# G1OJS/PyFT8

Measured on AMD Instinct MI355X. Metric: FT8 15-s frames decoded/sec, higher is better.
Workload: dtype f32

## Files before the change

pyft8_amd/csrc/ft8rx.hip:

```cpp
#include <hip/hip_runtime.h>
#include <math.h>
#include <stdarg.h>
#include <stdio.h>
#include <stdlib.h>
#include <string.h>
#include <new>
#include <string>
#include <vector>
#include "../../include/ft8rx.h"
#include "ft8_dev.h"

#define WL_MULT(i) ((i) == WL_BP0 ? 5 : (i) == WL_OSDNAN ? 10 : 1)
#define NF0MAX (FT8RX_MAX_F0 > 1024 ? 2048 : 1024)

#include "kernels/common.hpp"
#include "kernels/spectrogram.hpp"
#include "kernels/sync_search.hpp"
#include "kernels/llr.hpp"
#include "kernels/ap_patterns.hpp"
#include "kernels/bp.hpp"
#include "kernels/cycle_spectrum.hpp"
#include "kernels/fine_sync.hpp"
#include "kernels/osd.hpp"
#include "kernels/ap_calls.hpp"
#include "kernels/recall.hpp"
#include "kernels/report.hpp"
#include "kernels/synth.hpp"
#include "kernels/subtract.hpp"
#include "kernels/probes.hpp"
#include "host_messages.hpp"
#include "batch_plan.hpp"
#include "ilp_launch.hpp"

#define EV_EAGER_BYTES ((size_t)1 << 20)
#define HIPCHK(h, x) do { hipError_t _e = (x); if (_e != hipSuccess) { set_err(h, "%s failed: %s (%s:%d)", #x, hipGetErrorString(_e), __FILE__, __LINE__); return -2; } } while (0)

static std::vector<uint32_t> osd_trial_table(int S, int D, int T) {
    std::vector<uint32_t> t;
    const uint32_t N = OSD_NONE;
    t.push_back(N | (N << 8) | (N << 16));
    for (int i = 0; i < S; i++) t.push_back((uint32_t)i | (N << 8) | (N << 16));
    for (int i = 0; i < S; i++) for (int j = 0; j < D && j < i; j++) t.push_back((uint32_t)i | ((uint32_t)j << 8) | (N << 16));
    for (int i = 0; i < T; i++) for (int j = 0; j < i; j++) for (int k = 0; k < j; k++) t.push_back((uint32_t)i | ((uint32_t)j << 8) | ((uint32_t)k << 16));
    return t;
}
static int osd_nflip(int S, int T) { return S > T ? S : T; }

struct ft8rx_hashes { hostmsg::Hashes H; };

#define SYNC_WIN 352
static size_t sync_lds_bytes(const ft8rx_config& c) {
    const int nh0 = c.h0_hi - c.h0_lo;
    const size_t nrows = (size_t)((nh0 < SYNC_WIN ? nh0 : SYNC_WIN) + 24);
    return nrows * 16 * sizeof(double) + (nrows * 29 + 512) * sizeof(float);
}
static std::string g_create_err;

struct ResultSlot {
    ft8rx_record* rec = nullptr; int32_t* ncand = nullptr; ft8rx_event* ev = nullptr; int32_t* evcount = nullptr;
    ft8rx_record* h_rec = nullptr; int32_t* h_cnt = nullptr; ft8rx_event* h_ev = nullptr; int32_t* h_evc = nullptr;
    hipEvent_t ev_comp = nullptr, ev_done = nullptr;
    int B = 0;
    bool evpending = false;
    int32_t* d_evoffs = nullptr; ft8rx_event* h_evpacked = nullptr; ft8rx_event* d_evpacked = nullptr;
    bool packed = false;
    unsigned char* pk_buf = nullptr; hipEvent_t pk_fence = nullptr;
    ft8rx_packed_header* h_pkhdr = nullptr; ft8rx_packed_header* d_pkhdr = nullptr;
    bool recall = false;
    ft8rx_recall_entry* d_rc_ent = nullptr; int32_t* d_rc_cnt = nullptr; ft8rx_record* d_rc_rec = nullptr;
    ft8rx_record* h_rc_rec = nullptr; int32_t* h_rc_cnt = nullptr;
    bool reports = false;
    ft8rx_report* d_rp = nullptr; ft8rx_report* h_rp = nullptr;
};

static ApCalls ap_calls_off() { ApCalls a; memset(&a, 0, sizeof(a)); a.max_hd = FT8RX_AP_MAX_HD_DEFAULT; return a; }

struct ft8rx_handle {
    ft8rx_config cfg = {};
    int device = 0, max_frames = 0;
    hipStream_t stream = nullptr;
    int n_streams = 2;
    int ladder_mode = 0;
    int msg_types = 0;
    bool weak = false; float weak_sync_min = FT8RX_WEAK_SYNC_MIN_DEFAULT; int32_t weak_osd_max_hd = FT8RX_WEAK_OSD_MAX_HD_DEFAULT;
    ApCalls ap = ap_calls_off();
    uint32_t ap_version = 0, ap_chunk_version[batchplan::MAX_CHUNKS] = {};
    ApCalls* d_apc = nullptr;
    int32_t* d_apcount = nullptr;
    bool rc_armed = false; int rc_frames = 0; bool rc_td = false; std::vector<int32_t> rc_off;
    int32_t rc_max_hd = FT8RX_RECALL_MAX_HD_DEFAULT, rc_min_gap = FT8RX_RECALL_MIN_GAP_DEFAULT;
    ft8rx_recall_entry* d_rc_src = nullptr; int32_t* d_rc_srccnt = nullptr; int32_t* d_rc_off = nullptr;
    int32_t* d_rc_trip = nullptr; int32_t* d_rc_tout = nullptr; float* d_rc_tsd = nullptr; float* d_rc_sgrid = nullptr; float* d_rc_llr = nullptr;
    bool reports = false;
    int32_t* d_rp_items = nullptr; int32_t* d_rp_count = nullptr;
    int sub_frames = FT8RX_SUBBATCH_DEFAULT;
    hipStream_t sub[batchplan::MAX_STREAMS] = {};
    hipEvent_t ev_fork = nullptr, ev_join[batchplan::MAX_STREAMS] = {};
    hipStream_t copy_s = nullptr;
    hipEvent_t ev_chunk[batchplan::MAX_CHUNKS] = {};
    Tables T = {};
    std::vector<void*> allocs;
    struct Chunk { void* p; size_t cap, used; };
    std::vector<Chunk> arena;
    int16_t* d_audio = nullptr;
    int16_t* d_audio2 = nullptr;
    hipStream_t h2d_s = nullptr;
    float* d_grid = nullptr;
    float* d_best_score = nullptr; int32_t* d_best_h0 = nullptr;
    ft8rx_record* d_rec = nullptr; int32_t* d_ncand = nullptr; ft8rx_event* d_ev = nullptr; int32_t* d_evcount = nullptr;
    float* d_llr0 = nullptr; float* d_saved = nullptr;
    Att *d_att0 = nullptr, *d_attG = nullptr, *d_attB = nullptr, *d_attO = nullptr;
    cpx *d_A = nullptr, *d_spec = nullptr;
    const uint32_t* d_trials = nullptr; int n_trials = 0;
    int32_t* d_work[WL_N] = {};
    int32_t* d_wcount = nullptr;
    uint8_t* d_colmask = nullptr; bool use_mask = false;
    ResultSlot slots[2];
    int slot_enq = 0, slot_fetch = 0, inflight = 0, last_slot = -1, fetched_slot = -1;
    hipEvent_t ev_cdone[2][batchplan::MAX_STREAMS] = {};
    bool free_running = false, need_barrier = true; int part_B = 0, part_n = 0;
    uint64_t pk_cap = 0; uint64_t* d_pkneed = nullptr; int32_t* d_pknrec = nullptr;
    hipEvent_t d2h_ev[32] = {}; uint32_t d2h_next = 0;
    float* d_wf = nullptr; double2* d_part = nullptr; double* d_pulse = nullptr; double* d_pc = nullptr;
    ft8rx_subsig* d_sigs = nullptr; int32_t* d_sigcnt = nullptr; int sig_cap = 0;
    float2 *d_zdec = nullptr, *d_model = nullptr, *d_adec = nullptr; SubdCtx* d_subctx = nullptr;
    double* d_ones = nullptr;
    std::string err;
    bool profiling = false;
    std::vector<hipEvent_t> pev;
    std::vector<const char*> pnames;
    int n_stage = 0;
    float stage_ms[24] = {};
};
static_assert(sizeof(ft8rx_handle::ev_chunk) / sizeof(hipEvent_t) == batchplan::MAX_CHUNKS &&
              sizeof(ft8rx_handle::ap_chunk_version) / sizeof(uint32_t) == batchplan::MAX_CHUNKS &&
              sizeof(batchplan::BatchPlan::cb) / sizeof(int) == batchplan::MAX_CHUNKS + 1 &&
              batchplan::MAX_CHUNKS == 16 && batchplan::MAX_STREAMS == 8, "per-chunk arrays and the plan's boundaries");

static void set_err(ft8rx_handle* h, const char* fmt, ...) {
    char buf[512];
    va_list ap; va_start(ap, fmt); vsnprintf(buf, sizeof(buf), fmt, ap); va_end(ap);
    if (h) h->err = buf; else g_create_err = buf;
}

#include <mutex>
struct StreamPool { hipStream_t main = nullptr, copy = nullptr, h2d = nullptr, sub[8] = {}; };
static std::mutex g_pool_mu;
static StreamPool g_pool[64];
static hipStream_t pool_stream(int device, hipStream_t StreamPool::* which, bool blocking) {
    std::lock_guard<std::mutex> lk(g_pool_mu);
    StreamPool& P = g_pool[device & 63];
    if (!(P.*which)) {
        hipStream_t s = nullptr;
        if ((blocking ? hipStreamCreate(&s) : hipStreamCreateWithFlags(&s, hipStreamNonBlocking)) != hipSuccess) return nullptr;
        P.*which = s;
    }
    return P.*which;
}
static hipStream_t pool_sub(int device, int i) {
    std::lock_guard<std::mutex> lk(g_pool_mu);
    StreamPool& P = g_pool[device & 63];
    if (!P.sub[i] && hipStreamCreateWithFlags(&P.sub[i], hipStreamNonBlocking) != hipSuccess) P.sub[i] = nullptr;
    return P.sub[i];
}

template <typename T> static int dalloc(ft8rx_handle* h, T** p, size_t n) {
    void* q = nullptr;
    hipError_t e = hipMalloc(&q, n * sizeof(T));
    if (e != hipSuccess) { set_err(h, "hipMalloc(%zu bytes) failed: %s", n * sizeof(T), hipGetErrorString(e)); return -2; }
    h->allocs.push_back(q); *p = (T*)q; return 0;
}

static int need_staging(ft8rx_handle* h) {
    if (h->d_audio) return 0;
    return dalloc(h, &h->d_audio, (size_t)h->max_frames * FT8RX_NSAMP);
}

static void host_twiddle(int n, int count, std::vector<cpx>& w) {
    w.resize(count);
    for (int t = 0; t < count; t++) {
        double ang = (2.0 * M_PI * (double)t) / (double)n;
        w[t] = make_float2((float)cos(ang), (float)(-sin(ang)));
    }
}
template <typename T> static int upload(ft8rx_handle* h, const T** dst, const std::vector<T>& v) {
    T* p; if (dalloc(h, &p, v.size())) return -2;
    if (hipMemcpy(p, v.data(), v.size() * sizeof(T), hipMemcpyHostToDevice) != hipSuccess) { set_err(h, "table upload failed"); return -2; }
    *dst = p; return 0;
}

struct Scratch {
    ft8rx_handle* h;
    ~Scratch() { for (auto& c : h->arena) c.used = 0; }
    void* raw(size_t bytes) {
        bytes = (bytes + 255) & ~(size_t)255;
        if (!bytes) bytes = 256;
        for (auto& c : h->arena) if (c.cap - c.used >= bytes) { void* q = (char*)c.p + c.used; c.used += bytes; return q; }
        size_t largest = 0;
        for (auto& c : h->arena) if (c.cap > largest) largest = c.cap;
        size_t cap = bytes > 2 * largest ? bytes : 2 * largest;
        if (cap < ((size_t)1 << 20)) cap = (size_t)1 << 20;
        for (size_t i = 0; i < h->arena.size();) {
            if (h->arena[i].used == 0) { hipFree(h->arena[i].p); h->arena.erase(h->arena.begin() + i); } else i++;
        }
        void* q = nullptr;
        if (hipMalloc(&q, cap) != hipSuccess) { if (cap == bytes || hipMalloc(&q, bytes) != hipSuccess) return nullptr; cap = bytes; }
        h->arena.push_back({q, cap, bytes});
        return q;
    }
    template <typename T> T* get(size_t n) { return (T*)raw(n * sizeof(T)); }
    template <typename T> T* put(const T* src, size_t n) { T* q = get<T>(n); if (q && hipMemcpy(q, src, n * sizeof(T), hipMemcpyHostToDevice) != hipSuccess) return nullptr; return q; }
};

static int quiesce(ft8rx_handle* h, bool next_is_batch = false) {
    if (h->free_running || (h->last_slot >= 0 && !next_is_batch)) HIPCHK(h, hipStreamSynchronize(h->copy_s));
    h->free_running = false;
    h->need_barrier = true;
    return 0;
}
#define ENTER(h) do { HIPCHK(h, hipSetDevice((h)->device)); { const int _q = quiesce(h); if (_q) return _q; } } while (0)

template <class K, class KX, class... A>
static void launch_mt(K k, KX kx, unsigned mt, int grid, hipStream_t s, A... a) {
    if (!mt) k<<<grid, 64, 0, s>>>(a...);
    else kx<<<grid, 64, 0, s>>>(a..., mt);
}

extern "C" {

int ft8rx_default_config(ft8rx_config* c) {
    if (!c) return -1;
    c->sync_score_min = 85.0f; c->max_cands = 200; c->f0_lo = 32; c->f0_hi = 960; c->h0_lo = -37; c->h0_hi = 87;
    c->bp_nc0_a = 35; c->bp_iters_a = 5; c->bp_nc0_b = 90; c->bp_iters_b = 20; c->osd_single = 30; c->osd_double = 2;
    c->llr_sd_min = 5.0f;
    c->osd_triple = 0; c->osd_max_hd = 0;
    return 0;
}

int ft8rx_device_count(void) { int n = 0; if (hipGetDeviceCount(&n) != hipSuccess) return 0; return n; }
int ft8rx_device_pci_bus_id(int device, char* buf, int len) {
    if (!buf || len < 16) return -1;
    return hipDeviceGetPCIBusId(buf, len, device) == hipSuccess ? 0 : -2;
}
int ft8rx_build_info(int32_t* grid_cols, int32_t* spec_bins, int32_t* max_f0) {
    static_assert(NF0MAX >= FT8RX_GRID_COLS && NF0MAX >= FT8RX_MAX_F0, "per-f0 scratch stride");
    if (grid_cols) *grid_cols = FT8RX_GRID_COLS;
    if (spec_bins) *spec_bins = FT8RX_SPEC_BINS;
    if (max_f0) *max_f0 = FT8RX_MAX_F0;
    return 0;
}
int ft8rx_build_limits(int32_t* max_cands, int32_t* event_cap) {
    static_assert(FT8RX_MAX_CANDS <= NF0MAX && (1 << cand_shift(FT8RX_MAX_CANDS)) == FT8RX_MAX_CANDS,
                  "max_cands: never more than k_topk has keys, and the largest candidate stride is the limit itself");
    if (max_cands) *max_cands = FT8RX_MAX_CANDS;
    if (event_cap) *event_cap = FT8RX_EVENT_CAP;
    return 0;
}

int ft8rx_get_fft_plans(int32_t* p1920, int32_t* p3200, int32_t* p300, int32_t* p320) {
    const int32_t a[8] = {8, 4, 4, 5, 3, 0, 0, 0}, b[8] = {8, 4, 4, 5, 5, 0, 0, 0}, c[8] = {5, 5, 4, 3, 0, 0, 0, 0}, d[8] = {8, 8, 5, 0, 0, 0, 0, 0};
    if (p1920) memcpy(p1920, a, sizeof(a));
    if (p3200) memcpy(p3200, b, sizeof(b));
    if (p300) memcpy(p300, c, sizeof(c));
    if (p320) memcpy(p320, d, sizeof(d));
    return 0;
}

const char* ft8rx_last_error(ft8rx_handle* h) { return h ? h->err.c_str() : g_create_err.c_str(); }

void ft8rx_destroy(ft8rx_handle* h) {
    if (!h) return;
    hipSetDevice(h->device);
    if (h->stream) hipStreamSynchronize(h->stream);
    if (h->copy_s) hipStreamSynchronize(h->copy_s);
    if (h->h2d_s) hipStreamSynchronize(h->h2d_s);
    for (int i = 0; i < 8; i++) { if (h->sub[i]) hipStreamSynchronize(h->sub[i]); if (h->ev_join[i]) hipEventDestroy(h->ev_join[i]); }
    for (void* p : h->allocs) hipFree(p);
    for (auto& c : h->arena) hipFree(c.p);
    for (auto e : h->pev) hipEventDestroy(e);
    for (int k = 0; k < 2; k++) for (int i = 0; i < 8; i++) if (h->ev_cdone[k][i]) hipEventDestroy(h->ev_cdone[k][i]);
    for (int i = 0; i < 32; i++) if (h->d2h_ev[i]) hipEventDestroy(h->d2h_ev[i]);
    for (hipEvent_t e : h->ev_chunk) if (e) hipEventDestroy(e);
    if (h->ev_fork) hipEventDestroy(h->ev_fork);
    for (ResultSlot& sl : h->slots) {
        if (sl.ev_comp) hipEventDestroy(sl.ev_comp);
        if (sl.ev_done) hipEventDestroy(sl.ev_done);
        const auto hfree = [](void* p) { if (p) hipHostFree(p); };
        hfree(sl.h_rec); hfree(sl.h_cnt); hfree(sl.h_ev); hfree(sl.h_evc); hfree(sl.h_evpacked); hfree(sl.h_pkhdr);
        hfree(sl.h_rc_rec); hfree(sl.h_rc_cnt); hfree(sl.h_rp);
    }
    delete h;
}

int ft8rx_create(const ft8rx_config* cfg, int device, int max_frames, ft8rx_handle** out) {
    if (!cfg || !out || max_frames < 1) { set_err(nullptr, "ft8rx_create: bad arguments"); return -1; }
    if (cfg->max_cands < 1 || cfg->max_cands > FT8RX_MAX_CANDS || cfg->f0_lo < 4 || cfg->f0_hi > FT8RX_MAX_F0 || cfg->f0_lo >= cfg->f0_hi ||
        cfg->h0_hi <= cfg->h0_lo || cfg->h0_lo < FT8RX_MIN_H0 || cfg->h0_hi > FT8RX_MAX_H0 || cfg->bp_nc0_a > cfg->bp_nc0_b || cfg->bp_iters_a > cfg->bp_iters_b ||
        cfg->osd_single < 0 || cfg->osd_single > OSD_MAXFLIP || cfg->osd_double < 0 || cfg->osd_double > OSD_MAXFLIP ||
        cfg->osd_triple < 0 || cfg->osd_triple > 40 || cfg->osd_max_hd < 0 || cfg->osd_max_hd > 174 ||
        osd_trial_table(cfg->osd_single, cfg->osd_double, cfg->osd_triple).size() > OSD_MAXTRIALS) {
        set_err(nullptr, "ft8rx_create: configuration out of the supported range"); return -1; }
    int ndev = 0;
    if (hipGetDeviceCount(&ndev) != hipSuccess || ndev < 1) { set_err(nullptr, "ft8rx_create: no HIP device available (this library has no CPU fallback)"); return -3; }
    if (device < 0 || device >= ndev) { set_err(nullptr, "ft8rx_create: device %d out of range (%d devices)", device, ndev); return -1; }
    ft8rx_handle* h = new ft8rx_handle();
    h->cfg = *cfg; h->device = device; h->max_frames = max_frames;
    if (hipSetDevice(device) != hipSuccess || !(h->stream = pool_stream(device, &StreamPool::main, true))) { set_err(nullptr, "ft8rx_create: cannot open device %d", device); delete h; return -2; }
    const size_t B = (size_t)max_frames, S = (size_t)1 << cand_shift(*cfg);
    int rc = 0;
    rc |= dalloc(h, &h->d_grid, B * FT8RX_GRID_ROWS * FT8RX_GRID_COLS);
    rc |= dalloc(h, &h->d_best_score, B * NF0MAX);
    rc |= dalloc(h, &h->d_best_h0, B * NF0MAX);
    rc |= dalloc(h, &h->d_rec, B * S);
    rc |= dalloc(h, &h->d_ncand, B);
    rc |= dalloc(h, &h->d_llr0, B * S * 174);
    rc |= dalloc(h, &h->d_saved, B * S * 5 * 174);
    rc |= dalloc(h, &h->d_att0, B * S * 5);
    rc |= dalloc(h, &h->d_attG, B * S * 2);
    rc |= dalloc(h, &h->d_attB, B * S * 5);
    rc |= dalloc(h, &h->d_attO, B * S * 10);
    static_assert((size_t)(96000 + FT8RX_SPEC_BINS) * sizeof(cpx) <= (size_t)FT8RX_GRID_ROWS * FT8RX_GRID_COLS * sizeof(float), "scratch A + cycle spectrum fit a frame's grid");
    if (!rc) { h->d_A = reinterpret_cast<cpx*>(h->d_grid); h->d_spec = h->d_A + B * 96000; }
    for (int i = 0; i < WL_N; i++) rc |= dalloc(h, &h->d_work[i], B * S * WL_MULT(i));
    rc |= dalloc(h, &h->d_wcount, (size_t)batchplan::MAX_CHUNKS * WL_N);
    rc |= dalloc(h, &h->d_apc, batchplan::MAX_CHUNKS);
    rc |= dalloc(h, &h->d_apcount, (size_t)batchplan::MAX_CHUNKS * 2);
    rc |= dalloc(h, &h->d_ev, B * FT8RX_EVENT_CAP);
    rc |= dalloc(h, &h->d_evcount, B);
    ResultSlot* const sl = h->slots;
    sl[0].rec = h->d_rec; sl[0].ncand = h->d_ncand; sl[0].ev = h->d_ev; sl[0].evcount = h->d_evcount;
    rc |= dalloc(h, &sl[1].rec, B * S);
    rc |= dalloc(h, &sl[1].ncand, B);
    rc |= dalloc(h, &sl[1].ev, B * FT8RX_EVENT_CAP);
    rc |= dalloc(h, &sl[1].evcount, B);
    const bool ev_compact = B * FT8RX_EVENT_CAP * sizeof(ft8rx_event) > EV_EAGER_BYTES;
    for (int k = 0; k < 2 && ev_compact; k++) rc |= dalloc(h, &sl[k].d_evoffs, B + 1);
    for (int k = 0; k < 2 && !rc; k++) {
        bool okh = hipHostMalloc((void**)&sl[k].h_rec, sizeof(ft8rx_record) * B * cfg->max_cands, hipHostMallocDefault) == hipSuccess;
        okh = okh && hipHostMalloc((void**)&sl[k].h_cnt, sizeof(int32_t) * B, hipHostMallocDefault) == hipSuccess;
        okh = okh && hipHostMalloc((void**)&sl[k].h_ev, sizeof(ft8rx_event) * B * FT8RX_EVENT_CAP, hipHostMallocDefault) == hipSuccess;
        okh = okh && hipHostMalloc((void**)&sl[k].h_evc, sizeof(int32_t) * B, hipHostMallocDefault) == hipSuccess;
        if (ev_compact) okh = okh && hipHostMalloc((void**)&sl[k].h_evpacked, sizeof(ft8rx_event) * B * FT8RX_EVENT_CAP, hipHostMallocDefault) == hipSuccess
                                  && hipHostGetDevicePointer((void**)&sl[k].d_evpacked, sl[k].h_evpacked, 0) == hipSuccess;
        if (!okh) { set_err(h, "ft8rx_create: page-locked result buffers (%zu frames) could not be allocated", B); rc = -2; }
    }
    if (rc) { g_create_err = h->err; ft8rx_destroy(h); return -2; }
    std::vector<float> win(3840);
    for (int i = 0; i < 3840; i++) win[i] = (float)(0.5 + 0.5 * cos(M_PI * (double)(2 * i + 1 - 3840) / 3839.0));
    std::vector<double> taper(100);
    { double step = (0.0 - M_PI) / 99.0; for (int i = 0; i < 100; i++) { double y = (i == 99) ? 0.0 : (double)i * step + M_PI; taper[i] = 0.5 * (1.0 + cos(y)); } }
    std::vector<cpx> w;
    rc |= upload(h, &h->T.win, win);
    rc |= upload(h, &h->T.taper, taper);
    host_twiddle(1920, 1920, w);   rc |= upload(h, &h->T.W1920, w);
    host_twiddle(3840, FT8RX_GRID_COLS, w);    rc |= upload(h, &h->T.WR3840, w);
    host_twiddle(3200, 3200, w);   rc |= upload(h, &h->T.W3200, w);
    host_twiddle(96000, 96000, w); rc |= upload(h, &h->T.W96000, w);
    host_twiddle(300, 300, w);     rc |= upload(h, &h->T.W300, w);
    host_twiddle(320, 320, w);     rc |= upload(h, &h->T.W320, w);
    host_twiddle(192000, FT8RX_SPEC_BINS, w); rc |= upload(h, &h->T.WR192k, w);
    host_twiddle(32, 32, w);       rc |= upload(h, &h->T.W32, w);
    {
        std::vector<float> k32(1800);
        std::vector<cpx> cs(156), g1000(1000);
        for (int m = -900; m < 900; m++) {
            const int r = ((m % 100) + 100) % 100;
            k32[m + 900] = (r == 0) ? (m == 0 ? 32.0f : 0.0f) : (float)(sin(M_PI * (double)r / 100.0) / sin(M_PI * (double)m / 3200.0));
        }
        for (int sidx = 1; sidx < 7; sidx++) for (int q = 0; q <= 25; q++) {
            const double a = 2.0 * M_PI * (double)((q * sidx) % 100) / 100.0;
            cpx v = make_float2((float)cos(a), (float)sin(a));
            if (q == 0) v = make_float2(1.0f, 0.0f);
            cs[(sidx - 1) * 26 + q] = v;
        }
        for (int k = -150; k < 850; k++) {
            const int r = ((k % 100) + 100) % 100, j = (k - r) / 100;
            const double a = M_PI * (31.0 * (double)r - 100.0 * (double)j) / 3200.0;
            g1000[k + 150] = make_float2((float)cos(a), (float)sin(a));
        }
        std::vector<cpx> tw100(100);
        for (int m = 0; m < 100; m++) { const double a = -2.0 * M_PI * (double)m / 100.0; tw100[m] = make_float2((float)cos(a), (float)sin(a)); }
        rc |= upload(h, &h->T.K32, k32); rc |= upload(h, &h->T.CS100, cs); rc |= upload(h, &h->T.G1000, g1000); rc |= upload(h, &h->T.TW100, tw100);
    }
    if (rc) { g_create_err = h->err; ft8rx_destroy(h); return -2; }
    bool ok = true;
    ok &= hipMemcpyToSymbol(HIP_SYMBOL(d_CHK_N), FT8_CHK_N, sizeof(FT8_CHK_N)) == hipSuccess;
    ok &= hipMemcpyToSymbol(HIP_SYMBOL(d_CHK_V), FT8_CHK_V, sizeof(FT8_CHK_V)) == hipSuccess;
    {
        static uint8_t ev[522], ec[522]; static uint16_t ve[174][3];
        auto slot = [](int e) { const int c = FT8_EDGE_C[e], j = e - FT8_CHK_E0[c]; return j < 6 ? 83 * j + c : 498 + (c - 59); };
        for (int e = 0; e < 522; e++) { ev[slot(e)] = FT8_EDGE_V[e]; ec[slot(e)] = FT8_EDGE_C[e]; }
        for (int v = 0; v < 174; v++) for (int k = 0; k < 3; k++) ve[v][k] = (uint16_t)slot(FT8_VAR_E[v][k]);
        ok &= hipMemcpyToSymbol(HIP_SYMBOL(d_EDGE_V), ev, sizeof(ev)) == hipSuccess;
        ok &= hipMemcpyToSymbol(HIP_SYMBOL(d_EDGE_C), ec, sizeof(ec)) == hipSuccess;
        ok &= hipMemcpyToSymbol(HIP_SYMBOL(d_VAR_E), ve, sizeof(ve)) == hipSuccess;
    }
    ok &= hipMemcpyToSymbol(HIP_SYMBOL(d_G0), FT8_G0, sizeof(FT8_G0)) == hipSuccess;
    {
        static uint64_t rcg[83][2];
        memset(rcg, 0, sizeof(rcg));
        for (int r = 0; r < 91; r++) for (int j = 0; j < 83; j++) {
            const int v = 91 + j;
            if ((FT8_G0[r][v >> 6] >> (v & 63)) & 1ull) rcg[j][r >> 6] |= 1ull << (r & 63);
        }
        ok &= hipMemcpyToSymbol(HIP_SYMBOL(d_RCG), rcg, sizeof(rcg)) == hipSuccess;
    }
    {
        static uint64_t cm[128][3];
        memset(cm, 0, sizeof(cm));
        for (int c = 0; c < 83; c++) for (int j = 0; j < FT8_CHK_N[c]; j++) { int v = FT8_CHK_V[c][j]; cm[c][v >> 6] |= 1ull << (v & 63); }
        ok &= hipMemcpyToSymbol(HIP_SYMBOL(d_CHK_MASK), cm, sizeof(cm)) == hipSuccess;
    }
    {
        uint16_t syn[77];
        for (int pos = 0; pos < 77; pos++) syn[pos] = (uint16_t)hostmsg::crc14_serial(pos < 64 ? (1ull << pos) : 0ull, pos >= 64 ? (1ull << (pos - 64)) : 0ull);
        ok &= hipMemcpyToSymbol(HIP_SYMBOL(d_CRC_SYN), syn, sizeof(syn)) == hipSuccess;
    }
    {
        static uint32_t g0t[192][3];
        memset(g0t, 0, sizeof(g0t));
        for (int r = 0; r < 91; r++) for (int v = 0; v < 174; v++) if ((FT8_G0[r][v >> 6] >> (v & 63)) & 1ull) g0t[v][r >> 5] |= 1u << (r & 31);
        ok &= hipMemcpyToSymbol(HIP_SYMBOL(d_G0T), g0t, sizeof(g0t)) == hipSuccess;
        uint16_t syn91[96]; memset(syn91, 0, sizeof(syn91));
        for (int v = 0; v < 91; v++) {
            if (v < 77) { const int pos = 76 - v; syn91[v] = (uint16_t)hostmsg::crc14_serial(pos < 64 ? (1ull << pos) : 0ull, pos >= 64 ? (1ull << (pos - 64)) : 0ull); }
            else syn91[v] = (uint16_t)(1u << (13 - (v - 77)));
        }
        uint32_t synm[14][3]; memset(synm, 0, sizeof(synm));
        for (int v = 0; v < 91; v++) for (int k = 0; k < 14; k++) if ((syn91[v] >> k) & 1) synm[k][v >> 5] |= 1u << (v & 31);
        ok &= hipMemcpyToSymbol(HIP_SYMBOL(d_SYNM), synm, sizeof(synm)) == hipSuccess;
        static uint16_t ct[12][256];
        for (int b = 0; b < 12; b++) for (int x = 0; x < 256; x++) { uint16_t a = 0; for (int t = 0; t < 8; t++) if ((x >> t) & 1) a ^= syn91[8 * b + t]; ct[b][x] = a; }
        ok &= hipMemcpyToSymbol(HIP_SYMBOL(d_CRC_T), ct, sizeof(ct)) == hipSuccess;
        {
            float xn[174]; int perm[176], stk[64]; uint8_t p8[192];
            for (int i = 0; i < 174; i++) xn[i] = NAN;
            osd_std_sort_withnan(xn, perm, stk);
            memset(p8, 0, sizeof(p8));
            for (int i = 0; i < 174; i++) p8[i] = (uint8_t)perm[i];
            ok &= hipMemcpyToSymbol(HIP_SYMBOL(d_NANPERM), p8, sizeof(p8)) == hipSuccess;
        }
        const std::vector<uint32_t> tr = osd_trial_table(cfg->osd_single, cfg->osd_double, cfg->osd_triple);
        h->n_trials = (int)tr.size();
        if (upload(h, &h->d_trials, tr)) ok = false;
    }
    if (!ok) { set_err(nullptr, "ft8rx_create: device table upload failed"); ft8rx_destroy(h); return -2; }
    if (sync_lds_bytes(*cfg) > 65536) {
        ok &= hipFuncSetAttribute((const void*)k_sync, hipFuncAttributeMaxDynamicSharedMemorySize, (int)sync_lds_bytes(*cfg)) == hipSuccess;
        ok &= hipFuncSetAttribute((const void*)k_sync_acc, hipFuncAttributeMaxDynamicSharedMemorySize, (int)sync_lds_bytes(*cfg)) == hipSuccess;
    }
    if (!ok) { set_err(nullptr, "ft8rx_create: cannot reserve LDS for k_sync"); ft8rx_destroy(h); return -2; }
    int nfill = (int)B * FT8RX_GRID_COLS;
    k_fill_row0<<<(nfill + 255) / 256, 256, 0, h->stream>>>(h->d_grid, (int)B);
    if (hipStreamSynchronize(h->stream) != hipSuccess) { set_err(nullptr, "ft8rx_create: init kernel failed"); ft8rx_destroy(h); return -2; }
    bool okc = true;
    for (int i = 0; i < 24; i++) { hipEvent_t e = nullptr; okc = okc && hipEventCreate(&e) == hipSuccess; if (e) h->pev.push_back(e); }
    if (const char* e = getenv("FT8RX_SUBS_FIRST")) for (int i = 0; i < atoi(e) && i < 8; i++) pool_sub(device, i);
    okc = okc && (h->copy_s = pool_stream(device, &StreamPool::copy, false)) != nullptr;
    okc = okc && (h->h2d_s = pool_stream(device, &StreamPool::h2d, false)) != nullptr;
    for (hipEvent_t& e : h->ev_chunk) okc = okc && hipEventCreateWithFlags(&e, hipEventDisableTiming) == hipSuccess;
    okc = okc && hipEventCreateWithFlags(&h->ev_fork, hipEventDisableTiming) == hipSuccess;
    for (ResultSlot& s : h->slots) {
        okc = okc && hipEventCreateWithFlags(&s.ev_comp, hipEventDisableTiming) == hipSuccess;
        okc = okc && hipEventCreateWithFlags(&s.ev_done, hipEventDisableTiming) == hipSuccess;
    }
    if (!okc) { set_err(nullptr, "ft8rx_create: cannot create HIP streams/events"); ft8rx_destroy(h); return -2; }
    *out = h;
    return 0;
}

int ft8rx_set_profiling(ft8rx_handle* h, int on) { if (!h) return -1; h->profiling = on != 0; return 0; }

int ft8rx_get_stage_times(ft8rx_handle* h, int* n, const char** names, float* ms) {
    if (!h || !n) return -1;
    *n = h->n_stage;
    for (int i = 0; i < h->n_stage; i++) { if (names) names[i] = h->pnames[i]; if (ms) ms[i] = h->stage_ms[i]; }
    return 0;
}


#ifndef LADDER_GRID_CAP
#define LADDER_GRID_CAP (4 * 256 * 32)
#endif

static int ladder_grid(int max_items) { const int cap = LADDER_GRID_CAP; return max_items < cap ? max_items : cap; }

static void launch_sync(const float* grid, float* bs, int32_t* bh, const ft8rx_config& c, int B, hipStream_t s, bool weak) {
    const auto first = weak ? k_sync3 : k_sync, acc = weak ? k_sync3_acc : k_sync_acc;
    const int win = weak ? SYNC3_WIN : SYNC_WIN;
    const size_t lds = weak ? 0 : sync_lds_bytes(c);
    const int ntile = (c.f0_hi - c.f0_lo + 15) / 16;
    for (int lo = c.h0_lo; lo < c.h0_hi; lo += win) {
        ft8rx_config w = c;
        w.h0_lo = lo; w.h0_hi = lo + win < c.h0_hi ? lo + win : c.h0_hi;
        (lo == c.h0_lo ? first : acc)<<<dim3(ntile, B), 256, lds, s>>>(grid, bs, bh, w);
    }
}
static ft8rx_config weak_config(const ft8rx_handle* h) {
    ft8rx_config w = h->cfg;
    w.sync_score_min = h->weak_sync_min;
    w.llr_sd_min = -INFINITY;
    if (!w.osd_max_hd) w.osd_max_hd = h->weak_osd_max_hd;
    return w;
}
static void launch_fine(ft8rx_handle* h, const ft8rx_config& cfg, bool weak, int n_blocks, hipStream_t s, const cpx* spec, ft8rx_record* rec,
                        const int32_t* ncand, float* llr, const int32_t* trip, int32_t* t_out, float* t_sd, float* t_sgrid, WorkList work,
                        bool need_td) {
    if (weak) { k_fine_weak<<<n_blocks, FINE_NT, 0, s>>>(spec, rec, ncand, llr, h->T, cfg, trip, t_out, t_sd, t_sgrid, work); return; }
    ft8rx_ilp_fine(n_blocks, s, spec, rec, ncand, llr, h->T, cfg, trip, t_out, t_sd, t_sgrid, work);
    if (need_td) k_fine_td<<<n_blocks, FINE_NT, 0, s>>>(spec, rec, ncand, llr, h->T, cfg, trip, t_out, t_sd, t_sgrid, work);
}

static bool osd_wide(int nflip) { return nflip > OSD_FLIPS_A; }
static void launch_osd(unsigned mt, int grid, hipStream_t s, int mode, const float* llr, const float* saved, const Att* attB, ft8rx_record* rec,
                       const int32_t* ncand, Att* attO, ft8rx_event* ev, int32_t* evc, const uint32_t* trials, int ntr, int nflip, int max_hd,
                       int sh, WorkList work, WorkList nanl) {
    const bool wide = osd_wide(nflip);
    launch_mt(wide ? k_osd_wide : k_osd, wide ? k_osd_wide_ext : k_osd_ext, mt, grid, s,
              mode, llr, saved, attB, rec, ncand, attO, ev, evc, trials, ntr, nflip, max_hd, sh, work, nanl);
    launch_mt(wide ? k_osd_nan_wide : k_osd_nan, wide ? k_osd_nan_wide_ext : k_osd_nan_ext, mt, OSD_NAN_GRID, s,
              mode, llr, saved, attB, rec, ncand, attO, ev, evc, trials, ntr, nflip, max_hd, sh, nanl);
}

static void launch_ap_calls(ft8rx_handle* h, int B, const float* llr0, ft8rx_record* rec, const int32_t* ncand, Att* attO, ft8rx_event* ev,
                            int32_t* evc, int32_t* cand_items, int32_t* osd_items, int32_t* ac, const ApCalls* apc, hipStream_t s) {
    const ft8rx_config& c = h->cfg;
    const int sh = cand_shift(c); const size_t S = (size_t)1 << sh;
    const int nflip = osd_nflip(c.osd_single, c.osd_triple);
    hipMemsetAsync(ac, 0, 2 * sizeof(int32_t), s);
    const WorkList cl = {cand_items, ac}, ol = {osd_items, ac + 1};
    k_ap_worklist<<<(B * S + 255) / 256, 256, 0, s>>>(rec, ncand, B, sh, cl);
    k_bp_ap<<<ladder_grid(B * c.max_cands * h->ap.np), 64, 0, s>>>(llr0, rec, ncand, attO, ev, evc, c, apc, cl, ol);
    (osd_wide(nflip) ? k_osd_ap_wide : k_osd_ap)<<<ladder_grid(B * c.max_cands * 3), 64, 0, s>>>(
        llr0, rec, ncand, attO, ev, evc, h->d_trials, h->n_trials, nflip, sh, apc, ol);
    k_select_ap<<<(B * S + 255) / 256, 256, 0, s>>>(rec, attO, apc, cl);
}

static void launch_reports(ft8rx_handle* h, int B, const cpx* spec, const ft8rx_record* rec, const int32_t* ncand, int32_t* items,
                           int32_t* count, ft8rx_report* rep, hipStream_t s) {
    const ft8rx_config& c = h->cfg;
    const int sh = cand_shift(c); const size_t S = (size_t)1 << sh;
    hipMemsetAsync(count, 0, sizeof(int32_t), s);
    const WorkList wl = {items, count};
    k_report_worklist<<<(B * S + 255) / 256, 256, 0, s>>>(rec, ncand, B, sh, wl, rep);
    k_report<<<ladder_grid(B * c.max_cands), FINE_NT, 0, s>>>(spec, rec, rep, h->T, sh, wl);
}

static void enqueue_chain(ft8rx_handle* h, const int16_t* d_audio, int f0, int B, hipStream_t s, bool prof, int slot, int chunk) {
    const ResultSlot& sl = h->slots[slot];
    const bool weak = h->weak;
    const ft8rx_config cw = weak ? weak_config(h) : h->cfg;
    const ft8rx_config& c = weak ? cw : h->cfg;
    const size_t F = (size_t)f0;
    const int sh = cand_shift(c); const size_t S = (size_t)1 << sh, FS = F * S;
    const int16_t* audio = d_audio + F * FT8RX_NSAMP;
    float* grid = h->d_grid + F * FT8RX_GRID_ROWS * FT8RX_GRID_COLS;
    float* bs = h->d_best_score + F * NF0MAX; int32_t* bh = h->d_best_h0 + F * NF0MAX;
    ft8rx_record* rec = sl.rec + FS; int32_t* ncand = sl.ncand + F;
    float* llr0 = h->d_llr0 + FS * 174; float* saved = h->d_saved + FS * 5 * 174;
    Att* att0 = h->d_att0 + FS * 5; Att* attG = h->d_attG + FS * 2; Att* attB = h->d_attB + FS * 5; Att* attO = h->d_attO + FS * 10;
    cpx* A = reinterpret_cast<cpx*>(grid); cpx* spec = A + (size_t)B * 96000;
    ft8rx_event* ev = sl.ev + F * FT8RX_EVENT_CAP; int32_t* evc = sl.evcount + F;
#define STAGE(name) do { if (prof) { hipEventRecord(h->pev[h->pnames.size()], s); h->pnames.push_back(name); } } while (0)
    int32_t* wc = h->d_wcount + WL_N * chunk;
    WorkList wl[WL_N];
    for (int i = 0; i < WL_N; i++) { wl[i].items = h->d_work[i] + FS * WL_MULT(i); wl[i].count = wc + i; }
    STAGE("spectrogram");
    ft8rx_ilp_spectrogram(B, s, audio, grid, h->T);
    STAGE("sync");
    launch_sync(grid, bs, bh, c, B, s, weak);
    STAGE("topk");
    k_topk<<<B, 1024, 0, s>>>(bs, bh, rec, ncand, c, evc, wc, h->use_mask ? h->d_colmask + F * NF0MAX : nullptr);
    STAGE("grid_llr");
    const unsigned mt = (unsigned)h->msg_types;
    launch_mt(k_grid_llr, k_grid_llr_ext, mt, XCD_GRID(B, c.max_cands), s, grid, rec, ncand, llr0, c, nullptr, nullptr, nullptr, att0, ev, evc, B);
    k_worklist_att<<<(B * S * 5 + 255) / 256, 256, 0, s>>>(rec, ncand, att0, B, sh, wl[WL_BP0]);
    STAGE("bp_grid");
    launch_mt(k_bp, k_bp_ext, mt, ladder_grid(B * c.max_cands * 5), s, 0, llr0, rec, ncand, nullptr, att0, nullptr, ev, evc, c, c.bp_nc0_a, c.bp_iters_a, wl[WL_BP0], 0, 5);
    STAGE("select0");
    k_select0<<<(B * S + 255) / 256, 256, 0, s>>>(rec, ncand, att0, B, sh, wl[WL_FINE]);
    STAGE("cycle_fft");
    k_cyc_a<<<dim3(40, B), 256, 0, s>>>(audio, A, h->T);
    k_cyc_bc<<<dim3(CYC_BC_GRID, B), 256, 0, s>>>(A, spec, h->T);
    STAGE("fine");
    launch_fine(h, c, weak, ladder_grid(B * c.max_cands), s, spec, rec, ncand, llr0, nullptr, nullptr, nullptr, nullptr, wl[WL_FINE],
                c.h0_lo < FT8RX_MIN_H0_FD || c.h0_hi > FT8RX_MAX_H0_FD + 1);
    k_worklist<<<(B * S + 255) / 256, 256, 0, s>>>(rec, ncand, B, sh, wl[WL_BP1]);
    STAGE("bp_fine");
    const auto bp_fine = [&](int n_variants, const WorkList& work, int v0) {
        launch_mt(k_bp, k_bp_ext, mt, B * c.max_cands * n_variants, s, 1, llr0, rec, ncand, attG, attB, saved, ev, evc, c, c.bp_nc0_b, c.bp_iters_b,
                  work, v0, n_variants);
    };
    if (h->ladder_mode == 0) {
        bp_fine(1, wl[WL_BP1], 0);
        k_select1<<<(B * S + 255) / 256, 256, 0, s>>>(0, rec, ncand, attG, attB, B, c, wl[WL_BP1B]);
        bp_fine(1, wl[WL_BP1B], 1);
        k_select1<<<(B * S + 255) / 256, 256, 0, s>>>(1, rec, ncand, attG, attB, B, c, wl[WL_BP1C]);
        bp_fine(3, wl[WL_BP1C], 2);
        STAGE("select1");
        k_select1<<<(B * S + 255) / 256, 256, 0, s>>>(2, rec, ncand, attG, attB, B, c, wl[WL_OSD]);
    } else {
        bp_fine(5, wl[WL_BP1], 0);
        STAGE("select1");
        k_select1<<<(B * S + 255) / 256, 256, 0, s>>>(3, rec, ncand, attG, attB, B, c, wl[WL_OSD]);
    }
    STAGE("osd");
    launch_osd(mt, ladder_grid(B * c.max_cands * 10), s, 0, llr0, saved, attB, rec, ncand, attO, ev, evc, h->d_trials, h->n_trials,
               osd_nflip(c.osd_single, c.osd_triple), c.osd_max_hd, sh, wl[WL_OSD], wl[WL_OSDNAN]);
    STAGE("select2");
    k_select2<<<(B * S + 255) / 256, 256, 0, s>>>(rec, ncand, attO, B, sh);
    if (h->ap.np) {
        STAGE("ap_calls");
        ApCalls* apc = h->d_apc + chunk;
        if (h->ap_chunk_version[chunk] != h->ap_version) {
            k_ap_stage<<<1, 64, 0, s>>>(apc, h->ap);
            h->ap_chunk_version[chunk] = h->ap_version;
        }
        launch_ap_calls(h, B, llr0, rec, ncand, attO, ev, evc, wl[WL_BP0].items, wl[WL_OSDNAN].items, h->d_apcount + 2 * chunk, apc, s);
    }
    if (sl.recall) {
        STAGE("recall");
        ft8rx_recall_entry* ent = sl.d_rc_ent + F * FT8RX_RECALL_MAX;
        int32_t* rcnt = sl.d_rc_cnt + F;
        k_recall_stage<<<B, FT8RX_RECALL_MAX, 0, s>>>(h->d_rc_src + F * FT8RX_RECALL_MAX, h->d_rc_srccnt + F, ent, rcnt, sl.d_rc_rec + F * FT8RX_RECALL_MAX);
        const int base = h->rc_off[F], n = h->rc_off[F + B] - base;
        if (n > 0) {
            k_recall_trip<<<B, FT8RX_RECALL_MAX, 0, s>>>(ent, rcnt, h->d_rc_off + F, h->d_rc_trip);
            const size_t b = (size_t)base;
            launch_fine(h, c, false, n, s, spec, nullptr, nullptr, h->d_rc_llr + b * 174, h->d_rc_trip + 3 * b, h->d_rc_tout + 5 * b,
                        h->d_rc_tsd + b, h->d_rc_sgrid + b * 632, WorkList{nullptr, nullptr}, h->rc_td);
            k_recall_score<<<n, 64, 0, s>>>(h->d_rc_sgrid, h->d_rc_tout, h->d_rc_trip, h->d_rc_off + F, base, ent, rec, ncand, sh,
                                            h->rc_max_hd, h->rc_min_gap, sl.d_rc_rec + F * FT8RX_RECALL_MAX);
        }
    }
    if (sl.reports) {
        STAGE("report");
        launch_reports(h, B, spec, rec, ncand, h->d_rp_items + FS, h->d_rp_count + chunk, sl.d_rp + FS, s);
    }
    if (prof) hipEventRecord(h->pev[h->pnames.size()], s);
#undef STAGE
}

static void enqueue_chunk(ft8rx_handle* h, const int16_t* d_audio, int f0, int n, hipStream_t s, int slot, int chunk) {
    const int sub = (h->sub_frames > 0 && h->sub_frames < n) ? h->sub_frames : n;
    for (int o = 0; o < n; o += sub) enqueue_chain(h, d_audio, f0 + o, (o + sub <= n) ? sub : n - o, s, false, slot, chunk);
}

using batchplan::BatchPlan;
using batchplan::Entry;

static int batch_begin(ft8rx_handle* h, Entry e, int B, int slot, bool chunked, int16_t** stage) {
    ResultSlot& sl = h->slots[slot];
    h->pnames.clear();
    if (h->inflight == 2) { h->slot_fetch ^= 1; h->inflight = 1; }
    if (e != batchplan::DEVICE && need_staging(h)) return -2;
    if (h->rc_armed && B != h->rc_frames) { set_err(h, "recall entries were set for %d frames, the batch has %d", h->rc_frames, B); return -1; }
    sl.recall = h->rc_armed;
    h->rc_armed = false;
    sl.reports = h->reports;
    *stage = h->d_audio;
    if (e == batchplan::HOST_PIPELINED) {
        if (slot == 1 && !h->d_audio2 && dalloc(h, &h->d_audio2, (size_t)h->max_frames * FT8RX_NSAMP)) return -2;
        *stage = slot ? h->d_audio2 : h->d_audio;
        HIPCHK(h, hipStreamWaitEvent(h->h2d_s, sl.ev_comp, 0));
    }
    for (int i = 1; i < h->n_streams && chunked; i++) if (!h->sub[i - 1]) {
        if (!(h->sub[i - 1] = pool_sub(h->device, i - 1))) { set_err(h, "cannot create a chunk stream"); return -2; }
        HIPCHK(h, hipEventCreateWithFlags(&h->ev_join[i - 1], hipEventDisableTiming));
    }
    return 0;
}

static int batch_submit(ft8rx_handle* h, const BatchPlan& plan, Entry e, int slot, const int16_t* audio, int16_t* stage) {
    ResultSlot& sl = h->slots[slot];
    const bool host = e != batchplan::DEVICE;
    const int16_t* d_audio = host ? stage : audio; const int16_t* host_audio = host ? audio : nullptr;
    const int ns = h->n_streams, nc = plan.nc, B = plan.cb[nc];
    const bool free_run = plan.mode == batchplan::FREE_RUN, pipelined = e == batchplan::HOST_PIPELINED, sync_host = e == batchplan::HOST_SYNC;
    hipStream_t cs = pipelined ? h->h2d_s : h->copy_s;
    const size_t frame_bytes = sizeof(int16_t) * (size_t)FT8RX_NSAMP;
    auto chunk_stream = [&](int k) { const int i = k % ns; return i == 0 ? h->stream : h->sub[i - 1]; };
    if (free_run) {
        for (int i = 0; i < ns; i++) for (int k = 0; k < 2; k++)
            if (!h->ev_cdone[k][i]) HIPCHK(h, hipEventCreateWithFlags(&h->ev_cdone[k][i], hipEventDisableTiming));
        if (h->need_barrier || h->part_B != B || h->part_n != nc) {
            if (h->free_running) HIPCHK(h, hipStreamWaitEvent(h->stream, h->slots[h->last_slot].ev_comp, 0));
            HIPCHK(h, hipEventRecord(h->ev_fork, h->stream));
            for (int i = 1; i < ns; i++) HIPCHK(h, hipStreamWaitEvent(h->sub[i - 1], h->ev_fork, 0));
            h->need_barrier = false; h->part_B = B; h->part_n = nc;
        }
    } else {
        { const int q = quiesce(h, true); if (q) return q; }
        HIPCHK(h, hipStreamWaitEvent(h->stream, sl.ev_done, 0));
        if (plan.mode == batchplan::SINGLE) {
            if (host_audio) HIPCHK(h, hipMemcpyAsync(stage, host_audio, frame_bytes * B, hipMemcpyHostToDevice, h->stream));
            if (h->profiling) enqueue_chain(h, d_audio, 0, B, h->stream, true, slot, 0);
            else enqueue_chunk(h, d_audio, 0, B, h->stream, slot, 0);
            return 0;
        }
        HIPCHK(h, hipEventRecord(h->ev_fork, h->stream));
        if (sync_host) HIPCHK(h, hipStreamWaitEvent(cs, h->ev_fork, 0));
        for (int i = 1; i < ns; i++) HIPCHK(h, hipStreamWaitEvent(h->sub[i - 1], h->ev_fork, 0));
    }
    if (pipelined) {
        HIPCHK(h, hipMemcpyAsync(stage, host_audio, frame_bytes * B, hipMemcpyHostToDevice, cs));
        HIPCHK(h, hipEventRecord(h->ev_chunk[0], cs));
        if (!free_run) for (int i = 0; i < ns; i++) HIPCHK(h, hipStreamWaitEvent(chunk_stream(i), h->ev_chunk[0], 0));
    }
    for (int k = 0; k < nc; k++) {
        const int f0 = plan.cb[k], n = plan.cb[k + 1] - f0;
        if (n <= 0 && !free_run) continue;
        hipStream_t s = chunk_stream(k);
        if (free_run) {
            HIPCHK(h, hipStreamWaitEvent(s, sl.ev_done, 0));
            if (pipelined) HIPCHK(h, hipStreamWaitEvent(s, h->ev_chunk[0], 0));
        } else if (sync_host) {
            HIPCHK(h, hipMemcpyAsync(stage + (size_t)f0 * FT8RX_NSAMP, host_audio + (size_t)f0 * FT8RX_NSAMP, frame_bytes * n, hipMemcpyHostToDevice, cs));
            HIPCHK(h, hipEventRecord(h->ev_chunk[k], cs));
            HIPCHK(h, hipStreamWaitEvent(s, h->ev_chunk[k], 0));
        }
        if (n > 0) enqueue_chunk(h, d_audio, f0, n, s, slot, k);
        if (free_run) {
            HIPCHK(h, hipEventRecord(h->ev_cdone[slot][k], s));
            HIPCHK(h, hipStreamWaitEvent(h->copy_s, h->ev_cdone[slot][k], 0));
        }
    }
    if (free_run) h->free_running = true;
    else for (int i = 1; i < ns; i++) {
        HIPCHK(h, hipEventRecord(h->ev_join[i - 1], h->sub[i - 1]));
        HIPCHK(h, hipStreamWaitEvent(h->stream, h->ev_join[i - 1], 0));
    }
    return 0;
}

static int batch_finish(ft8rx_handle* h, int slot, int B, hipStream_t fin) {
    ResultSlot& sl = h->slots[slot];
    const int mc = h->cfg.max_cands, sh = cand_shift(h->cfg);
    const bool pack_events = sl.d_evpacked && (size_t)B * FT8RX_EVENT_CAP * sizeof(ft8rx_event) > EV_EAGER_BYTES;
    if (pack_events) {
        k_ev_scan<<<1, 1024, 0, fin>>>(sl.evcount, B, sl.d_evoffs);
        k_ev_compact<<<B, 64, 0, fin>>>(sl.ev, sl.evcount, sl.d_evoffs, sl.d_evpacked);
    }
    sl.packed = sl.pk_buf != nullptr;
    if (sl.packed) {
        if (sl.pk_fence) { HIPCHK(h, hipStreamWaitEvent(fin, sl.pk_fence, 0)); sl.pk_fence = nullptr; }
        k_pack_count<<<B, 256, 0, fin>>>(sl.rec, sl.ncand, sl.ev, sl.evcount, h->d_pkneed, h->d_pknrec, sh);
        k_pack_scan<<<1, 1024, 0, fin>>>(h->d_pknrec, sl.ncand, sl.evcount, B, mc, (unsigned long long)h->pk_cap, sl.pk_buf, sl.d_pkhdr);
        k_pack_write<<<B, 256, 0, fin>>>(sl.rec, sl.ev, h->d_pkneed, B, sl.pk_buf, sh);
    }
    HIPCHK(h, hipEventRecord(sl.ev_comp, fin));
    if (fin != h->copy_s) HIPCHK(h, hipStreamWaitEvent(h->copy_s, sl.ev_comp, 0));
    HIPCHK(h, hipMemcpyAsync(sl.h_cnt, sl.ncand, sizeof(int32_t) * B, hipMemcpyDeviceToHost, h->copy_s));
    HIPCHK(h, hipMemcpy2DAsync(sl.h_rec, sizeof(ft8rx_record) * mc, sl.rec, sizeof(ft8rx_record) << sh, sizeof(ft8rx_record) * mc, B, hipMemcpyDeviceToHost, h->copy_s));
    HIPCHK(h, hipMemcpyAsync(sl.h_evc, sl.evcount, sizeof(int32_t) * B, hipMemcpyDeviceToHost, h->copy_s));
    sl.evpending = pack_events;
    if (!pack_events) HIPCHK(h, hipMemcpyAsync(sl.h_ev, sl.ev, sizeof(ft8rx_event) * (size_t)B * FT8RX_EVENT_CAP, hipMemcpyDeviceToHost, h->copy_s));
    if (sl.recall) {
        HIPCHK(h, hipMemcpyAsync(sl.h_rc_cnt, sl.d_rc_cnt, sizeof(int32_t) * B, hipMemcpyDeviceToHost, h->copy_s));
        HIPCHK(h, hipMemcpyAsync(sl.h_rc_rec, sl.d_rc_rec, sizeof(ft8rx_record) * FT8RX_RECALL_MAX * (size_t)B, hipMemcpyDeviceToHost, h->copy_s));
    }
    if (sl.reports)
        HIPCHK(h, hipMemcpy2DAsync(sl.h_rp, sizeof(ft8rx_report) * mc, sl.d_rp, sizeof(ft8rx_report) << sh, sizeof(ft8rx_report) * mc, B, hipMemcpyDeviceToHost, h->copy_s));
    HIPCHK(h, hipEventRecord(sl.ev_done, h->copy_s));
    sl.B = B; h->last_slot = slot; h->slot_enq ^= 1; h->inflight++;
    return 0;
}

static int launch_batch(ft8rx_handle* h, Entry e, const int16_t* audio, int B) {
    HIPCHK(h, hipSetDevice(h->device));
    const BatchPlan plan = batchplan::plan_batch(B, h->n_streams, h->profiling, e);
    const int slot = h->slot_enq;
    int16_t* stage = nullptr;
    if (const int rc = batch_begin(h, e, B, slot, plan.mode != batchplan::SINGLE, &stage)) return rc;
    if (const int rc = batch_submit(h, plan, e, slot, audio, stage)) return rc;
    HIPCHK(h, hipGetLastError());
    return batch_finish(h, slot, B, plan.mode == batchplan::FREE_RUN ? h->copy_s : h->stream);
}

static void fetch_events(ResultSlot& sl) {
    if (!sl.evpending) return;
    size_t off = 0;
    for (int f = 0; f < sl.B; f++) {
        int c = sl.h_evc[f]; c = c > FT8RX_EVENT_CAP ? FT8RX_EVENT_CAP : (c < 0 ? 0 : c);
        if (c) memcpy(sl.h_ev + (size_t)f * FT8RX_EVENT_CAP, sl.h_evpacked + off, sizeof(ft8rx_event) * (size_t)c);
        off += (size_t)c;
    }
    sl.evpending = false;
}

int ft8rx_enqueue_batch(ft8rx_handle* h, const int16_t* d_audio, int B) {
    if (!h || !d_audio) return -1;
    if (B < 1 || B > h->max_frames) { set_err(h, "ft8rx_enqueue_batch: n_frames %d outside [1, %d]", B, h->max_frames); return -1; }
    return launch_batch(h, batchplan::DEVICE, d_audio, B);
}

int ft8rx_enqueue_batch_host(ft8rx_handle* h, const int16_t* audio, int B) {
    if (!h || !audio) return -1;
    if (B < 1 || B > h->max_frames) { set_err(h, "ft8rx_enqueue_batch_host: n_frames %d outside [1, %d]", B, h->max_frames); return -1; }
    return launch_batch(h, batchplan::HOST_PIPELINED, audio, B);
}

int ft8rx_set_streams(ft8rx_handle* h, int n) { if (!h || n < 1 || n > batchplan::MAX_STREAMS) return -1; h->n_streams = n; return 0; }
int ft8rx_set_subbatch(ft8rx_handle* h, int frames) { if (!h || frames < 0) return -1; h->sub_frames = frames; return 0; }
int ft8rx_set_ladder_mode(ft8rx_handle* h, int mode) { if (!h || mode < 0 || mode > 1) return -1; h->ladder_mode = mode; return 0; }

int ft8rx_set_weak(ft8rx_handle* h, int32_t on, float sync_min, int32_t osd_max_hd) {
    if (!h) return -1;
    if (on) {
        if (!(sync_min > 0.0f) || !(sync_min < INFINITY)) { set_err(h, "ft8rx_set_weak: sync_min %g must be a positive score", (double)sync_min); return -1; }
        if (osd_max_hd < 1 || osd_max_hd > 174) { set_err(h, "ft8rx_set_weak: osd_max_hd %d outside [1, 174]", osd_max_hd); return -1; }
        if (h->slots[0].pk_buf) { set_err(h, "ft8rx_set_weak: not supported together with the packed output (ft8rx_set_packed_output)"); return -1; }
        if (h->msg_types) { set_err(h, "ft8rx_set_weak: not supported together with msg_types != 0"); return -1; }
        if (h->ap.np) { set_err(h, "ft8rx_set_weak: not supported together with ft8rx_set_ap_calls"); return -1; }
        if (h->rc_armed) { set_err(h, "ft8rx_set_weak: not supported together with ft8rx_set_recall"); return -1; }
        h->weak_sync_min = sync_min; h->weak_osd_max_hd = osd_max_hd;
    }
    h->weak = on != 0;
    return 0;
}

int ft8rx_set_msg_types(ft8rx_handle* h, int32_t mask) {
    if (!h) return -1;
    if (mask < 0 || mask > FT8RX_MT_ALL) { set_err(h, "ft8rx_set_msg_types: mask %d outside [0, %d]", mask, FT8RX_MT_ALL); return -1; }
    if (mask && h->slots[0].pk_buf) { set_err(h, "ft8rx_set_msg_types: the packed output renders only the reference's message types"); return -1; }
    if (mask && h->ap.np) { set_err(h, "ft8rx_set_msg_types: not supported together with ft8rx_set_ap_calls"); return -1; }
    if (mask && h->rc_armed) { set_err(h, "ft8rx_set_msg_types: not supported together with ft8rx_set_recall"); return -1; }
    if (mask && h->weak) { set_err(h, "ft8rx_set_msg_types: not supported together with ft8rx_set_weak"); return -1; }
    h->msg_types = mask;
    return 0;
}

static int build_ap_patterns(const char* my, const char* dx, ApCalls* a, std::string* err) {
    const bool hm = my && *my, hd = dx && *dx;
    const long cm = hm ? hostmsg::pack_c28_std(my) : 0, cd = hd ? hostmsg::pack_c28_std(dx) : 0;
    if (cm < 0) { *err = std::string("my_call '") + my + "' is not a standard callsign"; return -1; }
    if (cd < 0) { *err = std::string("dx_call '") + dx + "' is not a standard callsign"; return -1; }
    const int32_t max_hd = a->max_hd;
    memset(a, 0, sizeof(*a)); a->max_hd = max_hd;
    auto word = [](long c1, long c2, unsigned g15) { return ((unsigned __int128)c1 << 49) | ((unsigned __int128)c2 << 20) | ((unsigned __int128)g15 << 3) | 1u; };
    const unsigned G_RRR = 32402, G_73 = 32404, G_RR73 = 32403;
    for (int p = 5; p <= 10; p++) {
        const bool on = p == 5 ? hm : p == 7 ? hd : (hm && hd);
        if (!on) continue;
        const int k = p - FT8RX_AP_FIRST;
        const unsigned __int128 w = word(p == 7 ? 2 : cm, p == 5 ? 0 : cd, p == 8 ? G_RRR : p == 9 ? G_73 : G_RR73);
        const uint64_t lo = (uint64_t)w, hi = (uint64_t)(w >> 64);
        if (p >= 8) {
            hostmsg::encode_cw174(lo, hi, a->val[k]);
            a->msk[k][0] = a->msk[k][1] = ~0ull; a->msk[k][2] = (1ull << 46) - 1;
            a->lo[k] = lo; a->hi[k] = hi;
            hostmsg::Hashes H; std::string f[3];
            if (!hostmsg::unpack_ext(lo, hi, 0, H, f)) { *err = "the words of my_call / dx_call do not unpack as a standard message"; return -1; }
        } else {
            const int nk = p == 5 ? 29 : 58;
            for (int i = 0; i < 77; i++) {
                if (!(i < nk || i >= 74)) continue;
                const unsigned b = (unsigned)((w >> (76 - i)) & 1u);
                a->msk[k][i >> 6] |= 1ull << (i & 63);
                if (b) a->val[k][i >> 6] |= 1ull << (i & 63);
            }
        }
        a->pat[a->np++] = p;
    }
    return 0;
}

int ft8rx_set_ap_calls(ft8rx_handle* h, const char* my_call, const char* dx_call) {
    if (!h) return -1;
    ApCalls a = h->ap;
    std::string err;
    if (build_ap_patterns(my_call, dx_call, &a, &err)) { set_err(h, "ft8rx_set_ap_calls: %s", err.c_str()); return -1; }
    if (a.np && h->msg_types) { set_err(h, "ft8rx_set_ap_calls: not supported together with msg_types != 0"); return -1; }
    if (a.np && h->weak) { set_err(h, "ft8rx_set_ap_calls: not supported together with ft8rx_set_weak"); return -1; }
    if (a.np && h->slots[0].pk_buf) { set_err(h, "ft8rx_set_ap_calls: not supported on the packed output"); return -1; }
    h->ap = a; h->ap_version++;
    return 0;
}

int ft8rx_set_ap_max_hd(ft8rx_handle* h, int32_t max_hd) {
    if (!h) return -1;
    if (max_hd < 1 || max_hd > 174) { set_err(h, "ft8rx_set_ap_max_hd: %d outside [1, 174]", max_hd); return -1; }
    h->ap.max_hd = max_hd; h->ap_version++;
    return 0;
}

int ft8rx_ap_patterns(const char* my_call, const char* dx_call, uint8_t* bits_out, uint8_t* mask_out) {
    ApCalls a = ap_calls_off();
    std::string err;
    if (build_ap_patterns(my_call, dx_call, &a, &err)) { g_create_err = "ft8rx_ap_patterns: " + err; return -1; }
    for (int k = 0; k < FT8RX_AP_N; k++) for (int i = 0; i < 174; i++) {
        if (bits_out) bits_out[k * 174 + i] = (uint8_t)((a.val[k][i >> 6] >> (i & 63)) & 1ull);
        if (mask_out) mask_out[k * 174 + i] = (uint8_t)((a.msk[k][i >> 6] >> (i & 63)) & 1ull);
    }
    return 0;
}

static int recall_kind(uint64_t lo, uint64_t hi) {
    const unsigned i3 = (unsigned)(lo & 7u);
    if (i3 != 1 && i3 != 2) return RC_SKIP;
    const uint64_t ca = ((lo >> 49) | (hi << 15)) & 0xFFFFFFFull, cb = (lo >> 20) & 0xFFFFFFFull;
    const uint64_t STD = 2063592ull + 4194304ull;
    if (cb < STD || !(ca < 3 || ca >= STD)) return RC_SKIP;
    hostmsg::Hashes H; std::string f[3];
    if (!hostmsg::unpack_ext(lo, hi & 0x1FFFull, 0, H, f)) return RC_SKIP;
    for (int k = 0; k < 3; k++) if (f[k].find('<') != std::string::npos) return RC_SKIP;
    return ca < 3 ? RC_TOKEN : RC_CALL;
}

int ft8rx_recall_hypotheses(const ft8rx_recall_entry* entry, uint64_t* words_lo, uint64_t* words_hi) {
    if (!entry) return -1;
    const uint64_t lo = entry->msg_lo, hi = entry->msg_hi & 0x1FFFull;
    const int kind = recall_kind(lo, hi);
    if (kind == RC_SKIP) return 0;
    int n = 0;
    for (int k = 0; k < 126; k++) {
        uint64_t w; unsigned g15 = 0, r = 0;
        if (k == 0) w = lo;
        else if (kind != RC_CALL) break;
        else {
            if (k <= 3) g15 = 32401u + (unsigned)k;
            else if (k < 65) g15 = (unsigned)(32435 + (k - 4) - 30);
            else { g15 = (unsigned)(32435 + (k - 65) - 30); r = 1; }
            w = (lo & ~(0xFFFFull << 3)) | ((uint64_t)g15 << 3) | ((uint64_t)r << 18);
            if (w == lo) continue;
        }
        if (words_lo) words_lo[n] = w;
        if (words_hi) words_hi[n] = hi;
        n++;
    }
    return n;
}

static int recall_alloc(ft8rx_handle* h) {
    if (h->d_rc_src) return 0;
    const size_t B = (size_t)h->max_frames, N = B * FT8RX_RECALL_MAX;
    int rc = 0;
    rc |= dalloc(h, &h->d_rc_src, N); rc |= dalloc(h, &h->d_rc_srccnt, B); rc |= dalloc(h, &h->d_rc_off, B + 1);
    rc |= dalloc(h, &h->d_rc_trip, N * 3); rc |= dalloc(h, &h->d_rc_tout, N * 5); rc |= dalloc(h, &h->d_rc_tsd, N);
    rc |= dalloc(h, &h->d_rc_sgrid, N * 632); rc |= dalloc(h, &h->d_rc_llr, N * 174);
    for (int k = 0; k < 2 && !rc; k++) {
        ResultSlot& sl = h->slots[k];
        rc |= dalloc(h, &sl.d_rc_ent, N); rc |= dalloc(h, &sl.d_rc_cnt, B); rc |= dalloc(h, &sl.d_rc_rec, N);
        if (!rc && (hipHostMalloc((void**)&sl.h_rc_rec, sizeof(ft8rx_record) * N, hipHostMallocDefault) != hipSuccess ||
                    hipHostMalloc((void**)&sl.h_rc_cnt, sizeof(int32_t) * B, hipHostMallocDefault) != hipSuccess)) {
            set_err(h, "ft8rx_set_recall: page-locked result buffers could not be allocated"); rc = -2; }
    }
    if (rc) { h->d_rc_src = nullptr; return -2; }
    return 0;
}

int ft8rx_set_recall(ft8rx_handle* h, const ft8rx_recall_entry* entries, const int32_t* counts, int n_frames) {
    if (!h) return -1;
    ENTER(h);
    if (!entries || n_frames == 0) { h->rc_armed = false; return 0; }
    if (!counts || n_frames < 1 || n_frames > h->max_frames) { set_err(h, "ft8rx_set_recall: n_frames %d outside [1, %d]", n_frames, h->max_frames); return -1; }
    if (h->msg_types) { set_err(h, "ft8rx_set_recall: not supported together with msg_types != 0"); return -1; }
    if (h->weak) { set_err(h, "ft8rx_set_recall: not supported together with ft8rx_set_weak"); return -1; }
    if (h->slots[0].pk_buf) { set_err(h, "ft8rx_set_recall: not supported on the packed output"); return -1; }
    const ft8rx_config& c = h->cfg;
    std::vector<ft8rx_recall_entry> st((size_t)n_frames * FT8RX_RECALL_MAX);
    std::vector<int32_t> cnt(n_frames), off(n_frames + 1, 0);
    bool td = false;
    for (int f = 0; f < n_frames; f++) {
        if (counts[f] < 0 || counts[f] > FT8RX_RECALL_MAX) { set_err(h, "ft8rx_set_recall: counts[%d] = %d outside [0, %d]", f, counts[f], FT8RX_RECALL_MAX); return -1; }
        cnt[f] = counts[f]; off[f + 1] = off[f] + counts[f];
        for (int e = 0; e < counts[f]; e++) {
            ft8rx_recall_entry E = entries[(size_t)f * FT8RX_RECALL_MAX + e];
            if (E.f0_idx < c.f0_lo || E.f0_idx >= c.f0_hi || E.h0_idx < c.h0_lo || E.h0_idx >= c.h0_hi) {
                set_err(h, "ft8rx_set_recall: entry %d of frame %d at (f0_idx %d, h0_idx %d) lies outside the search range", e, f, E.f0_idx, E.h0_idx); return -1; }
            E.pad = (uint16_t)recall_kind(E.msg_lo, E.msg_hi);
            td |= E.h0_idx < FT8RX_MIN_H0_FD || E.h0_idx > FT8RX_MAX_H0_FD;
            st[(size_t)f * FT8RX_RECALL_MAX + e] = E;
        }
    }
    if (recall_alloc(h)) return -2;
    HIPCHK(h, hipMemcpy(h->d_rc_src, st.data(), sizeof(ft8rx_recall_entry) * st.size(), hipMemcpyHostToDevice));
    HIPCHK(h, hipMemcpy(h->d_rc_srccnt, cnt.data(), sizeof(int32_t) * cnt.size(), hipMemcpyHostToDevice));
    HIPCHK(h, hipMemcpy(h->d_rc_off, off.data(), sizeof(int32_t) * off.size(), hipMemcpyHostToDevice));
    h->rc_off = off; h->rc_frames = n_frames; h->rc_td = td; h->rc_armed = true;
    return 0;
}

int ft8rx_fetch_recall(ft8rx_handle* h, int n_frames, ft8rx_record* records, int32_t* counts) {
    if (!h) return -1;
    const int slot = h->fetched_slot;
    if (slot < 0) { set_err(h, "ft8rx_fetch_recall: no batch has been fetched"); return -1; }
    const ResultSlot& sl = h->slots[slot];
    if (n_frames < 1 || n_frames > sl.B) { set_err(h, "ft8rx_fetch_recall: %d frames requested, the batch had %d", n_frames, sl.B); return -1; }
    HIPCHK(h, hipEventSynchronize(sl.ev_done));
    if (!sl.recall) {
        if (counts) memset(counts, 0, sizeof(int32_t) * n_frames);
        if (records) memset(records, 0, sizeof(ft8rx_record) * FT8RX_RECALL_MAX * (size_t)n_frames);
        return 0;
    }
    if (counts) memcpy(counts, sl.h_rc_cnt, sizeof(int32_t) * n_frames);
    if (records) memcpy(records, sl.h_rc_rec, sizeof(ft8rx_record) * FT8RX_RECALL_MAX * (size_t)n_frames);
    return 0;
}

int ft8rx_set_reports(ft8rx_handle* h, int32_t on) {
    if (!h) return -1;
    ENTER(h);
    if (!on) { h->reports = false; return 0; }
    if (h->slots[0].pk_buf) { set_err(h, "ft8rx_set_reports: not supported together with the packed output (ft8rx_set_packed_output)"); return -1; }
    if (!h->d_rp_items) {
        const size_t B = (size_t)h->max_frames, N = B << cand_shift(h->cfg);
        int rc = 0;
        rc |= dalloc(h, &h->d_rp_items, N); rc |= dalloc(h, &h->d_rp_count, (size_t)batchplan::MAX_CHUNKS);
        for (int k = 0; k < 2 && !rc; k++) {
            rc |= dalloc(h, &h->slots[k].d_rp, N);
            if (!rc && hipHostMalloc((void**)&h->slots[k].h_rp, sizeof(ft8rx_report) * B * h->cfg.max_cands, hipHostMallocDefault) != hipSuccess) {
                set_err(h, "ft8rx_set_reports: page-locked result buffers could not be allocated"); rc = -2; }
        }
        if (rc) { h->d_rp_items = nullptr; return -2; }
    }
    h->reports = true;
    return 0;
}

int ft8rx_fetch_reports(ft8rx_handle* h, int n_frames, ft8rx_report* reports) {
    if (!h || !reports) return -1;
    const int slot = h->fetched_slot;
    if (slot < 0) { set_err(h, "ft8rx_fetch_reports: no batch has been fetched"); return -1; }
    const ResultSlot& sl = h->slots[slot];
    if (n_frames < 1 || n_frames > sl.B) { set_err(h, "ft8rx_fetch_reports: %d frames requested, the batch had %d", n_frames, sl.B); return -1; }
    HIPCHK(h, hipEventSynchronize(sl.ev_done));
    const size_t bytes = sizeof(ft8rx_report) * (size_t)n_frames * h->cfg.max_cands;
    if (!sl.reports) memset(reports, 0, bytes);
    else memcpy(reports, sl.h_rp, bytes);
    return 0;
}

int ft8rx_set_recall_gates(ft8rx_handle* h, int32_t max_hd, int32_t min_gap) {
    if (!h) return -1;
    if (max_hd < 1 || max_hd > 174 || min_gap < 0 || min_gap > 174) { set_err(h, "ft8rx_set_recall_gates: max_hd %d / min_gap %d outside [1, 174] / [0, 174]", max_hd, min_gap); return -1; }
    h->rc_max_hd = max_hd; h->rc_min_gap = min_gap;
    return 0;
}

int ft8rx_set_search_mask(ft8rx_handle* h, const uint8_t* mask, int n_frames) {
    if (!h) return -1;
    ENTER(h);
    if (!mask) { h->use_mask = false; return 0; }
    if (n_frames < 1 || n_frames > h->max_frames) { set_err(h, "ft8rx_set_search_mask: n_frames %d outside [1, %d]", n_frames, h->max_frames); return -1; }
    if (!h->d_colmask && dalloc(h, &h->d_colmask, (size_t)h->max_frames * NF0MAX)) return -2;
    const int nf0 = h->cfg.f0_hi - h->cfg.f0_lo;
    HIPCHK(h, hipMemsetAsync(h->d_colmask, 0, (size_t)h->max_frames * NF0MAX, h->stream));
    HIPCHK(h, hipMemcpy2DAsync(h->d_colmask, NF0MAX, mask, (size_t)nf0, (size_t)nf0, n_frames, hipMemcpyHostToDevice, h->stream));
    HIPCHK(h, hipStreamSynchronize(h->stream));
    h->use_mask = true;
    return 0;
}

int ft8rx_sync(ft8rx_handle* h) {
    if (!h) return -1;
    HIPCHK(h, hipSetDevice(h->device));
    HIPCHK(h, hipStreamSynchronize(h->stream));
    HIPCHK(h, hipStreamSynchronize(h->copy_s));
    if (h->profiling && !h->pnames.empty()) {
        h->n_stage = (int)h->pnames.size();
        for (int i = 0; i < h->n_stage; i++) hipEventElapsedTime(&h->stage_ms[i], h->pev[i], h->pev[i + 1]);
    }
    return 0;
}

static int fetch_begin(ft8rx_handle* h, const char* who, int B, bool with_events, bool to_device, int* slot) {
    if (!h || B < 1 || B > h->max_frames) return -1;
    if (h->last_slot < 0) { set_err(h, "%s: nothing has been enqueued", who); return -1; }
    HIPCHK(h, hipSetDevice(h->device));
    *slot = (h->inflight && !to_device) ? h->slot_fetch : h->last_slot;
    ResultSlot& sl = h->slots[*slot];
    if (B > sl.B) { set_err(h, "%s: %d frames requested, the batch had %d", who, B, sl.B); return -1; }
    HIPCHK(h, hipEventSynchronize(to_device ? sl.ev_comp : sl.ev_done));
    if (with_events && !to_device) fetch_events(sl);
    return 0;
}
static void fetch_end(ft8rx_handle* h, int slot) {
    h->fetched_slot = slot;
    if (h->inflight) { h->slot_fetch ^= 1; h->inflight--; }
}

int ft8rx_fetch_results(ft8rx_handle* h, int B, ft8rx_record* records, int32_t* counts, ft8rx_event* events, int32_t* event_counts) {
    int slot;
    if (const int rc = fetch_begin(h, "ft8rx_fetch_results", B, events != nullptr, false, &slot)) return rc;
    const ResultSlot& sl = h->slots[slot];
    const size_t mc = (size_t)h->cfg.max_cands;
    if (counts) memcpy(counts, sl.h_cnt, sizeof(int32_t) * B);
    if (records) memcpy(records, sl.h_rec, sizeof(ft8rx_record) * mc * B);
    if (event_counts) memcpy(event_counts, sl.h_evc, sizeof(int32_t) * B);
    if (events) for (int f = 0; f < B; f++) {
        int c = sl.h_evc[f]; if (c > FT8RX_EVENT_CAP) c = FT8RX_EVENT_CAP;
        if (c > 0) memcpy(events + (size_t)f * FT8RX_EVENT_CAP, sl.h_ev + (size_t)f * FT8RX_EVENT_CAP, sizeof(ft8rx_event) * (size_t)c);
    }
    fetch_end(h, slot);
    return 0;
}

int ft8rx_fetch_results_view(ft8rx_handle* h, int B, const ft8rx_record** records, const int32_t** counts,
                             const ft8rx_event** events, const int32_t** event_counts) {
    int slot;
    if (const int rc = fetch_begin(h, "ft8rx_fetch_results_view", B, events != nullptr, false, &slot)) return rc;
    const ResultSlot& sl = h->slots[slot];
    if (records) *records = sl.h_rec;
    if (counts) *counts = sl.h_cnt;
    if (events) *events = sl.h_ev;
    if (event_counts) *event_counts = sl.h_evc;
    fetch_end(h, slot);
    return 0;
}

int ft8rx_set_packed_output(ft8rx_handle* h, void* d_buf0, void* d_buf1, uint64_t cap_bytes) {
    if (!h) return -1;
    ENTER(h);
    HIPCHK(h, hipStreamSynchronize(h->copy_s));
    ResultSlot* const sl = h->slots;
    sl[0].pk_fence = sl[1].pk_fence = nullptr;
    if (!d_buf0 && !d_buf1) { sl[0].pk_buf = sl[1].pk_buf = nullptr; h->pk_cap = 0; return 0; }
    if (h->msg_types) { set_err(h, "ft8rx_set_packed_output: msg_types != 0 -- the packed output renders only the reference's message types"); return -1; }
    if (h->ap.np) { set_err(h, "ft8rx_set_packed_output: not supported while ft8rx_set_ap_calls has a call set"); return -1; }
    if (h->rc_armed) { set_err(h, "ft8rx_set_packed_output: not supported while ft8rx_set_recall entries are pending"); return -1; }
    if (h->weak) { set_err(h, "ft8rx_set_packed_output: not supported together with ft8rx_set_weak"); return -1; }
    if (h->reports) { set_err(h, "ft8rx_set_packed_output: not supported together with ft8rx_set_reports"); return -1; }
    if (!d_buf0 || !d_buf1 || d_buf0 == d_buf1 || cap_bytes < sizeof(ft8rx_packed_header)) {
        set_err(h, "ft8rx_set_packed_output: two distinct buffers of at least %zu bytes each are needed", sizeof(ft8rx_packed_header)); return -1; }
    void* in[2] = {d_buf0, d_buf1};
    unsigned char* dev[2];
    for (int k = 0; k < 2; k++) {
        hipPointerAttribute_t at;
        if (hipPointerGetAttributes(&at, in[k]) != hipSuccess) { (void)hipGetLastError(); set_err(h, "ft8rx_set_packed_output: buffer %d is neither device nor page-locked host memory", k); return -1; }
        if (at.type != hipMemoryTypeDevice && at.type != hipMemoryTypeHost && at.type != hipMemoryTypeManaged) {
            set_err(h, "ft8rx_set_packed_output: buffer %d is ordinary host memory; use device memory or ft8rx_alloc_host", k); return -1; }
        dev[k] = (unsigned char*)(at.type == hipMemoryTypeHost ? at.devicePointer : in[k]);
        if (!dev[k] || ((uintptr_t)dev[k] & 15)) { set_err(h, "ft8rx_set_packed_output: buffer %d is not device-accessible / 16-byte aligned", k); return -1; }
    }
    if (!h->d_pkneed) {
        int rc = dalloc(h, &h->d_pkneed, (size_t)h->max_frames * ((1 << cand_shift(h->cfg)) / 64));
        rc |= dalloc(h, &h->d_pknrec, (size_t)h->max_frames);
        if (rc) return -2;
        for (int k = 0; k < 2; k++) {
            if (hipHostMalloc((void**)&sl[k].h_pkhdr, sizeof(ft8rx_packed_header), hipHostMallocDefault) != hipSuccess ||
                hipHostGetDevicePointer((void**)&sl[k].d_pkhdr, sl[k].h_pkhdr, 0) != hipSuccess) { set_err(h, "ft8rx_set_packed_output: page-locked header could not be allocated"); return -2; }
            memset(sl[k].h_pkhdr, 0, sizeof(ft8rx_packed_header));
        }
    }
    sl[0].pk_buf = dev[0]; sl[1].pk_buf = dev[1]; h->pk_cap = cap_bytes;
    return 0;
}

int ft8rx_packed_output_fence(ft8rx_handle* h, int which, void* hip_event) {
    if (!h || which < 0 || which > 1) return -1;
    h->slots[which].pk_fence = (hipEvent_t)hip_event;
    return 0;
}

int ft8rx_packed_results(ft8rx_handle* h, int32_t* which, ft8rx_packed_header* header) {
    if (!h) return -1;
    if (h->fetched_slot < 0 || !h->slots[h->fetched_slot].packed) { set_err(h, "ft8rx_packed_results: the batch fetched last was enqueued without a packed output (ft8rx_set_packed_output)"); return -1; }
    if (which) *which = h->fetched_slot;
    if (header) *header = *h->slots[h->fetched_slot].h_pkhdr;
    return 0;
}

int ft8rx_results_to_device(ft8rx_handle* h, int B, ft8rx_record* d_records, int32_t* d_counts, ft8rx_event* d_events, int32_t* d_event_counts) {
    int slot;
    if (const int rc = fetch_begin(h, "ft8rx_results_to_device", B, false, true, &slot)) return rc;
    const ResultSlot& sl = h->slots[slot];
    HIPCHK(h, hipStreamSynchronize(h->stream));
    const int mc = h->cfg.max_cands;
    if (d_counts) HIPCHK(h, hipMemcpyAsync(d_counts, sl.ncand, sizeof(int32_t) * B, hipMemcpyDeviceToDevice, h->stream));
    if (d_records) HIPCHK(h, hipMemcpy2DAsync(d_records, sizeof(ft8rx_record) * mc, sl.rec, sizeof(ft8rx_record) << cand_shift(h->cfg),
                                              sizeof(ft8rx_record) * mc, B, hipMemcpyDeviceToDevice, h->stream));
    if (d_event_counts) HIPCHK(h, hipMemcpyAsync(d_event_counts, sl.evcount, sizeof(int32_t) * B, hipMemcpyDeviceToDevice, h->stream));
    if (d_events) HIPCHK(h, hipMemcpyAsync(d_events, sl.ev, sizeof(ft8rx_event) * (size_t)B * FT8RX_EVENT_CAP, hipMemcpyDeviceToDevice, h->stream));
    HIPCHK(h, hipStreamSynchronize(h->stream));
    return 0;
}

static int launch_batch_sync(ft8rx_handle* h, const int16_t* audio, int B) {
    h->inflight = 0; h->slot_fetch = h->slot_enq;
    if (need_staging(h)) return -2;
    return launch_batch(h, batchplan::HOST_SYNC, audio, B);
}

int ft8rx_decode_batch(ft8rx_handle* h, const int16_t* audio, int B, ft8rx_record* records, int32_t* counts,
                       ft8rx_event* events, int32_t* event_counts) {
    if (!h || !audio) return -1;
    if (B < 1 || B > h->max_frames) { set_err(h, "ft8rx_decode_batch: n_frames %d outside [1, %d]", B, h->max_frames); return -1; }
    if (const int rc = launch_batch_sync(h, audio, B)) return rc;
    return ft8rx_fetch_results(h, B, records, counts, events, event_counts);
}

int ft8rx_decode_messages(ft8rx_handle* h, const int16_t* audio, int B, ft8rx_message* out, int max_msgs, int32_t* out_counts,
                          int n_threads, ft8rx_hashes* table, int32_t* flags) {
    if (!h || !audio || !out || !out_counts) return -1;
    if (B < 1 || B > h->max_frames || max_msgs < 1) { set_err(h, "ft8rx_decode_messages: bad n_frames / max_msgs"); return -1; }
    if (h->msg_types) { set_err(h, "ft8rx_decode_messages: msg_types != 0 -- ft8rx_message holds only the reference's message types"); return -1; }
    if (h->rc_armed) { set_err(h, "ft8rx_decode_messages: recall entries (ft8rx_set_recall) are not supported; use ft8rx_decode_batch + ft8rx_fetch_recall"); return -1; }
    int rc = launch_batch_sync(h, audio, B);
    if (rc) return rc;
    const ft8rx_record* rec; const int32_t* cnt; const ft8rx_event* ev; const int32_t* evc;
    rc = ft8rx_fetch_results_view(h, B, &rec, &cnt, &ev, &evc);
    if (rc) return rc;
    return hostmsg::package_batch(rec, cnt, ev, evc, B, h->cfg.max_cands, out, max_msgs, out_counts, n_threads, table ? &table->H : nullptr, flags);
}

#define NEED(p) do { if (!(p)) { set_err(h, "scratch allocation/copy failed (%s:%d)", __FILE__, __LINE__); return -2; } } while (0)

int ft8rx_spectrogram(ft8rx_handle* h, const int16_t* audio, int B, float* grid) {
    if (!h || !audio || !grid || B < 1 || B > h->max_frames) return -1;
    ENTER(h);
    if (need_staging(h)) return -2;
    HIPCHK(h, hipMemcpy(h->d_audio, audio, sizeof(int16_t) * (size_t)B * FT8RX_NSAMP, hipMemcpyHostToDevice));
    ft8rx_ilp_spectrogram(B, h->stream, h->d_audio, h->d_grid, h->T);
    HIPCHK(h, hipStreamSynchronize(h->stream));
    HIPCHK(h, hipMemcpy(grid, h->d_grid, sizeof(float) * (size_t)B * FT8RX_GRID_ROWS * FT8RX_GRID_COLS, hipMemcpyDeviceToHost));
    return 0;
}

int ft8rx_hop_spectrum(ft8rx_handle* h, const int16_t* window3840, float* row) {
    if (!h || !window3840 || !row) return -1;
    ENTER(h);
    if (need_staging(h)) return -2;
    float* d_row = h->d_best_score;
    HIPCHK(h, hipMemcpyAsync(h->d_audio, window3840, sizeof(int16_t) * 3840, hipMemcpyHostToDevice, h->stream));
    ft8rx_ilp_hop_spectrum(h->stream, h->d_audio, d_row, h->T);
    HIPCHK(h, hipMemcpyAsync(row, d_row, sizeof(float) * FT8RX_GRID_COLS, hipMemcpyDeviceToHost, h->stream));
    HIPCHK(h, hipStreamSynchronize(h->stream));
    return 0;
}

int ft8rx_sync_search(ft8rx_handle* h, const float* grid, int B, int32_t* f0_idx, int32_t* h0_idx, float* score, int32_t* counts) {
    if (!h || !grid || B < 1 || B > h->max_frames) return -1;
    ENTER(h);
    const ft8rx_config& c = h->cfg;
    HIPCHK(h, hipMemcpy(h->d_grid, grid, sizeof(float) * (size_t)B * FT8RX_GRID_ROWS * FT8RX_GRID_COLS, hipMemcpyHostToDevice));
    launch_sync(h->d_grid, h->d_best_score, h->d_best_h0, c, B, h->stream, false);
    k_topk<<<B, 1024, 0, h->stream>>>(h->d_best_score, h->d_best_h0, h->d_rec, h->d_ncand, c, nullptr, nullptr, nullptr);
    HIPCHK(h, hipStreamSynchronize(h->stream));
    const size_t S = (size_t)1 << cand_shift(c);
    std::vector<ft8rx_record> rec((size_t)B * S);
    HIPCHK(h, hipMemcpy(rec.data(), h->d_rec, sizeof(ft8rx_record) * rec.size(), hipMemcpyDeviceToHost));
    HIPCHK(h, hipMemcpy(counts, h->d_ncand, sizeof(int32_t) * B, hipMemcpyDeviceToHost));
    for (int f = 0; f < B; f++) for (int i = 0; i < c.max_cands; i++) {
        const ft8rx_record& r = rec[(size_t)f * S + i];
        size_t o = (size_t)f * c.max_cands + i;
        f0_idx[o] = r.f0_idx; h0_idx[o] = r.h0_idx; score[o] = r.score;
    }
    return 0;
}

static int sync_scores(ft8rx_handle* h, const float* grid, int B, int f0_lo, int f0_hi, float* score, int32_t* h0_idx, bool weak) {
    const char* who = weak ? "ft8rx_sync_scores_weak" : "ft8rx_sync_scores";
    if (!h || !grid || !score || !h0_idx || B < 1 || B > h->max_frames) return -1;
    if (f0_lo < 4 || f0_hi <= f0_lo || f0_hi > FT8RX_GRID_COLS - 15 || f0_hi - f0_lo > NF0MAX) {
        set_err(h, "%s: f0 range [%d, %d) outside [4, %d]", who, f0_lo, f0_hi, FT8RX_GRID_COLS - 15); return -1; }
    ENTER(h);
    ft8rx_config c = h->cfg;
    c.f0_lo = f0_lo; c.f0_hi = f0_hi;
    HIPCHK(h, hipMemcpy(h->d_grid, grid, sizeof(float) * (size_t)B * FT8RX_GRID_ROWS * FT8RX_GRID_COLS, hipMemcpyHostToDevice));
    const int nf0 = f0_hi - f0_lo;
    launch_sync(h->d_grid, h->d_best_score, h->d_best_h0, c, B, h->stream, weak);
    HIPCHK(h, hipGetLastError());
    HIPCHK(h, hipMemcpy2DAsync(score, sizeof(float) * nf0, h->d_best_score, sizeof(float) * NF0MAX, sizeof(float) * nf0, B, hipMemcpyDeviceToHost, h->stream));
    HIPCHK(h, hipMemcpy2DAsync(h0_idx, sizeof(int32_t) * nf0, h->d_best_h0, sizeof(int32_t) * NF0MAX, sizeof(int32_t) * nf0, B, hipMemcpyDeviceToHost, h->stream));
    HIPCHK(h, hipStreamSynchronize(h->stream));
    return 0;
}

int ft8rx_sync_scores(ft8rx_handle* h, const float* grid, int B, int f0_lo, int f0_hi, float* score, int32_t* h0_idx) {
    return sync_scores(h, grid, B, f0_lo, f0_hi, score, h0_idx, false);
}
int ft8rx_sync_scores_weak(ft8rx_handle* h, const float* grid, int B, int f0_lo, int f0_hi, float* score, int32_t* h0_idx) {
    return sync_scores(h, grid, B, f0_lo, f0_hi, score, h0_idx, true);
}

static std::vector<int32_t> pack_triples(int n, const int32_t* frame, const int32_t* f0_idx, const int32_t* h0_idx) {
    std::vector<int32_t> trip(3 * (size_t)n);
    for (int i = 0; i < n; i++) { trip[3 * i] = frame[i]; trip[3 * i + 1] = f0_idx[i]; trip[3 * i + 2] = h0_idx[i]; }
    return trip;
}

int ft8rx_llr_grid(ft8rx_handle* h, const float* grid, int B, int n, const int32_t* frame, const int32_t* f0_idx,
                   const int32_t* h0_idx, float* llr, float* sd, int32_t* snr) {
    if (!h || !grid || B < 1 || B > h->max_frames || n < 1) return -1;
    ENTER(h);
    HIPCHK(h, hipMemcpy(h->d_grid, grid, sizeof(float) * (size_t)B * FT8RX_GRID_ROWS * FT8RX_GRID_COLS, hipMemcpyHostToDevice));
    const std::vector<int32_t> trip = pack_triples(n, frame, f0_idx, h0_idx);
    Scratch S{h};
    int32_t* d_trip = S.put(trip.data(), trip.size()); NEED(d_trip);
    float* d_llr = S.get<float>((size_t)n * 174); NEED(d_llr);
    float* d_sd = S.get<float>(n); NEED(d_sd);
    int32_t* d_snr = S.get<int32_t>(n); NEED(d_snr);
    k_grid_llr<<<n, 64, 0, h->stream>>>(h->d_grid, nullptr, nullptr, d_llr, h->cfg, d_trip, d_sd, d_snr, nullptr, nullptr, nullptr, n);
    HIPCHK(h, hipStreamSynchronize(h->stream));
    HIPCHK(h, hipMemcpy(llr, d_llr, sizeof(float) * (size_t)n * 174, hipMemcpyDeviceToHost));
    HIPCHK(h, hipMemcpy(sd, d_sd, sizeof(float) * n, hipMemcpyDeviceToHost));
    HIPCHK(h, hipMemcpy(snr, d_snr, sizeof(int32_t) * n, hipMemcpyDeviceToHost));
    return 0;
}

int ft8rx_cycle_spectrum(ft8rx_handle* h, const int16_t* audio, int B, float* spec) {
    if (!h || !audio || !spec || B < 1 || B > h->max_frames) return -1;
    ENTER(h);
    if (need_staging(h)) return -2;
    HIPCHK(h, hipMemcpy(h->d_audio, audio, sizeof(int16_t) * (size_t)B * FT8RX_NSAMP, hipMemcpyHostToDevice));
    k_cyc_a<<<dim3(40, B), 256, 0, h->stream>>>(h->d_audio, h->d_A, h->T);
    k_cyc_bc<<<dim3(CYC_BC_GRID, B), 256, 0, h->stream>>>(h->d_A, h->d_spec, h->T);
    HIPCHK(h, hipStreamSynchronize(h->stream));
    HIPCHK(h, hipMemcpy(spec, h->d_spec, sizeof(cpx) * (size_t)B * FT8RX_SPEC_BINS, hipMemcpyDeviceToHost));
    return 0;
}

static int fine_probe(ft8rx_handle* h, const float* spec, int B, int n, const int32_t* frame, const int32_t* f0_idx, const int32_t* h0_idx,
                      int32_t* ret, int32_t* ttweak, int32_t* ftweak, int32_t* nsync, float* llr, float* sd, int32_t* snr, float* sgrid, bool weak) {
    if (!h || !spec || B < 1 || B > h->max_frames || n < 1) return -1;
    if (weak) for (int i = 0; i < n; i++)
        if (frame[i] < 0 || frame[i] >= B || f0_idx[i] < 4 || f0_idx[i] >= FT8RX_MAX_F0 || h0_idx[i] < FT8RX_MIN_H0 || h0_idx[i] >= FT8RX_MAX_H0) {
            set_err(h, "ft8rx_fine_weak: triple %d (frame %d, f0 %d, h0 %d) outside [0, %d) x [4, %d) x [%d, %d)", i,
                    frame[i], f0_idx[i], h0_idx[i], B, FT8RX_MAX_F0, FT8RX_MIN_H0, FT8RX_MAX_H0); return -1; }
    ENTER(h);
    HIPCHK(h, hipMemcpy(h->d_spec, spec, sizeof(cpx) * (size_t)B * FT8RX_SPEC_BINS, hipMemcpyHostToDevice));
    const std::vector<int32_t> trip = pack_triples(n, frame, f0_idx, h0_idx);
    Scratch S{h};
    int32_t* d_trip = S.put(trip.data(), trip.size()); NEED(d_trip);
    float* d_llr = S.get<float>((size_t)n * 174); NEED(d_llr);
    HIPCHK(h, hipMemset(d_llr, 0, sizeof(float) * (size_t)n * 174));
    float* d_sd = S.get<float>(n); NEED(d_sd);
    int32_t* d_out = S.get<int32_t>((size_t)n * 5); NEED(d_out);
    float* d_sg = sgrid ? S.get<float>((size_t)n * 632) : nullptr; if (sgrid) NEED(d_sg);
    launch_fine(h, weak ? weak_config(h) : h->cfg, weak, n, h->stream, h->d_spec, nullptr, nullptr, d_llr, d_trip, d_out, d_sd, d_sg,
                WorkList{nullptr, nullptr}, true);
    HIPCHK(h, hipStreamSynchronize(h->stream));
    std::vector<int32_t> o((size_t)n * 5);
    HIPCHK(h, hipMemcpy(o.data(), d_out, sizeof(int32_t) * o.size(), hipMemcpyDeviceToHost));
    for (int i = 0; i < n; i++) { ret[i] = o[5 * i]; ttweak[i] = o[5 * i + 1]; ftweak[i] = o[5 * i + 2]; nsync[i] = o[5 * i + 3]; snr[i] = o[5 * i + 4]; }
    HIPCHK(h, hipMemcpy(llr, d_llr, sizeof(float) * (size_t)n * 174, hipMemcpyDeviceToHost));
    HIPCHK(h, hipMemcpy(sd, d_sd, sizeof(float) * n, hipMemcpyDeviceToHost));
    if (sgrid) HIPCHK(h, hipMemcpy(sgrid, d_sg, sizeof(float) * (size_t)n * 632, hipMemcpyDeviceToHost));
    return 0;
}

int ft8rx_fine(ft8rx_handle* h, const float* spec, int B, int n, const int32_t* frame, const int32_t* f0_idx, const int32_t* h0_idx,
               int32_t* ret, int32_t* ttweak, int32_t* ftweak, int32_t* nsync, float* llr, float* sd, int32_t* snr, float* sgrid) {
    return fine_probe(h, spec, B, n, frame, f0_idx, h0_idx, ret, ttweak, ftweak, nsync, llr, sd, snr, sgrid, false);
}
int ft8rx_fine_weak(ft8rx_handle* h, const float* spec, int B, int n, const int32_t* frame, const int32_t* f0_idx, const int32_t* h0_idx,
                    int32_t* ret, int32_t* ttweak, int32_t* ftweak, int32_t* nsync, float* llr, float* sd, int32_t* snr, float* sgrid) {
    return fine_probe(h, spec, B, n, frame, f0_idx, h0_idx, ret, ttweak, ftweak, nsync, llr, sd, snr, sgrid, true);
}

int ft8rx_ldpc(ft8rx_handle* h, const float* llr, int n, int max_ncheck0, int max_iters, int32_t* ok, uint64_t* msg_lo,
               uint64_t* msg_hi, int32_t* n_its, int32_t* has_out, float* llr_out) {
    if (!h || !llr || n < 1) return -1;
    ENTER(h);
    Scratch S{h};
    float* d_in = S.put(llr, (size_t)n * 174); NEED(d_in);
    float* d_out = S.get<float>((size_t)n * 174); NEED(d_out);
    HIPCHK(h, hipMemset(d_out, 0, sizeof(float) * (size_t)n * 174));
    Att* d_att = S.get<Att>(n); NEED(d_att);
    k_bp<<<n, 64, 0, h->stream>>>(2, d_in, nullptr, nullptr, nullptr, d_att, d_out, nullptr, nullptr, h->cfg, max_ncheck0, max_iters, WorkList{nullptr, nullptr}, 0, 1);
    HIPCHK(h, hipStreamSynchronize(h->stream));
    std::vector<Att> a(n);
    HIPCHK(h, hipMemcpy(a.data(), d_att, sizeof(Att) * n, hipMemcpyDeviceToHost));
    for (int i = 0; i < n; i++) { ok[i] = a[i].ok; msg_lo[i] = a[i].lo; msg_hi[i] = a[i].hi; n_its[i] = a[i].ok ? a[i].n_its : -1; has_out[i] = a[i].has_out; }
    if (llr_out) HIPCHK(h, hipMemcpy(llr_out, d_out, sizeof(float) * (size_t)n * 174, hipMemcpyDeviceToHost));
    return 0;
}

int ft8rx_ap_calls_probe(ft8rx_handle* h, const float* llr, int n, ft8rx_record* records, ft8rx_event* events, int32_t* event_count) {
    if (!h || !llr || !records || n < 1 || n > h->cfg.max_cands) { if (h) set_err(h, "ft8rx_ap_calls_probe: 1 <= n <= max_cands"); return -1; }
    if (!h->ap.np) { set_err(h, "ft8rx_ap_calls_probe: no call set (ft8rx_set_ap_calls)"); return -1; }
    ENTER(h);
    Scratch S{h};
    const size_t st = (size_t)1 << cand_shift(h->cfg);
    std::vector<ft8rx_record> r0(st);
    memset(r0.data(), 0, sizeof(ft8rx_record) * st);
    for (int i = 0; i < n; i++) r0[i].status = FT8RX_ST_EXHAUSTED;
    std::vector<float> l0(st * 174, 0.0f);
    memcpy(l0.data(), llr, sizeof(float) * (size_t)n * 174);
    const int32_t nc = n, zero = 0;
    float* d_llr = S.put(l0.data(), l0.size()); NEED(d_llr);
    ft8rx_record* d_rec = S.put(r0.data(), st); NEED(d_rec);
    int32_t* d_nc = S.put(&nc, 1); NEED(d_nc);
    int32_t* d_evc = S.put(&zero, 1); NEED(d_evc);
    Att* d_att = S.get<Att>(st * 10); NEED(d_att);
    ft8rx_event* d_ev = S.get<ft8rx_event>(FT8RX_EVENT_CAP); NEED(d_ev);
    int32_t* d_cl = S.get<int32_t>(st); NEED(d_cl);
    int32_t* d_ol = S.get<int32_t>(st * 3); NEED(d_ol);
    int32_t* d_ac = S.get<int32_t>(2); NEED(d_ac);
    ApCalls* d_apc = S.get<ApCalls>(1); NEED(d_apc);
    k_ap_stage<<<1, 64, 0, h->stream>>>(d_apc, h->ap);
    launch_ap_calls(h, 1, d_llr, d_rec, d_nc, d_att, d_ev, d_evc, d_cl, d_ol, d_ac, d_apc, h->stream);
    HIPCHK(h, hipStreamSynchronize(h->stream));
    HIPCHK(h, hipMemcpy(records, d_rec, sizeof(ft8rx_record) * (size_t)n, hipMemcpyDeviceToHost));
    int32_t ne = 0;
    HIPCHK(h, hipMemcpy(&ne, d_evc, sizeof(int32_t), hipMemcpyDeviceToHost));
    if (event_count) *event_count = ne;
    if (events) HIPCHK(h, hipMemcpy(events, d_ev, sizeof(ft8rx_event) * (size_t)(ne < FT8RX_EVENT_CAP ? ne : FT8RX_EVENT_CAP), hipMemcpyDeviceToHost));
    return 0;
}

int ft8rx_recall_probe(ft8rx_handle* h, const float* sgrid, const ft8rx_recall_entry* entries, int n, ft8rx_record* records) {
    if (!h || !sgrid || !entries || !records || n < 1) { if (h) set_err(h, "ft8rx_recall_probe: bad arguments"); return -1; }
    ENTER(h);
    Scratch S{h};
    std::vector<ft8rx_recall_entry> st((size_t)n * FT8RX_RECALL_MAX);
    std::vector<int32_t> trip(3 * (size_t)n), off(n + 1), tout(5 * (size_t)n, 0);
    for (int i = 0; i < n; i++) {
        ft8rx_recall_entry E = entries[i];
        E.pad = (uint16_t)recall_kind(E.msg_lo, E.msg_hi);
        st[(size_t)i * FT8RX_RECALL_MAX] = E;
        trip[3 * i] = i; trip[3 * i + 1] = E.f0_idx; trip[3 * i + 2] = E.h0_idx; off[i] = i;
    }
    off[n] = n;
    float* d_sg = S.put(sgrid, (size_t)n * 632); NEED(d_sg);
    ft8rx_recall_entry* d_ent = S.put(st.data(), st.size()); NEED(d_ent);
    int32_t* d_trip = S.put(trip.data(), trip.size()); NEED(d_trip);
    int32_t* d_off = S.put(off.data(), off.size()); NEED(d_off);
    int32_t* d_tout = S.put(tout.data(), tout.size()); NEED(d_tout);
    ft8rx_record* d_rec = S.get<ft8rx_record>((size_t)n * FT8RX_RECALL_MAX); NEED(d_rec);
    HIPCHK(h, hipMemset(d_rec, 0, sizeof(ft8rx_record) * (size_t)n * FT8RX_RECALL_MAX));
    k_recall_score<<<n, 64, 0, h->stream>>>(d_sg, d_tout, d_trip, d_off, 0, d_ent, nullptr, nullptr, 0, h->rc_max_hd, h->rc_min_gap, d_rec);
    HIPCHK(h, hipStreamSynchronize(h->stream));
    HIPCHK(h, hipMemcpy2D(records, sizeof(ft8rx_record), d_rec, sizeof(ft8rx_record) * FT8RX_RECALL_MAX, sizeof(ft8rx_record), n, hipMemcpyDeviceToHost));
    return 0;
}

int ft8rx_report_probe(ft8rx_handle* h, const float* spec, int B, int n, const int32_t* frame, const int32_t* f0_idx, const int32_t* h0_idx,
                       const int32_t* ttweak, const int32_t* ftweak, const uint64_t* msg_lo, const uint64_t* msg_hi, ft8rx_report* reports) {
    if (!h || !spec || !frame || !f0_idx || !h0_idx || !ttweak || !ftweak || !msg_lo || !msg_hi || !reports || B < 1 || B > h->max_frames || n < 1) {
        if (h) set_err(h, "ft8rx_report_probe: bad arguments (1 <= n_frames <= max_frames, n >= 1)"); return -1; }
    const int sh = cand_shift(h->cfg); const size_t S = (size_t)1 << sh;
    std::vector<ft8rx_record> r0((size_t)B * S);
    memset(r0.data(), 0, sizeof(ft8rx_record) * r0.size());
    std::vector<int32_t> nc(B, 0), where(n);
    for (int i = 0; i < n; i++) {
        if (frame[i] < 0 || frame[i] >= B || f0_idx[i] < -32768 || f0_idx[i] > 32767 || h0_idx[i] < -32768 || h0_idx[i] > 32767 ||
            ttweak[i] < -128 || ttweak[i] > 127 || ftweak[i] < -128 || ftweak[i] > 127) {
            set_err(h, "ft8rx_report_probe: candidate %d (frame %d, f0 %d, h0 %d, tweaks %d / %d) is out of range", i, frame[i], f0_idx[i], h0_idx[i], ttweak[i], ftweak[i]); return -1; }
        if (nc[frame[i]] >= (int)S) { set_err(h, "ft8rx_report_probe: more than %zu candidates in frame %d", S, frame[i]); return -1; }
        where[i] = (int32_t)((size_t)frame[i] * S + nc[frame[i]]++);
        ft8rx_record& r = r0[where[i]];
        r.msg_lo = msg_lo[i]; r.msg_hi = msg_hi[i]; r.f0_idx = (int16_t)f0_idx[i]; r.h0_idx = (int16_t)h0_idx[i];
        r.ttweak = (int8_t)ttweak[i]; r.ftweak = (int8_t)ftweak[i]; r.status = FT8RX_ST_DECODED;
    }
    ENTER(h);
    HIPCHK(h, hipMemcpy(h->d_spec, spec, sizeof(cpx) * (size_t)B * FT8RX_SPEC_BINS, hipMemcpyHostToDevice));
    Scratch Sc{h};
    ft8rx_record* d_rec = Sc.put(r0.data(), r0.size()); NEED(d_rec);
    int32_t* d_nc = Sc.put(nc.data(), nc.size()); NEED(d_nc);
    int32_t* d_items = Sc.get<int32_t>((size_t)B * S); NEED(d_items);
    int32_t* d_count = Sc.get<int32_t>(1); NEED(d_count);
    ft8rx_report* d_rep = Sc.get<ft8rx_report>((size_t)B * S); NEED(d_rep);
    launch_reports(h, B, h->d_spec, d_rec, d_nc, d_items, d_count, d_rep, h->stream);
    HIPCHK(h, hipGetLastError());
    HIPCHK(h, hipStreamSynchronize(h->stream));
    std::vector<ft8rx_report> out((size_t)B * S);
    HIPCHK(h, hipMemcpy(out.data(), d_rep, sizeof(ft8rx_report) * out.size(), hipMemcpyDeviceToHost));
    for (int i = 0; i < n; i++) reports[i] = out[where[i]];
    return 0;
}

int ft8rx_osd_ext(ft8rx_handle* h, const float* llr, int n, int singleflips, int doubleflips, int tripleflips, int max_hd,
                  int32_t* ok, uint64_t* msg_lo, uint64_t* msg_hi, int32_t* trial, int32_t* hd) {
    if (!h || !llr || n < 1) return -1;
    if (singleflips < 0 || singleflips > OSD_MAXFLIP || doubleflips < 0 || doubleflips > OSD_MAXFLIP || tripleflips < 0 || tripleflips > 40 ||
        max_hd < 0 || max_hd > 174) { set_err(h, "ft8rx_osd: flip counts out of range"); return -1; }
    const std::vector<uint32_t> tr = osd_trial_table(singleflips, doubleflips, tripleflips);
    if (tr.size() > OSD_MAXTRIALS) { set_err(h, "ft8rx_osd: %zu trials exceed %d", tr.size(), OSD_MAXTRIALS); return -1; }
    ENTER(h);
    Scratch S{h};
    float* d_in = S.put(llr, (size_t)n * 174); NEED(d_in);
    uint32_t* d_tr = S.put(tr.data(), tr.size()); NEED(d_tr);
    Att* d_att = S.get<Att>(n); NEED(d_att);
    int32_t* d_nan = S.get<int32_t>((size_t)n + 1); NEED(d_nan);
    HIPCHK(h, hipMemsetAsync(d_nan, 0, sizeof(int32_t), h->stream));
    const WorkList nanl{d_nan + 1, d_nan};
    launch_osd(0, n, h->stream, 2, d_in, nullptr, nullptr, nullptr, nullptr, d_att, nullptr, nullptr, d_tr, (int)tr.size(),
               osd_nflip(singleflips, tripleflips), max_hd, cand_shift(h->cfg), WorkList{nullptr, nullptr}, nanl);
    HIPCHK(h, hipStreamSynchronize(h->stream));
    std::vector<Att> a(n);
    HIPCHK(h, hipMemcpy(a.data(), d_att, sizeof(Att) * n, hipMemcpyDeviceToHost));
    for (int i = 0; i < n; i++) {
        ok[i] = a[i].ok; msg_lo[i] = a[i].lo; msg_hi[i] = a[i].hi; trial[i] = a[i].ok ? a[i].n_its : -1;
        if (hd) hd[i] = a[i].ok ? a[i].pad[0] : -1;
    }
    return 0;
}

int ft8rx_osd(ft8rx_handle* h, const float* llr, int n, int singleflips, int doubleflips, int32_t* ok, uint64_t* msg_lo,
              uint64_t* msg_hi, int32_t* trial) {
    return ft8rx_osd_ext(h, llr, n, singleflips, doubleflips, 0, 0, ok, msg_lo, msg_hi, trial, nullptr);
}

int ft8rx_crc_valid(ft8rx_handle* h, const float* cw91, int n, int32_t* res, uint64_t* msg_lo, uint64_t* msg_hi) {
    if (!h || !cw91 || n < 1) return -1;
    ENTER(h);
    Scratch S{h};
    float* d_in = S.put(cw91, (size_t)n * 91); NEED(d_in);
    int32_t* d_res = S.get<int32_t>(n); NEED(d_res);
    uint64_t* d_lo = S.get<uint64_t>(n); NEED(d_lo);
    uint64_t* d_hi = S.get<uint64_t>(n); NEED(d_hi);
    k_crc_probe<<<n, 64, 0, h->stream>>>(d_in, n, d_res, d_lo, d_hi);
    HIPCHK(h, hipStreamSynchronize(h->stream));
    HIPCHK(h, hipMemcpy(res, d_res, sizeof(int32_t) * n, hipMemcpyDeviceToHost));
    HIPCHK(h, hipMemcpy(msg_lo, d_lo, sizeof(uint64_t) * n, hipMemcpyDeviceToHost));
    HIPCHK(h, hipMemcpy(msg_hi, d_hi, sizeof(uint64_t) * n, hipMemcpyDeviceToHost));
    return 0;
}

int ft8rx_valid77(ft8rx_handle* h, const uint64_t* msg_lo, const uint64_t* msg_hi, int n, int32_t* valid) {
    if (!h || !msg_lo || !msg_hi || n < 1) return -1;
    ENTER(h);
    Scratch S{h};
    uint64_t* d_lo = S.put(msg_lo, n); NEED(d_lo);
    uint64_t* d_hi = S.put(msg_hi, n); NEED(d_hi);
    int32_t* d_v = S.get<int32_t>(n); NEED(d_v);
    k_valid_probe<<<(n + 255) / 256, 256, 0, h->stream>>>(d_lo, d_hi, n, d_v);
    HIPCHK(h, hipStreamSynchronize(h->stream));
    HIPCHK(h, hipMemcpy(valid, d_v, sizeof(int32_t) * n, hipMemcpyDeviceToHost));
    return 0;
}

int ft8rx_valid77_ext(ft8rx_handle* h, const uint64_t* msg_lo, const uint64_t* msg_hi, int n, int32_t mask, int32_t* valid) {
    if (!h || !msg_lo || !msg_hi || n < 1 || mask < 0 || mask > FT8RX_MT_ALL) return -1;
    ENTER(h);
    Scratch S{h};
    uint64_t* d_lo = S.put(msg_lo, n); NEED(d_lo);
    uint64_t* d_hi = S.put(msg_hi, n); NEED(d_hi);
    int32_t* d_v = S.get<int32_t>(n); NEED(d_v);
    k_valid_ext_probe<<<(n + 255) / 256, 256, 0, h->stream>>>(d_lo, d_hi, n, (unsigned)mask, d_v);
    HIPCHK(h, hipStreamSynchronize(h->stream));
    HIPCHK(h, hipMemcpy(valid, d_v, sizeof(int32_t) * n, hipMemcpyDeviceToHost));
    return 0;
}

int16_t* ft8rx_staging_audio(ft8rx_handle* h) {
    if (!h || hipSetDevice(h->device) != hipSuccess || need_staging(h)) return nullptr;
    return h->d_audio;
}

int ft8rx_d2h_async(ft8rx_handle* h, void* dst, const void* d_src, uint64_t bytes, int32_t* ticket) {
    if (!h || !dst || !d_src || !ticket) return -1;
    HIPCHK(h, hipSetDevice(h->device));
    const uint32_t id = h->d2h_next;
    hipEvent_t& e = h->d2h_ev[id & 31];
    if (!e) HIPCHK(h, hipEventCreateWithFlags(&e, hipEventDisableTiming));
    else if (id >= 32 && hipEventQuery(e) == hipErrorNotReady) HIPCHK(h, hipEventSynchronize(e));
    if (bytes) HIPCHK(h, hipMemcpyAsync(dst, d_src, (size_t)bytes, hipMemcpyDeviceToHost, h->copy_s));
    HIPCHK(h, hipEventRecord(e, h->copy_s));
    h->d2h_next = id + 1;
    *ticket = (int32_t)(id & 0x7fffffffu);
    return 0;
}
int ft8rx_d2h_query(ft8rx_handle* h, int32_t ticket) {
    if (!h || ticket < 0) return -1;
    const uint32_t id = (uint32_t)ticket, next = h->d2h_next & 0x7fffffffu;
    const uint32_t age = (next - id) & 0x7fffffffu;
    if (age == 0u || age > 0x40000000u) { set_err(h, "ft8rx_d2h_query: ticket %d was never issued", ticket); return -1; }
    if (age > 32u) return 1;
    const hipError_t r = hipEventQuery(h->d2h_ev[id & 31]);
    if (r == hipSuccess) return 1;
    if (r == hipErrorNotReady) return 0;
    set_err(h, "ft8rx_d2h_query: %s", hipGetErrorString(r));
    return -2;
}
void* ft8rx_d2h_event(ft8rx_handle* h, int32_t ticket) {
    if (!h || ticket < 0) return nullptr;
    const uint32_t id = (uint32_t)ticket, next = h->d2h_next & 0x7fffffffu;
    const uint32_t age = (next - id) & 0x7fffffffu;
    return (age >= 1u && age <= 32u) ? (void*)h->d2h_ev[id & 31] : nullptr;
}

int ft8rx_copy_to_host(ft8rx_handle* h, void* dst, const void* d_src, uint64_t bytes) {
    if (!h || !dst || !d_src) return -1;
    ENTER(h);
    HIPCHK(h, hipMemcpy(dst, d_src, (size_t)bytes, hipMemcpyDeviceToHost));
    return 0;
}

int ft8rx_subtract(ft8rx_handle* h, int16_t* d_audio, int B, ft8rx_subsig* sigs, const int32_t* counts, int max_sigs,
                   int refine, float* audio_f32_out) {
    if (!h || !d_audio || !sigs || !counts) return -1;
    if (B < 1 || B > h->max_frames || max_sigs < 1 || max_sigs > 256 || refine < 0 || refine > 3) { set_err(h, "ft8rx_subtract: bad n_frames / max_sigs / refine"); return -1; }
    ENTER(h);
    HIPCHK(h, hipStreamSynchronize(h->stream));
    if (!h->d_wf) {
        const size_t MB = (size_t)h->max_frames;
        int rc = dalloc(h, &h->d_wf, MB * FT8RX_NSAMP);
        rc |= dalloc(h, &h->d_part, MB * SUB_NCH * 20);
        rc |= dalloc(h, &h->d_pulse, (size_t)5760);
        rc |= dalloc(h, &h->d_pc, (size_t)5760);
        rc |= dalloc(h, &h->d_sigcnt, MB);
        if (rc) return -2;
        std::vector<double> pulse(5760), pc(5760);
        const double c = M_PI * sqrt(2.0 / log(2.0)), bt = 2.0;
        double acc = 0.0;
        for (int i = 0; i < 5760; i++) {
            const double tt = ((double)i - 1.5 * 1920.0) / 1920.0;
            pulse[i] = 0.5 * (erf(c * bt * (tt + 0.5)) - erf(c * bt * (tt - 0.5)));
            acc += pulse[i]; pc[i] = acc;
        }
        HIPCHK(h, hipMemcpy(h->d_pulse, pulse.data(), sizeof(double) * 5760, hipMemcpyHostToDevice));
        HIPCHK(h, hipMemcpy(h->d_pc, pc.data(), sizeof(double) * 5760, hipMemcpyHostToDevice));
    }
    if (h->sig_cap < max_sigs) {
        ft8rx_subsig* p = nullptr;
        if (dalloc(h, &p, (size_t)h->max_frames * max_sigs)) return -2;
        h->d_sigs = p; h->sig_cap = max_sigs;
    }
    int nmax = 0;
    for (int f = 0; f < B; f++) {
        if (counts[f] < 0 || counts[f] > max_sigs) { set_err(h, "ft8rx_subtract: counts[%d] = %d outside [0, %d]", f, counts[f], max_sigs); return -1; }
        if (counts[f] > nmax) nmax = counts[f];
    }
    HIPCHK(h, hipMemcpyAsync(h->d_sigs, sigs, sizeof(ft8rx_subsig) * (size_t)B * max_sigs, hipMemcpyHostToDevice, h->stream));
    HIPCHK(h, hipMemcpyAsync(h->d_sigcnt, counts, sizeof(int32_t) * B, hipMemcpyHostToDevice, h->stream));
    const size_t n = (size_t)B * FT8RX_NSAMP;
    k_sub_to_f32<<<(unsigned)((n + 255) / 256), 256, 0, h->stream>>>(d_audio, h->d_wf, n);
    const SubTables T{h->d_pulse, h->d_pc};
    SubShifts coarse, fine;
    coarse.stride = 1; fine.stride = 1;
    coarse.n = 16; for (int i = 0; i < 16; i++) coarse.shift[i] = -1680 + 120 * i;
    fine.n = 9;    for (int i = 0; i < 9; i++) fine.shift[i] = -120 + 30 * i;
    for (int i = 9; i < SUB_MAXSHIFT; i++) fine.shift[i] = 0;
    if (refine == 2 && !h->d_zdec) {
        const size_t MB = (size_t)h->max_frames;
        int rc = dalloc(h, &h->d_zdec, MB * SUBD_NZ);
        rc |= dalloc(h, &h->d_model, MB * SUBD_N);
        rc |= dalloc(h, &h->d_adec, MB * (SUBD_N + 1));
        rc |= dalloc(h, &h->d_subctx, MB);
        if (rc) return -2;
    }
    SubShifts dcoarse, dfine;
    dcoarse.stride = 1; dfine.stride = 1;
    dcoarse.n = 15; for (int i = 0; i < 15; i++) dcoarse.shift[i] = SUBD_D * (-52 + 4 * i);
    dcoarse.shift[15] = 0;
    dfine.n = 9;    for (int i = 0; i < 9; i++) dfine.shift[i] = SUBD_D * (-4 + i);
    for (int i = 9; i < SUB_MAXSHIFT; i++) dfine.shift[i] = 0;
    const dim3 gmodel((SUBD_N + 255) / 256, B);
    Tables Tones = h->T;
    if (refine == 3) {
        if (!h->d_ones) {
            if (dalloc(h, &h->d_ones, (size_t)100)) return -2;
            double ones[100]; for (int i = 0; i < 100; i++) ones[i] = 1.0;
            HIPCHK(h, hipMemcpy(h->d_ones, ones, sizeof(ones), hipMemcpyHostToDevice));
        }
        Tones.taper = h->d_ones;
    }
    for (int s = 0; s < nmax; s++) {
        if (refine == 3) {
            k_cyc_a_f32<<<dim3(40, B), 256, 0, h->stream>>>(h->d_wf, h->d_A, h->T);
            k_cyc_bc<<<dim3(CYC_BC_GRID, B), 256, 0, h->stream>>>(h->d_A, h->d_spec, h->T);
            k_refine3<<<B, FINE_NT, 0, h->stream>>>(h->d_spec, h->d_sigs, h->d_sigcnt, max_sigs, s, Tones);
            k_sub_accum<<<dim3(SUB_GRIDX, B), 256, 0, h->stream>>>(h->d_wf, h->d_sigs, h->d_sigcnt, max_sigs, s, T, h->d_part);
            k_sub_apply<<<dim3(SUB_GRIDX, B), 256, 0, h->stream>>>(h->d_wf, h->d_sigs, h->d_sigcnt, max_sigs, s, T, h->d_part);
            continue;
        }
        if (refine == 2) {
            k_subd_mix<<<dim3(SUBD_NZ / 256, B), 256, 0, h->stream>>>(h->d_wf, h->d_sigs, h->d_sigcnt, max_sigs, s, h->d_zdec, h->d_subctx);
            k_subd_model<<<gmodel, 256, 0, h->stream>>>(h->d_sigs, h->d_sigcnt, max_sigs, s, T, h->d_subctx, h->d_model);
            k_subd_scan<<<B, 256, 0, h->stream>>>(h->d_zdec, h->d_model, h->d_sigs, h->d_sigcnt, max_sigs, s, h->d_subctx, dcoarse, h->d_part);
            k_sub_pick<<<B, 256, 0, h->stream>>>(h->d_sigs, h->d_sigcnt, max_sigs, s, dcoarse, h->d_part, -1.0f, 0.0625f, 113, SUBD_D * SUBD_CH);
            k_subd_model<<<gmodel, 256, 0, h->stream>>>(h->d_sigs, h->d_sigcnt, max_sigs, s, T, h->d_subctx, h->d_model);
            k_subd_scan<<<B, 256, 0, h->stream>>>(h->d_zdec, h->d_model, h->d_sigs, h->d_sigcnt, max_sigs, s, h->d_subctx, dfine, h->d_part);
            k_sub_pick<<<B, 256, 0, h->stream>>>(h->d_sigs, h->d_sigcnt, max_sigs, s, dfine, h->d_part, 0.4375f, 0.015625f, 9, SUBD_D * SUBD_CH);
            k_subd_model<<<gmodel, 256, 0, h->stream>>>(h->d_sigs, h->d_sigcnt, max_sigs, s, T, h->d_subctx, h->d_model);
            k_subd_accum<<<B, 256, 0, h->stream>>>(h->d_zdec, h->d_model, h->d_sigs, h->d_sigcnt, max_sigs, s, h->d_subctx, h->d_adec);
            k_subd_apply<<<dim3(SUB_GRIDX, B), 256, 0, h->stream>>>(h->d_wf, h->d_sigs, h->d_sigcnt, max_sigs, s, T, h->d_adec);
            continue;
        }
        if (refine) {
            k_sub_scan<<<dim3(SUB_GRIDX, B), 256, 0, h->stream>>>(h->d_wf, h->d_sigs, h->d_sigcnt, max_sigs, s, T, coarse, h->d_part);
            k_sub_pick<<<B, 256, 0, h->stream>>>(h->d_sigs, h->d_sigcnt, max_sigs, s, coarse, h->d_part, -1.0f, 0.0625f, 113, SUB_CH);
            k_sub_scan<<<dim3(SUB_GRIDX, B), 256, 0, h->stream>>>(h->d_wf, h->d_sigs, h->d_sigcnt, max_sigs, s, T, fine, h->d_part);
            k_sub_pick<<<B, 256, 0, h->stream>>>(h->d_sigs, h->d_sigcnt, max_sigs, s, fine, h->d_part, 0.4375f, 0.015625f, 9, SUB_CH);
        }
        k_sub_accum<<<dim3(SUB_GRIDX, B), 256, 0, h->stream>>>(h->d_wf, h->d_sigs, h->d_sigcnt, max_sigs, s, T, h->d_part);
        k_sub_apply<<<dim3(SUB_GRIDX, B), 256, 0, h->stream>>>(h->d_wf, h->d_sigs, h->d_sigcnt, max_sigs, s, T, h->d_part);
    }
    k_sub_to_i16<<<(unsigned)((n + 255) / 256), 256, 0, h->stream>>>(h->d_wf, d_audio, n);
    HIPCHK(h, hipGetLastError());
    if (audio_f32_out) HIPCHK(h, hipMemcpyAsync(audio_f32_out, h->d_wf, sizeof(float) * n, hipMemcpyDeviceToHost, h->stream));
    if (refine) HIPCHK(h, hipMemcpyAsync(sigs, h->d_sigs, sizeof(ft8rx_subsig) * (size_t)B * max_sigs, hipMemcpyDeviceToHost, h->stream));
    HIPCHK(h, hipStreamSynchronize(h->stream));
    return 0;
}

int ft8rx_encode_tones(const uint64_t* msg_lo, const uint64_t* msg_hi, int n, uint8_t* tones) {
    if (!msg_lo || !msg_hi || !tones || n < 0) return -1;
    for (int i = 0; i < n; i++) hostmsg::encode_tones(msg_lo[i], msg_hi[i], tones + (size_t)i * 79);
    return 0;
}

void* ft8rx_alloc_host(ft8rx_handle* h, uint64_t bytes) {
    if (!h || bytes == 0) return nullptr;
    void* p = nullptr;
    if (hipSetDevice(h->device) != hipSuccess || hipHostMalloc(&p, (size_t)bytes, hipHostMallocDefault) != hipSuccess) {
        set_err(h, "ft8rx_alloc_host: hipHostMalloc(%llu) failed", (unsigned long long)bytes);
        return nullptr;
    }
    return p;
}

int ft8rx_free_host(ft8rx_handle* h, void* p) {
    if (!p) return -1;
    const hipError_t e = hipHostFree(p);
    if (e != hipSuccess) { if (h) set_err(h, "hipHostFree failed: %s", hipGetErrorString(e)); return -2; }
    return 0;
}

int ft8rx_synth_frames_ex(ft8rx_handle* h, uint64_t seed, int first_index, int n_frames, int n_signals,
                          const void* signal_table, int signal_bytes, const double* pulse_cumsum, int16_t* d_audio, int no_noise) {
    if (!h || !signal_table || !pulse_cumsum || !d_audio || n_frames < 1 || n_signals < 0 || n_signals > 64) return -1;
    if (signal_bytes != (int)sizeof(SynthSig)) { set_err(h, "ft8rx_synth_frames: signal record is %d bytes, expected %d", signal_bytes, (int)sizeof(SynthSig)); return -1; }
    ENTER(h);
    Scratch S{h};
    SynthSig* d_s = S.put((const SynthSig*)signal_table, (size_t)n_frames * (n_signals ? n_signals : 1)); NEED(d_s);
    double* d_q = S.put(pulse_cumsum, 5761); NEED(d_q);
    k_synth<<<dim3((FT8RX_NSAMP / 4 + 255) / 256, n_frames), 256, 0, h->stream>>>(d_audio, d_s, n_signals, d_q, (uint32_t)seed, (uint32_t)(seed >> 32), first_index, no_noise);
    HIPCHK(h, hipStreamSynchronize(h->stream));
    return 0;
}

int ft8rx_synth_frames(ft8rx_handle* h, uint64_t seed, int first_index, int n_frames, int n_signals,
                       const void* signal_table, int signal_bytes, const double* pulse_cumsum, int16_t* d_audio) {
    return ft8rx_synth_frames_ex(h, seed, first_index, n_frames, n_signals, signal_table, signal_bytes, pulse_cumsum, d_audio, 0);
}

int ft8rx_package_batch(const ft8rx_record* records, const int32_t* counts, const ft8rx_event* events, const int32_t* event_counts,
                        int n_frames, int max_cands, ft8rx_message* out, int max_msgs, int32_t* out_counts, int n_threads,
                        ft8rx_hashes* table, int32_t* flags) {
    return hostmsg::package_batch(records, counts, events, event_counts, n_frames, max_cands, out, max_msgs, out_counts, n_threads,
                                  table ? &table->H : nullptr, flags);
}

int ft8rx_package_batch_ext(const ft8rx_record* records, const int32_t* counts, const ft8rx_event* events, const int32_t* event_counts,
                            int n_frames, int max_cands, ft8rx_message_ext* out, int max_msgs, int32_t* out_counts, int n_threads,
                            ft8rx_hashes* table, int32_t* flags, int32_t mask) {
    if (mask < 0 || mask > FT8RX_MT_ALL) return -1;
    return hostmsg::package_batch(records, counts, events, event_counts, n_frames, max_cands, out, max_msgs, out_counts, n_threads,
                                  table ? &table->H : nullptr, flags, (unsigned)mask);
}

int ft8rx_package_batch_recall(const ft8rx_record* records, const int32_t* counts, const ft8rx_event* events, const int32_t* event_counts,
                               const ft8rx_record* recall, const int32_t* recall_counts, int n_frames, int max_cands, ft8rx_message* out,
                               int max_msgs, int32_t* out_counts, int n_threads, ft8rx_hashes* table, int32_t* flags) {
    if (!recall || !recall_counts) return -1;
    return hostmsg::package_batch(records, counts, events, event_counts, n_frames, max_cands, out, max_msgs, out_counts, n_threads,
                                  table ? &table->H : nullptr, flags, 0u, recall, recall_counts);
}

int ft8rx_package_packed(const void* packed, uint64_t bytes, int frame_lo, int n_frames, ft8rx_message* out, int max_msgs,
                         int32_t* out_counts, int n_threads, ft8rx_hashes* table, int32_t* flags) {
    return hostmsg::package_packed(packed, bytes, frame_lo, n_frames, out, max_msgs, out_counts, n_threads, table ? &table->H : nullptr, flags);
}

int ft8rx_merge_messages(ft8rx_message* out, int32_t* out_counts, int max_out, const ft8rx_message* add, const int32_t* add_counts,
                         int max_add, int n_frames, int pass_tag, int drop_osd, ft8rx_message* fresh, int32_t* fresh_counts) {
    if (!out || !out_counts || !add || !add_counts || n_frames < 0 || max_out < 1 || max_add < 1) return -1;
    hostmsg::merge_messages(out, out_counts, max_out, add, add_counts, max_add, n_frames, pass_tag, drop_osd, fresh, fresh_counts);
    return 0;
}

int ft8rx_subtraction_list(const ft8rx_message* msgs, const int32_t* counts, int max_msgs, const ft8rx_record* records, int max_cands,
                           int n_frames, int min_snr, ft8rx_subsig* sigs, int max_sigs, int32_t* sig_counts) {
    if (!msgs || !counts || !records || !sigs || !sig_counts || n_frames < 0 || max_msgs < 1 || max_cands < 1 || max_sigs < 1) return -1;
    return hostmsg::subtraction_list(msgs, counts, max_msgs, records, max_cands, n_frames, min_snr, sigs, max_sigs, sig_counts);
}

ft8rx_hashes* ft8rx_hashes_create(void) { return new (std::nothrow) ft8rx_hashes(); }
void ft8rx_hashes_destroy(ft8rx_hashes* t) { delete t; }
int ft8rx_hashes_clear(ft8rx_hashes* t) { if (!t) return -1; t->H.clear(); return 0; }
int ft8rx_hashes_add(ft8rx_hashes* t, const char* call) { if (!t || !call) return -1; t->H.add(call); return 0; }
int ft8rx_hashes_size(const ft8rx_hashes* t) { return t ? (int)t->H.size() : -1; }

int ft8rx_set_reject_log(const char* path) { hostmsg::set_reject_log(path); return 0; }

#ifdef FINE_TIMING
int ft8rx_debug_fine_times(ft8rx_handle* h, unsigned long long* out32, int reset) {
    if (!h) return -1;
    ENTER(h);
    return ft8rx_ilp_fine_times(out32, reset);
}
#endif

#ifdef BP_TIMING
int ft8rx_debug_bp_times(ft8rx_handle* h, unsigned long long* out8, int reset) {
    if (!h) return -1;
    ENTER(h);
    if (hipDeviceSynchronize() != hipSuccess) return -2;
    std::vector<unsigned long long> all((size_t)65536 * 8);
    if (out8) {
        if (hipMemcpyFromSymbol(all.data(), HIP_SYMBOL(g_bp_t), sizeof(unsigned long long) * all.size()) != hipSuccess) return -2;
        for (int i = 0; i < 8; i++) out8[i] = 0;
        for (size_t b = 0; b < 65536; b++) for (int i = 0; i < 8; i++) out8[i] += all[b * 8 + i];
    }
    if (reset) { std::fill(all.begin(), all.end(), 0ull); if (hipMemcpyToSymbol(HIP_SYMBOL(g_bp_t), all.data(), sizeof(unsigned long long) * all.size()) != hipSuccess) return -2; }
    return 0;
}
#endif
#ifdef OSD_TIMING
int ft8rx_debug_osd_times(ft8rx_handle* h, unsigned long long* out16, int reset) {
    if (!h) return -1;
    ENTER(h);
    if (hipDeviceSynchronize() != hipSuccess) return -2;
    std::vector<unsigned long long> all((size_t)32768 * 10);
    if (out16) {
        if (hipMemcpyFromSymbol(all.data(), HIP_SYMBOL(g_osd_t), sizeof(unsigned long long) * all.size()) != hipSuccess) return -2;
        for (int i = 0; i < 16; i++) out16[i] = 0;
        for (size_t b = 0; b < 32768; b++) for (int i = 0; i < 10; i++) out16[i == 9 ? 15 : i] += all[b * 10 + i];
    }
    if (reset) { std::fill(all.begin(), all.end(), 0ull); if (hipMemcpyToSymbol(HIP_SYMBOL(g_osd_t), all.data(), sizeof(unsigned long long) * all.size()) != hipSuccess) return -2; }
    return 0;
}
#endif

int ft8rx_math_probe(ft8rx_handle* h, int which, const float* x, int n, float* y) {
    if (!h || !x || !y || n < 1) return -1;
    ENTER(h);
    Scratch S{h};
    if (which == 0 || which == 1) {
        float* d_x = S.put(x, n); NEED(d_x);
        float* d_y = S.get<float>(n); NEED(d_y);
        k_math_probe<<<(n + 255) / 256, 256, 0, h->stream>>>(which, d_x, d_y, n);
        HIPCHK(h, hipStreamSynchronize(h->stream));
        HIPCHK(h, hipMemcpy(y, d_y, sizeof(float) * n, hipMemcpyDeviceToHost));
        return 0;
    }
    if (which == 2) {
        cpx* d_x = S.put((const cpx*)x, n); NEED(d_x);
        cpx* d_y = S.get<cpx>(n); NEED(d_y);
        const size_t lds = 2 * (size_t)n * sizeof(cpx);
        if (n == 1920) k_fft_probe<1920, 8, 4, 4, 5, 3><<<1, 256, lds, h->stream>>>(d_x, d_y, h->T.W1920);
        else if (n == 3200) k_fft_probe<3200, 8, 4, 4, 5, 5><<<1, 256, lds, h->stream>>>(d_x, d_y, h->T.W3200);
        else if (n == 300) k_fft_probe<300, 5, 5, 4, 3><<<1, 256, lds, h->stream>>>(d_x, d_y, h->T.W300);
        else if (n == 320) k_fft_probe<320, 8, 8, 5><<<1, 256, lds, h->stream>>>(d_x, d_y, h->T.W320);
        else { set_err(h, "ft8rx_math_probe: no FFT plan of length %d", n); return -1; }
        HIPCHK(h, hipStreamSynchronize(h->stream));
        HIPCHK(h, hipMemcpy(y, d_y, sizeof(cpx) * n, hipMemcpyDeviceToHost));
        return 0;
    }
    return -1;
}

}
```

pyft8_amd/csrc/kernels/ap_calls.hpp:

```cpp
#ifndef FT8RX_AP_CALLS_HPP
#define FT8RX_AP_CALLS_HPP

__global__ void k_ap_stage(ApCalls* dst, ApCalls a) {
    if (threadIdx.x == 0) *dst = a;
}

__global__ void k_ap_worklist(const ft8rx_record* rec, const int32_t* ncand, int B, int sh, WorkList next) {
    const int c = blockIdx.x * blockDim.x + threadIdx.x;
    const bool on = cand_live(c, B, sh, ncand) && rec[c].status == FT8RX_ST_EXHAUSTED;
    work_push_block(next, on, c);
}

FT8_DEV void ap_codeword_test(int lane, int c, int p, const float* __restrict__ llr0, Att* __restrict__ att7, ft8rx_event* ev,
                              int32_t* evcount, int sh, const ApCalls* __restrict__ a) {
    const float* src = llr0 + (size_t)c * 174;
    const int k = p - FT8RX_AP_FIRST;
    const uint64_t h0 = __ballot(src[lane] > 0.0f), h1 = __ballot(src[64 + lane] > 0.0f), h2 = __ballot(lane < 46 && src[128 + (lane < 46 ? lane : 0)] > 0.0f);
    const int hd = __popcll(h0 ^ a->val[k][0]) + __popcll(h1 ^ a->val[k][1]) + __popcll(h2 ^ a->val[k][2]);
    if (lane != 0) return;
    Att r; memset(&r, 0, sizeof(r)); r.n_its = 0;
    if (hd <= a->max_hd) {
        r.ok = 1; r.lo = a->lo[k]; r.hi = a->hi[k]; r.method = FT8RX_M_AP_CODEWORD; r.pad[0] = (uint8_t)hd;
        log_event(ev, evcount, c >> sh, c & ((1 << sh) - 1), 7, 2 * p, 0, r.lo, r.hi, 1);
    }
    att7[(size_t)c * 10 + k] = r;
}

__global__ __launch_bounds__(64, BP_WV) void k_bp_ap(const float* __restrict__ llr0, ft8rx_record* __restrict__ rec, const int32_t* __restrict__ ncand,
                                                     Att* __restrict__ att7, ft8rx_event* ev, int32_t* evcount, ft8rx_config cfg,
                                                     const ApCalls* __restrict__ apc, WorkList cands, WorkList osdl) {
    const int np = apc->np, n = *cands.count * np;
    _Pragma("unroll 1")
    for (int item = blockIdx.x; item < n; item += gridDim.x) {
        int tid = threadIdx.x;
        asm volatile("" : "+v"(tid));
        const int c = cands.items[item / np], p = apc->pat[item % np];
        if (p >= 8) ap_codeword_test(tid, c, p, llr0, att7, ev, evcount, cand_shift(cfg), apc);
        else bp_attempt<false, true>(tid, 1, (c << 4) | p, llr0, rec, ncand, nullptr, att7, nullptr, ev, evcount, cfg,
                                     cfg.bp_nc0_b, cfg.bp_iters_b, 0u, apc, &osdl);
        __syncthreads();
    }
}

#define OSD_AP_KERNEL(NAME, WIDE)                                                                                                   \
__global__ __launch_bounds__(64) OSD_ATTR void NAME(const float* __restrict__ llr0, ft8rx_record* __restrict__ rec,                \
                                                    const int32_t* __restrict__ ncand, Att* __restrict__ att7, ft8rx_event* ev,     \
                                                    int32_t* evcount, const uint32_t* __restrict__ trials, int ntr, int nflip,      \
                                                    int sh, const ApCalls* __restrict__ apc, WorkList work) {                       \
    const OsdArgs a = {llr0, nullptr, nullptr, rec, ncand, att7, ev, evcount, trials, ntr, nflip, 0, sh, {nullptr, nullptr}, 0u, apc}; \
    osd_blocks<WIDE, false, false, true>(*work.count, 0, a, [&](int item) { return work.items[item]; });                            \
}
OSD_AP_KERNEL(k_osd_ap, false)
OSD_AP_KERNEL(k_osd_ap_wide, true)
#undef OSD_AP_KERNEL

__global__ void k_select_ap(ft8rx_record* rec, const Att* att7, const ApCalls* __restrict__ apc, WorkList cands) {
    const int i = blockIdx.x * blockDim.x + threadIdx.x;
    if (i >= *cands.count) return;
    const int c = cands.items[i], np = apc->np;
    int best = -1, bhd = 1 << 30;
    for (int k = 0; k < np; k++) {
        const int p = apc->pat[k];
        const Att& a = att7[(size_t)c * 10 + (p - FT8RX_AP_FIRST)];
        if (a.ok && (int)a.pad[0] < bhd) { best = p; bhd = a.pad[0]; }
    }
    if (best < 0) return;
    const Att& a = att7[(size_t)c * 10 + (best - FT8RX_AP_FIRST)];
    ft8rx_record& r = rec[c];
    r.status = FT8RX_ST_DECODED; r.ipass = 7; r.ap = (uint8_t)best; r.method = a.method; r.n_its = a.n_its;
    r.msg_lo = a.lo; r.msg_hi = a.hi; r.osd_hd = (uint8_t)bhd;
}

#endif
```

pyft8_amd/csrc/kernels/bp.hpp:

```cpp
#ifndef FT8RX_BP_HPP
#define FT8RX_BP_HPP

#ifndef BP_WV
#define BP_WV 7
#endif
#ifdef BP_TIMING
__device__ unsigned long long g_bp_t[65536][8];
#define BT_DECL unsigned long long bt_prev = __builtin_readcyclecounter();
#define BT(i) do { const unsigned long long bt_now = __builtin_readcyclecounter(); if (lane == 0) atomicAdd(&g_bp_t[blockIdx.x & 65535][i], bt_now - bt_prev); bt_prev = __builtin_readcyclecounter(); } while (0)
#else
#define BT_DECL
#define BT(i) do { } while (0)
#endif
template <bool EXT, bool AP7 = false>
FT8_DEV void bp_attempt(int lane, int mode, int bid, const float* __restrict__ llr_in, ft8rx_record* __restrict__ rec,
                        const int32_t* __restrict__ ncand, Att* __restrict__ attG, Att* __restrict__ attB,
                        float* __restrict__ saved, ft8rx_event* ev, int32_t* evcount, const ft8rx_config& cfg,
                        int max_nc0, int max_iters, unsigned mt, const ApCalls* __restrict__ apc = nullptr, const WorkList* osdl = nullptr) {
    __shared__ float llr[176];
    __shared__ float tl[576];
    float* dl = tl;
    __shared__ float P[84];
    int ap = 0; size_t vec;
    BT_DECL
    uint64_t ho0 = 0, ho1 = 0, ho2 = 0;
    if (AP7) { ap = bid & 15; vec = (size_t)(bid >> 4); }
    else if (mode == 2) vec = bid;
    else {
        const int sh = cand_shift(cfg);
        ap = bid % 5; const int c = bid / 5;
        if ((c & ((1 << sh) - 1)) >= ncand[c >> sh]) return;
        if (rec[c].status != FT8RX_ST_ACTIVE) return;
        vec = (size_t)c;
    }
    {
        const float* src = llr_in + vec * 174;
        const float v0 = src[lane], v1 = src[64 + lane], v2 = src[128 + (lane < 46 ? lane : 0)];
        if constexpr (AP7) {
            llr[lane] = ap7_value(apc, ap, lane, v0); llr[64 + lane] = ap7_value(apc, ap, 64 + lane, v1);
            if (lane < 46) llr[128 + lane] = ap7_value(apc, ap, 128 + lane, v2);
            ho0 = __ballot(v0 > 0.0f); ho1 = __ballot(v1 > 0.0f); ho2 = __ballot(lane < 46 && v2 > 0.0f);
        } else {
            llr[lane] = ap_value(ap, lane, v0); llr[64 + lane] = ap_value(ap, 64 + lane, v1);
            if (lane < 46) llr[128 + lane] = ap_value(ap, 128 + lane, v2);
        }
    }
    if (lane < 2) llr[174 + lane] = 0.0f;
    if (lane == 0) P[83] = 1.0f;
    __syncthreads();
    Att res; memset(&res, 0, sizeof(res)); res.n_its = -1;
    if (!AP7 && mode == 1 && ap == 0) {
        bool any = false;
#pragma unroll
        for (int g = 0; g < 2; g++) {
            Att resG; memset(&resG, 0, sizeof(resG)); resG.n_its = -1;
            const uint64_t b0 = __ballot(ap_value(g, lane, llr[lane]) > 0.0f);
            const uint64_t b1 = __ballot(lane < 27 && ap_value(g, 64 + lane, llr[64 + (lane < 27 ? lane : 0)]) > 0.0f);
            uint64_t lo, hi;
            const int r = ft8_crc_check_wave<EXT>(b0, b1, lane, &lo, &hi, mt);
            if (r) { if (lane == 0) log_event(ev, evcount, (int)vec >> cand_shift(cfg), (int)vec & ((1 << cand_shift(cfg)) - 1), 2, g, 0, lo, hi, r == 2); }
            if (r == 2) { resG.ok = 1; resG.lo = lo; resG.hi = hi; resG.n_its = 0; resG.method = FT8RX_M_GOOD91; any = true; }
            if (lane == 0) attG[vec * 2 + g] = resG;
        }
        if (any) return;
    }
    const int c0 = lane, c1 = lane + 64;
    const uint64_t cm00 = d_CHK_MASK[c0][0], cm01 = d_CHK_MASK[c0][1], cm02 = d_CHK_MASK[c0][2];
    const uint64_t cm10 = d_CHK_MASK[c1][0], cm11 = d_CHK_MASK[c1][1], cm12 = d_CHK_MASK[c1][2];
    int ev_[9], ec_[9];
    uint32_t ve_[3] = {0u, 0u, 0u};
    int n0 = 0, n1 = 0;
    bool tables = false;
    float mc[9];
#pragma unroll
    for (int i = 0; i < 9; i++) mc[i] = 0.0f;
    res.has_out = 1;
    BT(0);
    for (int it = 0; it < max_iters; it++) {
        const uint64_t h0 = __ballot(llr[lane] > 0.0f), h1 = __ballot(llr[64 + lane] > 0.0f),
                       h2 = __ballot(lane < 46 && llr[128 + (lane < 46 ? lane : 0)] > 0.0f);
        const int par0 = (__popcll(h0 & cm00) + __popcll(h1 & cm01) + __popcll(h2 & cm02)) & 1;
        const int par1 = (__popcll(h0 & cm10) + __popcll(h1 & cm11) + __popcll(h2 & cm12)) & 1;
        int ncheck = __popcll(__ballot(par0)) + __popcll(__ballot(par1));
        if (it == 0) { res.nc0 = (uint8_t)ncheck; if (ncheck > max_nc0) { res.has_out = 0; break; } }
        if (ncheck == 0) {
            uint64_t b0 = h0;
            uint64_t b1 = h1 & ((1ull << 27) - 1);
            uint64_t lo, hi;
            int r = ft8_crc_check_wave<EXT>(b0, b1, lane, &lo, &hi, mt);
            if constexpr (AP7) {
                if (r && lane == 0) log_event(ev, evcount, (int)vec >> cand_shift(cfg), (int)vec & ((1 << cand_shift(cfg)) - 1), 7, 2 * ap, it + 1, lo, hi, r == 2);
                const int hd = __popcll(h0 ^ ho0) + __popcll(h1 ^ ho1) + __popcll(h2 ^ ho2);
                res.pad[1] = (uint8_t)(r == 2);
                if (r == 2 && hd <= apc->max_hd) { res.ok = 1; res.lo = lo; res.hi = hi; res.n_its = (int16_t)it; res.pad[0] = (uint8_t)hd; }
                res.has_out = 0;
                break;
            }
            if (r) {
                int ipass = (mode == 0) ? 0 : ((ap < 2 && res.nc0 <= cfg.bp_nc0_a && it < cfg.bp_iters_a) ? 3 : 4);
                if (lane == 0) log_event(ev, evcount, (int)vec >> cand_shift(cfg), (int)vec & ((1 << cand_shift(cfg)) - 1), ipass, ap, it + 1, lo, hi, r == 2);
            }
            if (r == 2) { res.ok = 1; res.lo = lo; res.hi = hi; res.n_its = (int16_t)it; res.has_out = 0; }
            break;
        }
        BT(1);
        if (!tables) {
            tables = true;
#pragma unroll
            for (int i = 0; i < 9; i++) { int e = lane + 64 * i; ev_[i] = (e < 522) ? d_EDGE_V[e] : 174; ec_[i] = (e < 522) ? d_EDGE_C[e] : 83; }
            n0 = d_CHK_N[c0];
            n1 = (c1 < 83) ? d_CHK_N[c1] : 0;
#pragma unroll
            for (int q = 0; q < 3; q++) {
                const int v = lane + 64 * q, vc = v < 174 ? v : 0;
                ve_[q] = (uint32_t)d_VAR_E[vc][0] | ((uint32_t)d_VAR_E[vc][1] << 10) | ((uint32_t)d_VAR_E[vc][2] << 20);
            }
        }
#pragma unroll
        for (int i = 0; i < 9; i++) {
            const int e = lane + 64 * i;
            const float v2c = llr[ev_[i]] - mc[i];
            tl[e] = ft8_tanhf(-v2c);
        }
        BT(2);
        __syncthreads();
        {
            float Pp = tl[c0];
#pragma unroll
            for (int j = 1; j < 6; j++) Pp = Pp * tl[c0 + 83 * j];
            if (n0 == 7) Pp = Pp * tl[439 + c0];
            P[c0] = Pp;
            if (c1 < 83) {
                float Q = tl[c1];
#pragma unroll
                for (int j = 1; j < 6; j++) Q = Q * tl[c1 + 83 * j];
                if (n1 == 7) Q = Q * tl[439 + c1];
                P[c1] = Q;
            }
        }
        BT(3);
        __syncthreads();
#pragma unroll
        for (int i = 0; i < 9; i++) {
            const int e = lane + 64 * i;
            const float tti = tl[e];
            const float Pc = P[ec_[i]];
            const float nm = (Pc * tti) / (__builtin_fmaf(-1.18f, tti, Pc) * __builtin_fmaf(1.18f, tti, Pc));
            dl[e] = nm - mc[i];
            mc[i] = nm;
        }
        BT(4);
        __syncthreads();
#pragma unroll
        for (int q = 0; q < 3; q++) {
            const int v = lane + 64 * q;
            if (v < 174) {
                float col = 0.0f;
                col += dl[ve_[q] & 1023u]; col += dl[(ve_[q] >> 10) & 1023u]; col += dl[ve_[q] >> 20];
                llr[v] += col;
            }
        }
        __syncthreads();
        BT(5);
    }
    BT(6);
    if constexpr (AP7) {
        if (res.ok) res.method = FT8RX_M_LDPC_B;
        if (lane == 0) { attB[vec * 10 + (ap - 5)] = res; if (!res.pad[1]) work_push(*osdl, bid); }
        return;
    }
    if (res.ok) res.method = (mode == 0) ? FT8RX_M_LDPC_A : FT8RX_M_LDPC_B;
    if (mode == 2) {
        if (lane == 0) attB[vec] = res;
        if (res.has_out) for (int i = lane; i < 174; i += 64) saved[vec * 174 + i] = llr[i];
        return;
    }
    if (mode == 0) { if (lane == 0) attB[vec * 5 + ap] = res; return; }
    if (lane == 0) attB[vec * 5 + ap] = res;
#ifndef BP_TIMING_NO_SAVED
    if (res.has_out) for (int i = lane; i < 174; i += 64) saved[(vec * 5 + ap) * 174 + i] = llr[i];
#endif
}

#define BP_KERNEL(NAME, EXT, MT_PARAM, MT)                                                                                                                       \
__global__ __launch_bounds__(64, BP_WV) void NAME(int mode, const float* __restrict__ llr_in, ft8rx_record* __restrict__ rec,                         \
                                           const int32_t* __restrict__ ncand, Att* __restrict__ attG, Att* __restrict__ attB,                         \
                                           float* __restrict__ saved, ft8rx_event* ev, int32_t* evcount, ft8rx_config cfg,                            \
                                           int max_nc0, int max_iters, WorkList work, int ap_lo, int ap_n MT_PARAM) {                                      \
    if (mode == 2) { bp_attempt<EXT>(threadIdx.x, 2, blockIdx.x, llr_in, rec, ncand, attG, attB, saved, ev, evcount, cfg, max_nc0, max_iters, MT); return; }\
                    \
                       \
                         \
    if (mode == 0) {                                                                                                                                  \
        const int n = *work.count;                                                                                                                    \
_Pragma("unroll 1")                                                                                                                                   \
        for (int item = blockIdx.x; item < n; item += gridDim.x) {                                                                                    \
            int tid = threadIdx.x;                                                                                                                    \
            asm volatile("" : "+v"(tid));                           \
            bp_attempt<EXT>(tid, 0, work.items[item], llr_in, rec, ncand, attG, attB, saved, ev, evcount, cfg, max_nc0, max_iters, MT);                   \
            __syncthreads();                                                                       \
        }                                                                                                                                             \
        return;                                                                                                                                       \
    }                                                                                                                                                 \
                    \
                \
    const int item = blockIdx.x;                                                                                                                      \
    if (item >= *work.count * ap_n) return;                                                                                                           \
    bp_attempt<EXT>(threadIdx.x, mode, work.items[item / ap_n] * 5 + ap_lo + item % ap_n, llr_in, rec, ncand, attG, attB, saved, ev, evcount, cfg, max_nc0, max_iters, MT);\
}
#define BP_MT_PARAM , unsigned mt
BP_KERNEL(k_bp, false, , 0u)
BP_KERNEL(k_bp_ext, true, BP_MT_PARAM, mt)
#undef BP_MT_PARAM
#undef BP_KERNEL

__global__ void k_select0(ft8rx_record* rec, const int32_t* ncand, const Att* att0, int B, int sh, WorkList next) {
    int c = blockIdx.x * blockDim.x + threadIdx.x;
    bool go_on = false;
    if (cand_live(c, B, sh, ncand)) {
        ft8rx_record& r = rec[c];
        if (r.status == FT8RX_ST_ACTIVE) {
            go_on = true;
            for (int ap = 0; ap < 5; ap++) {
                const Att& a = att0[(size_t)c * 5 + ap];
                if (a.ok) { r.status = FT8RX_ST_DECODED; r.ipass = 0; r.ap = (uint8_t)ap; r.method = a.method; r.n_its = a.n_its; r.msg_lo = a.lo; r.msg_hi = a.hi; go_on = false; break; }
            }
        }
    }
    work_push_block(next, go_on, c);
}

__global__ void k_worklist(const ft8rx_record* rec, const int32_t* ncand, int B, int sh, WorkList next) {
    int c = blockIdx.x * blockDim.x + threadIdx.x;
    const bool on = cand_live(c, B, sh, ncand) && rec[c].status == FT8RX_ST_ACTIVE;
    work_push_block(next, on, c);
}

__global__ void k_worklist_att(const ft8rx_record* rec, const int32_t* ncand, const Att* att0, int B, int sh, WorkList next) {
    const int i = blockIdx.x * blockDim.x + threadIdx.x, c = i / 5;
    const bool on = cand_live(c, B, sh, ncand) && rec[c].status == FT8RX_ST_ACTIVE && att0[i].pad[1] != 0;
    work_push_block(next, on, i);
}

FT8_DEV bool sel_take(ft8rx_record& r, const Att& a, int ipass, int ap, int method) {
    r.status = FT8RX_ST_DECODED; r.ipass = (uint8_t)ipass; r.ap = (uint8_t)ap; r.method = (uint8_t)method; r.n_its = a.n_its; r.msg_lo = a.lo; r.msg_hi = a.hi;
    return false;
}
__global__ void k_select1(int step, ft8rx_record* rec, const int32_t* ncand, const Att* attG, const Att* attB, int B, ft8rx_config cfg, WorkList next) {
    int c = blockIdx.x * blockDim.x + threadIdx.x;
    bool go_on = false;
    if (cand_live(c, B, cand_shift(cfg), ncand) && rec[c].status == FT8RX_ST_ACTIVE) {
        ft8rx_record& r = rec[c];
        go_on = true;
        const Att* b = attB + (size_t)c * 5;
#define IS_A(a) ((a).ok && (a).nc0 <= cfg.bp_nc0_a && (a).n_its < cfg.bp_iters_a)
        if (step == 0) {
            const Att& g0 = attG[(size_t)c * 2], & g1 = attG[(size_t)c * 2 + 1];
            if (g0.ok) go_on = sel_take(r, g0, 2, 0, FT8RX_M_GOOD91);
            else if (g1.ok) go_on = sel_take(r, g1, 2, 1, FT8RX_M_GOOD91);
            else if (IS_A(b[0])) go_on = sel_take(r, b[0], 3, 0, FT8RX_M_LDPC_A);
        } else if (step == 1) {
            if (IS_A(b[1])) go_on = sel_take(r, b[1], 3, 1, FT8RX_M_LDPC_A);
            else if (b[0].ok) go_on = sel_take(r, b[0], 4, 0, FT8RX_M_LDPC_B);
            else if (b[1].ok) go_on = sel_take(r, b[1], 4, 1, FT8RX_M_LDPC_B);
        } else if (step == 2) {
            for (int ap = 2; ap < 5 && go_on; ap++) if (b[ap].ok) go_on = sel_take(r, b[ap], 4, ap, FT8RX_M_LDPC_B);
        } else {
            const Att& g0 = attG[(size_t)c * 2], & g1 = attG[(size_t)c * 2 + 1];
            if (g0.ok) go_on = sel_take(r, g0, 2, 0, FT8RX_M_GOOD91);
            else if (g1.ok) go_on = sel_take(r, g1, 2, 1, FT8RX_M_GOOD91);
            else if (IS_A(b[0])) go_on = sel_take(r, b[0], 3, 0, FT8RX_M_LDPC_A);
            else if (IS_A(b[1])) go_on = sel_take(r, b[1], 3, 1, FT8RX_M_LDPC_A);
            else for (int ap = 0; ap < 5 && go_on; ap++) if (b[ap].ok) go_on = sel_take(r, b[ap], 4, ap, FT8RX_M_LDPC_B);
        }
#undef IS_A
    }
    work_push_block(next, go_on, c);
}

__global__ void k_select2(ft8rx_record* rec, const int32_t* ncand, const Att* attO, int B, int sh) {
    int c = blockIdx.x * blockDim.x + threadIdx.x;
    if (!cand_live(c, B, sh, ncand)) return;
    ft8rx_record& r = rec[c];
    if (r.status != FT8RX_ST_ACTIVE) return;
    for (int s = 0; s < 10; s++) {
        const Att& a = attO[(size_t)c * 10 + s];
        if (a.ok) {
            r.status = FT8RX_ST_DECODED; r.ipass = (s < 5) ? 5 : 6; r.ap = (uint8_t)(s % 5);
            r.method = (s < 5) ? FT8RX_M_OSD : FT8RX_M_LDPC_B_OSD; r.n_its = a.n_its; r.msg_lo = a.lo; r.msg_hi = a.hi; r.osd_hd = a.pad[0]; return; }
    }
    r.status = FT8RX_ST_EXHAUSTED;
}

#endif
```

pyft8_amd/csrc/kernels/common.hpp:

```cpp
#ifndef FT8RX_COMMON_HPP
#define FT8RX_COMMON_HPP

struct Tables {
    const float* win;
    const cpx* W1920;
    const cpx* WR3840;
    const cpx* W3200;
    const cpx* W96000;
    const cpx* W300;
    const cpx* W320;
    const cpx* WR192k;
    const cpx* W32;
    const double* taper;
    const float* K32;
    const cpx* CS100;
    const cpx* TW100;
    const cpx* G1000;
};

__device__ __constant__ int d_COSTAS[7] = {3, 1, 4, 0, 6, 5, 2};
__device__ __constant__ uint8_t d_PAYSYM[58] = {7,8,9,10,11,12,13,14,15,16,17,18,19,20,21,22,23,24,25,26,27,28,29,30,31,32,33,34,35,
    43,44,45,46,47,48,49,50,51,52,53,54,55,56,57,58,59,60,61,62,63,64,65,66,67,68,69,70,71};
struct WorkList { int32_t* items; int32_t* count; };

constexpr __host__ __device__ int cand_shift(int max_cands) { return max_cands <= 256 ? 8 : max_cands <= 512 ? 9 : max_cands <= 1024 ? 10 : 11; }
constexpr __host__ __device__ int cand_shift(const ft8rx_config& c) { return cand_shift(c.max_cands); }
FT8_DEV bool cand_live(int c, int B, int sh, const int32_t* ncand) { return c < (B << sh) && (c & ((1 << sh) - 1)) < ncand[c >> sh]; }

FT8_DEV bool xcd_frame_map(int L, int per, int B, int& frame, int& idx) {
    const int x = L & 7, j = L >> 3;
    frame = 8 * (j / per) + x; idx = j % per;
    return frame < B;
}
#define XCD_GRID(B, per) ((((B) + 7) / 8) * 8 * (per))
enum { WL_BP0 = 0, WL_FINE = 1, WL_BP1 = 2, WL_BP1B = 3, WL_BP1C = 4, WL_OSD = 5, WL_OSDNAN = 6, WL_N = 7 };

#define W6 ((double)(-0.16666667163372040f))

#ifndef FT8RX_ILP_UNIT
__device__ __constant__ int8_t d_AP_CQ[29]   = {0,0,0,0,0, 0,0,0,0,0, 0,0,0,0,0, 0,0,0,0,0, 0,0,0,0,0, 0,1,0,0};
__device__ __constant__ int8_t d_AP_END[3][19] = {{0,1, 1,1,1,1,1, 0,0,1,1,1, 0,1,0,1,0, 0,1},
                                                  {0,1, 1,1,1,1,1, 0,1,0,0,1, 0,1,0,0,0, 0,1},
                                                  {0,1, 1,1,1,1,1, 0,1,0,0,1, 0,0,1,0,0, 0,1}};
__device__ uint8_t  d_CHK_N[83];
__device__ int16_t  d_CHK_V[83][7];
__device__ uint8_t  d_EDGE_V[522];
__device__ uint8_t  d_EDGE_C[522];
__device__ uint16_t d_VAR_E[174][3];
__device__ uint64_t d_G0[91][3];
__device__ uint64_t d_CHK_MASK[128][3];

struct Att {
    uint64_t lo, hi;
    int16_t n_its;
    uint8_t ok;
    uint8_t method;
    uint8_t nc0;
    uint8_t has_out;
    uint8_t pad[2];
};

FT8_DEV void work_push(const WorkList& w, int cand) { if (w.items) w.items[atomicAdd(w.count, 1)] = cand; }
FT8_DEV void work_push_block(const WorkList& w, bool want, int cand) {
    __shared__ int s_wave[4], s_base;
    const int lane = threadIdx.x & 63, wv = threadIdx.x >> 6;
    const uint64_t m = __ballot(want);
    if (lane == 0) s_wave[wv] = __popcll(m);
    __syncthreads();
    if (threadIdx.x == 0) {
        const int tot = s_wave[0] + s_wave[1] + s_wave[2] + s_wave[3];
        s_base = tot ? atomicAdd(w.count, tot) : 0;
    }
    __syncthreads();
    if (want) {
        int off = s_base + __popcll(m & ((1ull << lane) - 1));
        for (int i = 0; i < wv; i++) off += s_wave[i];
        w.items[off] = cand;
    }
}
FT8_DEV float grid_at(const float* __restrict__ g, int row, int col) {
    row %= 750; if (row < 0) row += 750;
    const bool in = row >= 1 && row <= 375;
    const uint32_t raw = __float_as_uint(g[(in ? row : 1) * FT8RX_GRID_COLS + col]);
    const uint32_t m = in ? 0xFFFFFFFFu : 0u;
    return __uint_as_float((raw & m) | (0x3F800000u & ~m));
}

FT8_DEV void log_event(ft8rx_event* ev, int32_t* evcount, int frame, int cand, int ipass, int slot, int seq,
                       uint64_t lo, uint64_t hi, int valid) {
    if (!ev) return;
    int idx = atomicAdd(&evcount[frame], 1);
    if (idx < FT8RX_EVENT_CAP) {
        ft8rx_event e; e.msg_lo = lo; e.msg_hi = hi; e.cand = (uint16_t)cand; e.ipass = (uint8_t)ipass;
        e.slot = (uint8_t)slot; e.seq = (uint16_t)seq; e.valid = (uint16_t)valid;
        ev[(size_t)frame * FT8RX_EVENT_CAP + idx] = e;
    }
}

__global__ __launch_bounds__(1024) void k_ev_scan(const int32_t* __restrict__ evcount, int B, int32_t* __restrict__ offs) {
    __shared__ int s_wave[16];
    __shared__ int s_carry;
    const int tid = threadIdx.x, lane = tid & 63, wv = tid >> 6;
    if (tid == 0) s_carry = 0;
    __syncthreads();
    for (int base = 0; base < B; base += 1024) {
        const int f = base + tid;
        int c = f < B ? evcount[f] : 0;
        c = c > FT8RX_EVENT_CAP ? FT8RX_EVENT_CAP : (c < 0 ? 0 : c);
        int incl = c;
#pragma unroll
        for (int d = 1; d < 64; d <<= 1) { const int t = __shfl_up(incl, d); if (lane >= d) incl += t; }
        if (lane == 63) s_wave[wv] = incl;
        __syncthreads();
        int before = s_carry;
        for (int i = 0; i < wv; i++) before += s_wave[i];
        if (f < B) offs[f] = before + incl - c;
        __syncthreads();
        if (tid == 1023) s_carry = before + incl;
        __syncthreads();
    }
    if (tid == 0) offs[B] = s_carry;
}
__global__ __launch_bounds__(64) void k_ev_compact(const ft8rx_event* __restrict__ ev, const int32_t* __restrict__ evcount,
                                                   const int32_t* __restrict__ offs, ft8rx_event* __restrict__ out) {
    const int f = blockIdx.x;
    int c = evcount[f]; c = c > FT8RX_EVENT_CAP ? FT8RX_EVENT_CAP : c;
    const uint32_t* src = reinterpret_cast<const uint32_t*>(ev + (size_t)f * FT8RX_EVENT_CAP);
    uint32_t* dst = reinterpret_cast<uint32_t*>(out + offs[f]);
    for (int i = threadIdx.x; i < c * 6; i += 64) dst[i] = src[i];
}

static_assert(sizeof(ft8rx_record) == 48 && sizeof(ft8rx_event) == 24 && sizeof(ft8rx_packed_frame) == 16 &&
              sizeof(ft8rx_packed_header) == 32, "packed result layout");
__global__ __launch_bounds__(256) void k_pack_count(const ft8rx_record* __restrict__ rec, const int32_t* __restrict__ ncand,
                                                    const ft8rx_event* __restrict__ ev, const int32_t* __restrict__ evcount,
                                                    uint64_t* __restrict__ need , int32_t* __restrict__ nrec , int sh) {
    __shared__ uint32_t s_has[FT8RX_MAX_CANDS / 32];
    __shared__ int s_cnt[FT8RX_MAX_CANDS / 64], s_nan;
    const int f = blockIdx.x, tid = threadIdx.x, lane = tid & 63, S = 1 << sh, nw = S >> 6;
    for (int i = tid; i < S / 32; i += 256) s_has[i] = 0;
    if (tid == 0) s_nan = 0;
    __syncthreads();
    int c = evcount[f]; c = c > FT8RX_EVENT_CAP ? FT8RX_EVENT_CAP : (c < 0 ? 0 : c);
    for (int i = tid; i < c; i += 256) {
        const unsigned cand = ev[(size_t)f * FT8RX_EVENT_CAP + i].cand;
        if (cand < (unsigned)S) atomicOr(&s_has[cand >> 5], 1u << (cand & 31));
    }
    int n = ncand[f]; n = n > S ? S : (n < 0 ? 0 : n);
    for (int i = tid; i < n; i += 256) {
        const ft8rx_record& r = rec[((size_t)f << sh) + i];
        if (r.grid_sd != r.grid_sd || r.fine_sd != r.fine_sd) s_nan = 1;
    }
    __syncthreads();
#pragma unroll 1
    for (int q = 0; q < S / 256; q++) {
        const int i = tid + 256 * q;
        const bool decoded = i < n && rec[((size_t)f << sh) + (i < n ? i : 0)].status == FT8RX_ST_DECODED;
        const bool want = i < n && (decoded || ((s_has[i >> 5] >> (i & 31)) & 1u) || s_nan);
        const uint64_t m = __ballot(want);
        if (lane == 0) { need[(size_t)f * nw + (i >> 6)] = m; s_cnt[i >> 6] = __popcll(m); }
    }
    __syncthreads();
    if (tid == 0) { int t = 0; for (int w = 0; w < nw; w++) t += s_cnt[w]; nrec[f] = t; }
}
__global__ __launch_bounds__(1024) void k_pack_scan(const int32_t* __restrict__ nrec, const int32_t* __restrict__ ncand,
                                                    const int32_t* __restrict__ evcount, int B, int max_cands, unsigned long long cap_bytes,
                                                    unsigned char* __restrict__ buf, ft8rx_packed_header* __restrict__ hdr_host) {
    __shared__ int s_wr[16], s_we[16];
    __shared__ int s_cr, s_ce;
    const int tid = threadIdx.x, lane = tid & 63, wv = tid >> 6;
    ft8rx_packed_frame* table = reinterpret_cast<ft8rx_packed_frame*>(buf + sizeof(ft8rx_packed_header));
    const bool table_fits = sizeof(ft8rx_packed_header) + (size_t)B * sizeof(ft8rx_packed_frame) <= cap_bytes;
    if (tid == 0) { s_cr = 0; s_ce = 0; }
    __syncthreads();
    for (int base = 0; base < B; base += 1024) {
        const int f = base + tid;
        const int r = f < B ? nrec[f] : 0;
        const int eraw = f < B ? evcount[f] : 0;
        const int e = eraw > FT8RX_EVENT_CAP ? FT8RX_EVENT_CAP : (eraw < 0 ? 0 : eraw);
        int ir = r, ie = e;
#pragma unroll
        for (int d = 1; d < 64; d <<= 1) { const int tr = __shfl_up(ir, d), te = __shfl_up(ie, d); if (lane >= d) { ir += tr; ie += te; } }
        if (lane == 63) { s_wr[wv] = ir; s_we[wv] = ie; }
        __syncthreads();
        int br = s_cr, be = s_ce;
        for (int i = 0; i < wv; i++) { br += s_wr[i]; be += s_we[i]; }
        if (f < B && table_fits) {
            ft8rx_packed_frame t;
            t.rec_off = br + ir - r; t.ev_off = be + ie - e;
            int n = ncand[f]; n = n > max_cands ? max_cands : (n < 0 ? 0 : n);
            t.n_cand = (uint16_t)n; t.n_rec = (uint16_t)r; t.n_ev = eraw < 0 ? 0 : eraw;
            table[f] = t;
        }
        __syncthreads();
        if (tid == 1023) { s_cr = br + ir; s_ce = be + ie; }
        __syncthreads();
    }
    if (tid == 0) {
        ft8rx_packed_header hd;
        hd.magic = FT8RX_PACKED_MAGIC; hd.n_frames = B; hd.n_records = s_cr; hd.n_events = s_ce; hd.max_cands = max_cands;
        hd.bytes = sizeof(ft8rx_packed_header) + (unsigned long long)B * sizeof(ft8rx_packed_frame) +
                   (unsigned long long)s_cr * sizeof(ft8rx_record) + (unsigned long long)s_ce * sizeof(ft8rx_event);
        hd.overflow = hd.bytes > cap_bytes;
        if (cap_bytes >= sizeof(hd)) *reinterpret_cast<ft8rx_packed_header*>(buf) = hd;
        *hdr_host = hd;
    }
}
__global__ __launch_bounds__(256) void k_pack_write(const ft8rx_record* __restrict__ rec, const ft8rx_event* __restrict__ ev,
                                                    const uint64_t* __restrict__ need, int B, unsigned char* __restrict__ buf, int sh) {
    const ft8rx_packed_header hd = *reinterpret_cast<const ft8rx_packed_header*>(buf);
    if (hd.overflow) return;
    __shared__ int s_pre[FT8RX_MAX_CANDS / 64];
    const int f = blockIdx.x, tid = threadIdx.x, lane = tid & 63, S = 1 << sh, nw = S >> 6;
    const ft8rx_packed_frame t = reinterpret_cast<const ft8rx_packed_frame*>(buf + sizeof(ft8rx_packed_header))[f];
    unsigned char* recs = buf + sizeof(ft8rx_packed_header) + (size_t)B * sizeof(ft8rx_packed_frame);
    unsigned char* evs = recs + (size_t)hd.n_records * sizeof(ft8rx_record);
    if (tid == 0) { int a = 0; for (int w = 0; w < nw; w++) { s_pre[w] = a; a += __popcll(need[(size_t)f * nw + w]); } }
    __syncthreads();
#pragma unroll 1
    for (int q = 0; q < S / 256; q++) {
        const int i = tid + 256 * q;
        const uint64_t mine = need[(size_t)f * nw + (i >> 6)];
        if ((mine >> lane) & 1ull) {
            const int p = s_pre[i >> 6] + __popcll(mine & ((1ull << lane) - 1));
            const uint4* src = reinterpret_cast<const uint4*>(rec + ((size_t)f << sh) + i);
            uint4* dst = reinterpret_cast<uint4*>(recs + ((size_t)t.rec_off + p) * sizeof(ft8rx_record));
            uint4 a = src[0], b = src[1], c = src[2];
            c.w = (uint32_t)i;
            dst[0] = a; dst[1] = b; dst[2] = c;
        }
    }
    const int ne = t.n_ev > FT8RX_EVENT_CAP ? FT8RX_EVENT_CAP : t.n_ev;
    const uint2* es = reinterpret_cast<const uint2*>(ev + (size_t)f * FT8RX_EVENT_CAP);
    uint2* ed = reinterpret_cast<uint2*>(evs + (size_t)t.ev_off * sizeof(ft8rx_event));
    for (int i = tid; i < ne * 3; i += 256) ed[i] = es[i];
}
#endif

#endif
```

pyft8_amd/csrc/kernels/llr.hpp:

```cpp
#ifndef FT8RX_LLR_HPP
#define FT8RX_LLR_HPP

FT8_DEV void llr_from_p(const float* p, float* llr, float* sq, int lane, bool active, float* sd_out, int* snr_out) {
    float sd = 0.0f; int snr = 0;
    if (active) {
        float pmax = -__builtin_inff(), pmin = __builtin_inff();
        for (int i = lane; i < 464; i += 64) { float v = p[i]; if (v > pmax) pmax = v; if (v < pmin) pmin = v; }
        for (int o = 32; o > 0; o >>= 1) {
            float a = __shfl_xor(pmax, o), b = __shfl_xor(pmin, o);
            if (a > pmax) pmax = a;
            if (b < pmin) pmin = b;
        }
        float d = (pmax - pmin) - 58.0f;
        snr = (int)d; if (snr < -24) snr = -24; if (snr > 24) snr = 24;
        if (lane < 58) {
            const float* q = p + 8 * lane;
            float q0 = q[0], q1 = q[1], q2 = q[2], q3 = q[3], q4 = q[4], q5 = q[5], q6 = q[6], q7 = q[7];
#define MAX4(a, b, c, d) ({ float _m = (a); if ((b) > _m) _m = (b); if ((c) > _m) _m = (c); if ((d) > _m) _m = (d); _m; })
            float la = MAX4(q4, q5, q6, q7) - MAX4(q0, q1, q2, q3);
            float lb = MAX4(q2, q3, q4, q7) - MAX4(q0, q1, q5, q6);
            float lc = MAX4(q1, q2, q6, q7) - MAX4(q0, q3, q4, q5);
#undef MAX4
            llr[3 * lane] = la; llr[3 * lane + 1] = lb; llr[3 * lane + 2] = lc;
            sq[3 * lane] = la * la; sq[3 * lane + 1] = lb * lb; sq[3 * lane + 2] = lc * lc;
        }
    }
    __syncthreads();
    if (active) {
        const float* arr = (lane & 16) ? sq : llr;
        const int j = lane & 7, half = (lane >> 3) & 1;
        const int base = half ? 80 : 0, nblk = half ? 88 : 80;
        float r = arr[base + j];
        for (int i = 8; i < nblk; i += 8) r += arr[base + i + j];
        r = r + __shfl_xor(r, 1);
        r = r + __shfl_xor(r, 2);
        r = r + __shfl_xor(r, 4);
        if (half) for (int i = 88; i < 94; i++) r += arr[80 + i];
        float tot_l = __shfl(r, 0) + __shfl(r, 8);
        float tot_s = __shfl(r, 16) + __shfl(r, 24);
        float mean = tot_l / 174.0f;
        float var = tot_s / 174.0f - mean * mean;
        sd = sqrtf(var);
    }
    __syncthreads();
    if (active) for (int i = lane; i < 174; i += 64) llr[i] = (2.83f * llr[i]) / sd;
    __syncthreads();
    *sd_out = sd; *snr_out = snr;
}

#ifndef FT8RX_ILP_UNIT
FT8_DEV float ap_value(int ap, int i, float v) {
    if (ap == 1) {
        if (i < 29) return d_AP_CQ[i] ? 5.0f : -5.0f;
        if (i == 74 || i == 75 || i == 57 || i == 58) return -5.0f;
        if (i == 76) return 5.0f;
    } else if (ap >= 2) {
        if (i >= 58 && i < 77) return d_AP_END[ap - 2][i - 58] ? 5.0f : -5.0f;
    }
    return v;
}

struct ChkMasks { uint64_t m[6]; };
FT8_DEV ChkMasks chk_masks(int lane) {
    ChkMasks c;
    c.m[0] = d_CHK_MASK[lane][0]; c.m[1] = d_CHK_MASK[lane][1]; c.m[2] = d_CHK_MASK[lane][2];
    c.m[3] = d_CHK_MASK[lane + 64][0]; c.m[4] = d_CHK_MASK[lane + 64][1]; c.m[5] = d_CHK_MASK[lane + 64][2];
    return c;
}
template <bool EXT>
FT8_DEV void bp0_precheck(int lane, const float* llr , const ChkMasks& cm, int frame, int ci,
                          Att* __restrict__ att , ft8rx_event* ev, int32_t* evcount, int max_nc0, int max_iters,
                          unsigned msg_types) {
    const float v0 = llr[lane], v1 = llr[64 + lane], v2 = llr[128 + (lane < 46 ? lane : 0)];
    const uint64_t m27 = (1ull << 27) - 1;
    uint64_t h0[5], h1[5];
    int nchk[5];
#pragma unroll
    for (int ap = 0; ap < 5; ap++) {
        h0[ap] = __ballot(ap_value(ap, lane, v0) > 0.0f); h1[ap] = __ballot(ap_value(ap, 64 + lane, v1) > 0.0f);
        const uint64_t h2 = __ballot(lane < 46 && ap_value(ap, 128 + lane, v2) > 0.0f);
        const int par0 = (__popcll(h0[ap] & cm.m[0]) + __popcll(h1[ap] & cm.m[1]) + __popcll(h2 & cm.m[2])) & 1;
        const int par1 = (__popcll(h0[ap] & cm.m[3]) + __popcll(h1[ap] & cm.m[4]) + __popcll(h2 & cm.m[5])) & 1;
        nchk[ap] = __popcll(__ballot(par0)) + __popcll(__ballot(par1));
    }
    const int g = lane >> 4;
    const uint64_t w0 = g == 0 ? h0[0] : g == 1 ? h0[1] : g == 2 ? h0[2] : h0[3];
    const uint64_t w1 = g == 0 ? h1[0] : g == 1 ? h1[1] : g == 2 ? h1[2] : h1[3];
    const unsigned t = ft8_xor_row16(ft8_crc_entry(w0, w1 & m27, lane) | (ft8_crc_entry(h0[4], h1[4] & m27, lane) << 16));
    const unsigned syn_lo = (unsigned)__builtin_amdgcn_ds_bpermute((lane & 3) << 6, (int)t) & 0xFFFFu;
    const unsigned syn4 = (unsigned)__builtin_amdgcn_readfirstlane((int)t) >> 16;
    int r = 0;
    uint64_t lo = 0, hi = 0;
    int myn = 0;
    if (lane < 5) {
        const unsigned syn = lane < 4 ? syn_lo : syn4;
        const uint64_t my0 = lane == 0 ? h0[0] : lane == 1 ? h0[1] : lane == 2 ? h0[2] : lane == 3 ? h0[3] : h0[4];
        const uint64_t my1 = lane == 0 ? h1[0] : lane == 1 ? h1[1] : lane == 2 ? h1[2] : lane == 3 ? h1[3] : h1[4];
        myn = lane == 0 ? nchk[0] : lane == 1 ? nchk[1] : lane == 2 ? nchk[2] : lane == 3 ? nchk[3] : nchk[4];
        if (syn == 0) r = ft8_crc_check<EXT>(my0, my1 & m27, &lo, &hi, msg_types);
    }
    const uint64_t okm = __ballot(r == 2);
    const int first = okm ? __builtin_ctzll(okm) : 5;
    if (lane < 5) {
        Att a; memset(&a, 0, sizeof(a)); a.n_its = -1;
        if (lane <= first) {
            if (r) log_event(ev, evcount, frame, ci, 0, lane, 0, lo, hi, r == 2);
            if (r == 2) { a.ok = 1; a.lo = lo; a.hi = hi; a.n_its = 0; a.method = FT8RX_M_GOOD91; }
            else if (max_iters > 0 && myn > max_nc0) a.nc0 = (uint8_t)myn;
            else a.pad[1] = 1;
        }
        att[lane] = a;
    }
}

template <bool EXT>
FT8_DEV void k_grid_llr_body(const float* __restrict__ grid, ft8rx_record* __restrict__ rec,
                             const int32_t* __restrict__ ncand, float* __restrict__ llr0,
                             const ft8rx_config& cfg, const int32_t* __restrict__ trip, float* __restrict__ t_sd,
                             int32_t* __restrict__ t_snr, Att* __restrict__ att0, ft8rx_event* ev,
                             int32_t* evcount, int B, unsigned mt) {
    __shared__ float p[464];
    __shared__ float llr[174];
    __shared__ float sq[174];
    const int lane = threadIdx.x;
    int frame, ci, f0, h0;
    size_t slot = blockIdx.x;
    if (trip) { frame = trip[3 * blockIdx.x]; f0 = trip[3 * blockIdx.x + 1]; h0 = trip[3 * blockIdx.x + 2]; ci = 0; }
    else {
        if (!xcd_frame_map(blockIdx.x, cfg.max_cands, B, frame, ci)) return;
        slot = ((size_t)frame << cand_shift(cfg)) + ci;
        if (ci >= ncand[frame]) return;
        const ft8rx_record& r = rec[slot];
        f0 = r.f0_idx; h0 = r.h0_idx;
    }
    ChkMasks cm;
    if (att0) cm = chk_masks(lane);
    const float* g = grid + (size_t)frame * FT8RX_GRID_ROWS * FT8RX_GRID_COLS;
    {
        float v[8];
#pragma unroll
        for (int q = 0; q < 8; q++) {
            const int i = lane + 64 * q, ic = i < 464 ? i : 0;
            v[q] = grid_at(g, h0 + 4 + 4 * (int)d_PAYSYM[ic >> 3], f0 + 1 + 2 * (ic & 7));
        }
#pragma unroll
        for (int q = 0; q < 8; q++) if (lane + 64 * q < 464) p[lane + 64 * q] = v[q];
    }
    __syncthreads();
    float sd; int snr;
    llr_from_p(p, llr, sq, lane, true, &sd, &snr);
    float* out = llr0 + slot * 174;
    for (int i = lane; i < 174; i += 64) out[i] = llr[i];
    if (lane == 0) {
        if (trip) { t_sd[blockIdx.x] = sd; t_snr[blockIdx.x] = snr; }
        else {
            ft8rx_record& r = rec[slot];
            r.grid_sd = sd; r.snr_grid = (int8_t)snr;
            if (sd <= cfg.llr_sd_min) r.status = FT8RX_ST_STOP_GRID_SD;
        }
    }
    if (att0 && !(sd <= cfg.llr_sd_min))
        bp0_precheck<EXT>(lane, llr, cm, frame, ci, att0 + slot * 5, ev, evcount, cfg.bp_nc0_a, cfg.bp_iters_a, mt);
}
#define GRID_LLR_KERNEL(NAME, EXT, MT_PARAM, MT)                                                                                               \
__global__ __launch_bounds__(64) void NAME(const float* __restrict__ grid, ft8rx_record* __restrict__ rec,                          \
                                           const int32_t* __restrict__ ncand, float* __restrict__ llr0,                            \
                                           ft8rx_config cfg, const int32_t* __restrict__ trip, float* __restrict__ t_sd,           \
                                           int32_t* __restrict__ t_snr, Att* __restrict__ att0, ft8rx_event* ev,                   \
                                           int32_t* evcount, int B MT_PARAM) {                                                    \
    k_grid_llr_body<EXT>(grid, rec, ncand, llr0, cfg, trip, t_sd, t_snr, att0, ev, evcount, B, MT);                                 \
}
#define GRID_LLR_MT_PARAM , unsigned mt
GRID_LLR_KERNEL(k_grid_llr, false, , 0u)
GRID_LLR_KERNEL(k_grid_llr_ext, true, GRID_LLR_MT_PARAM, mt)
#undef GRID_LLR_MT_PARAM
#undef GRID_LLR_KERNEL
#endif

#endif
```

Measured before the change: 88710.

## Run AP variants sequentially per block with early exit in BP fine ladder

Fine BP now runs several AP variants in sequence inside one block and stops early once an earlier variant decodes, replacing a separate launch, select pass and worklist. AP forcing is turned into constexpr bitmasks that are applied in registers, so the lookups in constant memory go away. Edge tables are packed and preloaded, and the early status and ncand checks are dropped from bp_attempt. The cost is less parallelism per launch, because work that used to be spread across blocks is now serialised within one block, and the selection semantics change.

```diff
diff --git a/pyft8_amd/csrc/ft8rx.hip b/pyft8_amd/csrc/ft8rx.hip
--- a/pyft8_amd/csrc/ft8rx.hip
+++ b/pyft8_amd/csrc/ft8rx.hip
@@ -576,7 +576,7 @@
     launch_mt(k_grid_llr, k_grid_llr_ext, mt, XCD_GRID(B, c.max_cands), s, grid, rec, ncand, llr0, c, nullptr, nullptr, nullptr, att0, ev, evc, B);
     k_worklist_att<<<(B * S * 5 + 255) / 256, 256, 0, s>>>(rec, ncand, att0, B, sh, wl[WL_BP0]);
     STAGE("bp_grid");
-    launch_mt(k_bp, k_bp_ext, mt, ladder_grid(B * c.max_cands * 5), s, 0, llr0, rec, ncand, nullptr, att0, nullptr, ev, evc, c, c.bp_nc0_a, c.bp_iters_a, wl[WL_BP0], 0, 5);
+    launch_mt(k_bp, k_bp_ext, mt, ladder_grid(B * c.max_cands * 5), s, 0, llr0, nullptr, att0, nullptr, ev, evc, c, c.bp_nc0_a, c.bp_iters_a, wl[WL_BP0], 0, 5, 1);
     STAGE("select0");
     k_select0<<<(B * S + 255) / 256, 256, 0, s>>>(rec, ncand, att0, B, sh, wl[WL_FINE]);
     STAGE("cycle_fft");
@@ -587,20 +587,18 @@
                 c.h0_lo < FT8RX_MIN_H0_FD || c.h0_hi > FT8RX_MAX_H0_FD + 1);
     k_worklist<<<(B * S + 255) / 256, 256, 0, s>>>(rec, ncand, B, sh, wl[WL_BP1]);
     STAGE("bp_fine");
-    const auto bp_fine = [&](int n_variants, const WorkList& work, int v0) {
-        launch_mt(k_bp, k_bp_ext, mt, B * c.max_cands * n_variants, s, 1, llr0, rec, ncand, attG, attB, saved, ev, evc, c, c.bp_nc0_b, c.bp_iters_b,
-                  work, v0, n_variants);
+    const auto bp_fine = [&](const WorkList& work, int v0, int n_waves, int n_seq) {
+        launch_mt(k_bp, k_bp_ext, mt, B * c.max_cands * n_waves, s, 1, llr0, attG, attB, saved, ev, evc, c, c.bp_nc0_b, c.bp_iters_b,
+                  work, v0, n_waves, n_seq);
     };
     if (h->ladder_mode == 0) {
-        bp_fine(1, wl[WL_BP1], 0);
-        k_select1<<<(B * S + 255) / 256, 256, 0, s>>>(0, rec, ncand, attG, attB, B, c, wl[WL_BP1B]);
-        bp_fine(1, wl[WL_BP1B], 1);
+        bp_fine(wl[WL_BP1], 0, 1, 2);
         k_select1<<<(B * S + 255) / 256, 256, 0, s>>>(1, rec, ncand, attG, attB, B, c, wl[WL_BP1C]);
-        bp_fine(3, wl[WL_BP1C], 2);
+        bp_fine(wl[WL_BP1C], 2, 3, 1);
         STAGE("select1");
         k_select1<<<(B * S + 255) / 256, 256, 0, s>>>(2, rec, ncand, attG, attB, B, c, wl[WL_OSD]);
     } else {
-        bp_fine(5, wl[WL_BP1], 0);
+        bp_fine(wl[WL_BP1], 0, 5, 1);
         STAGE("select1");
         k_select1<<<(B * S + 255) / 256, 256, 0, s>>>(3, rec, ncand, attG, attB, B, c, wl[WL_OSD]);
     }
@@ -1358,7 +1356,7 @@
     float* d_out = S.get<float>((size_t)n * 174); NEED(d_out);
     HIPCHK(h, hipMemset(d_out, 0, sizeof(float) * (size_t)n * 174));
     Att* d_att = S.get<Att>(n); NEED(d_att);
-    k_bp<<<n, 64, 0, h->stream>>>(2, d_in, nullptr, nullptr, nullptr, d_att, d_out, nullptr, nullptr, h->cfg, max_ncheck0, max_iters, WorkList{nullptr, nullptr}, 0, 1);
+    k_bp<<<n, 64, 0, h->stream>>>(2, d_in, nullptr, d_att, d_out, nullptr, nullptr, h->cfg, max_ncheck0, max_iters, WorkList{nullptr, nullptr}, 0, 1, 1);
     HIPCHK(h, hipStreamSynchronize(h->stream));
     std::vector<Att> a(n);
     HIPCHK(h, hipMemcpy(a.data(), d_att, sizeof(Att) * n, hipMemcpyDeviceToHost));
@@ -1790,11 +1788,11 @@
     if (!h) return -1;
     ENTER(h);
     if (hipDeviceSynchronize() != hipSuccess) return -2;
-    std::vector<unsigned long long> all((size_t)65536 * 8);
+    std::vector<unsigned long long> all((size_t)4 * 16384 * 8);
     if (out8) {
         if (hipMemcpyFromSymbol(all.data(), HIP_SYMBOL(g_bp_t), sizeof(unsigned long long) * all.size()) != hipSuccess) return -2;
-        for (int i = 0; i < 8; i++) out8[i] = 0;
-        for (size_t b = 0; b < 65536; b++) for (int i = 0; i < 8; i++) out8[i] += all[b * 8 + i];
+        for (int i = 0; i < 32; i++) out8[i] = 0;
+        for (size_t b = 0; b < 4 * 16384; b++) for (int i = 0; i < 8; i++) out8[(b / 16384) * 8 + i] += all[b * 8 + i];
     }
     if (reset) { std::fill(all.begin(), all.end(), 0ull); if (hipMemcpyToSymbol(HIP_SYMBOL(g_bp_t), all.data(), sizeof(unsigned long long) * all.size()) != hipSuccess) return -2; }
     return 0;
diff --git a/pyft8_amd/csrc/kernels/ap_calls.hpp b/pyft8_amd/csrc/kernels/ap_calls.hpp
--- a/pyft8_amd/csrc/kernels/ap_calls.hpp
+++ b/pyft8_amd/csrc/kernels/ap_calls.hpp
@@ -36,7 +36,7 @@
         asm volatile("" : "+v"(tid));
         const int c = cands.items[item / np], p = apc->pat[item % np];
         if (p >= 8) ap_codeword_test(tid, c, p, llr0, att7, ev, evcount, cand_shift(cfg), apc);
-        else bp_attempt<false, true>(tid, 1, (c << 4) | p, llr0, rec, ncand, nullptr, att7, nullptr, ev, evcount, cfg,
+        else bp_attempt<false, true>(tid, 1, (c << 4) | p, llr0, nullptr, att7, nullptr, ev, evcount, cfg,
                                      cfg.bp_nc0_b, cfg.bp_iters_b, 0u, apc, &osdl);
         __syncthreads();
     }
diff --git a/pyft8_amd/csrc/kernels/bp.hpp b/pyft8_amd/csrc/kernels/bp.hpp
--- a/pyft8_amd/csrc/kernels/bp.hpp
+++ b/pyft8_amd/csrc/kernels/bp.hpp
@@ -5,16 +5,16 @@
 #define BP_WV 7
 #endif
 #ifdef BP_TIMING
-__device__ unsigned long long g_bp_t[65536][8];
-#define BT_DECL unsigned long long bt_prev = __builtin_readcyclecounter();
-#define BT(i) do { const unsigned long long bt_now = __builtin_readcyclecounter(); if (lane == 0) atomicAdd(&g_bp_t[blockIdx.x & 65535][i], bt_now - bt_prev); bt_prev = __builtin_readcyclecounter(); } while (0)
+__device__ unsigned long long g_bp_t[4][16384][8];
+#define BT_DECL unsigned long long bt_prev = __builtin_readcyclecounter(); const int bt_l = AP7 ? 3 : mode == 0 ? 0 : (bid % 5) < 2 ? 1 : 2;
+#define BT(i) do { const unsigned long long bt_now = __builtin_readcyclecounter(); if (lane == 0) atomicAdd(&g_bp_t[bt_l][blockIdx.x & 16383][i], bt_now - bt_prev); bt_prev = __builtin_readcyclecounter(); } while (0)
 #else
 #define BT_DECL
 #define BT(i) do { } while (0)
 #endif
+enum { BP_OK = 1, BP_OK_A = 2, BP_DECIDED = 4 };
 template <bool EXT, bool AP7 = false>
-FT8_DEV void bp_attempt(int lane, int mode, int bid, const float* __restrict__ llr_in, ft8rx_record* __restrict__ rec,
-                        const int32_t* __restrict__ ncand, Att* __restrict__ attG, Att* __restrict__ attB,
+FT8_DEV int bp_attempt(int lane, int mode, int bid, const float* __restrict__ llr_in, Att* __restrict__ attG, Att* __restrict__ attB,
                         float* __restrict__ saved, ft8rx_event* ev, int32_t* evcount, const ft8rx_config& cfg,
                         int max_nc0, int max_iters, unsigned mt, const ApCalls* __restrict__ apc = nullptr, const WorkList* osdl = nullptr) {
     __shared__ float llr[176];
@@ -26,168 +26,188 @@
     uint64_t ho0 = 0, ho1 = 0, ho2 = 0;
     if (AP7) { ap = bid & 15; vec = (size_t)(bid >> 4); }
     else if (mode == 2) vec = bid;
-    else {
-        const int sh = cand_shift(cfg);
-        ap = bid % 5; const int c = bid / 5;
-        if ((c & ((1 << sh) - 1)) >= ncand[c >> sh]) return;
-        if (rec[c].status != FT8RX_ST_ACTIVE) return;
-        vec = (size_t)c;
-    }
-    {
-        const float* src = llr_in + vec * 174;
-        const float v0 = src[lane], v1 = src[64 + lane], v2 = src[128 + (lane < 46 ? lane : 0)];
-        if constexpr (AP7) {
-            llr[lane] = ap7_value(apc, ap, lane, v0); llr[64 + lane] = ap7_value(apc, ap, 64 + lane, v1);
-            if (lane < 46) llr[128 + lane] = ap7_value(apc, ap, 128 + lane, v2);
-            ho0 = __ballot(v0 > 0.0f); ho1 = __ballot(v1 > 0.0f); ho2 = __ballot(lane < 46 && v2 > 0.0f);
-        } else {
-            llr[lane] = ap_value(ap, lane, v0); llr[64 + lane] = ap_value(ap, 64 + lane, v1);
-            if (lane < 46) llr[128 + lane] = ap_value(ap, 128 + lane, v2);
-        }
-    }
+    else { ap = bid % 5; vec = (size_t)(bid / 5); }
+    const float* src = llr_in + vec * 174;
+    float v0 = src[lane], v1 = src[64 + lane], v2 = src[128 + (lane < 46 ? lane : 0)];
     if (lane < 2) llr[174 + lane] = 0.0f;
     if (lane == 0) P[83] = 1.0f;
-    __syncthreads();
-    Att res; memset(&res, 0, sizeof(res)); res.n_its = -1;
     if (!AP7 && mode == 1 && ap == 0) {
         bool any = false;
 #pragma unroll
         for (int g = 0; g < 2; g++) {
             Att resG; memset(&resG, 0, sizeof(resG)); resG.n_its = -1;
-            const uint64_t b0 = __ballot(ap_value(g, lane, llr[lane]) > 0.0f);
-            const uint64_t b1 = __ballot(lane < 27 && ap_value(g, 64 + lane, llr[64 + (lane < 27 ? lane : 0)]) > 0.0f);
+            const ApWords w = ap_words(g);
+            const uint64_t b0 = __ballot(ap_select(w.f0, w.v0, lane, v0) > 0.0f);
+            const uint64_t b1 = __ballot(ap_select(w.f1, w.v1, lane, v1) > 0.0f) & ((1ull << 27) - 1);
             uint64_t lo, hi;
             const int r = ft8_crc_check_wave<EXT>(b0, b1, lane, &lo, &hi, mt);
             if (r) { if (lane == 0) log_event(ev, evcount, (int)vec >> cand_shift(cfg), (int)vec & ((1 << cand_shift(cfg)) - 1), 2, g, 0, lo, hi, r == 2); }
             if (r == 2) { resG.ok = 1; resG.lo = lo; resG.hi = hi; resG.n_its = 0; resG.method = FT8RX_M_GOOD91; any = true; }
             if (lane == 0) attG[vec * 2 + g] = resG;
         }
-        if (any) return;
-    }
-    const int c0 = lane, c1 = lane + 64;
-    const uint64_t cm00 = d_CHK_MASK[c0][0], cm01 = d_CHK_MASK[c0][1], cm02 = d_CHK_MASK[c0][2];
-    const uint64_t cm10 = d_CHK_MASK[c1][0], cm11 = d_CHK_MASK[c1][1], cm12 = d_CHK_MASK[c1][2];
-    int ev_[9], ec_[9];
-    uint32_t ve_[3] = {0u, 0u, 0u};
-    int n0 = 0, n1 = 0;
-    bool tables = false;
-    float mc[9];
-#pragma unroll
-    for (int i = 0; i < 9; i++) mc[i] = 0.0f;
-    res.has_out = 1;
-    BT(0);
-    for (int it = 0; it < max_iters; it++) {
-        const uint64_t h0 = __ballot(llr[lane] > 0.0f), h1 = __ballot(llr[64 + lane] > 0.0f),
-                       h2 = __ballot(lane < 46 && llr[128 + (lane < 46 ? lane : 0)] > 0.0f);
-        const int par0 = (__popcll(h0 & cm00) + __popcll(h1 & cm01) + __popcll(h2 & cm02)) & 1;
-        const int par1 = (__popcll(h0 & cm10) + __popcll(h1 & cm11) + __popcll(h2 & cm12)) & 1;
-        int ncheck = __popcll(__ballot(par0)) + __popcll(__ballot(par1));
-        if (it == 0) { res.nc0 = (uint8_t)ncheck; if (ncheck > max_nc0) { res.has_out = 0; break; } }
-        if (ncheck == 0) {
-            uint64_t b0 = h0;
-            uint64_t b1 = h1 & ((1ull << 27) - 1);
-            uint64_t lo, hi;
-            int r = ft8_crc_check_wave<EXT>(b0, b1, lane, &lo, &hi, mt);
-            if constexpr (AP7) {
-                if (r && lane == 0) log_event(ev, evcount, (int)vec >> cand_shift(cfg), (int)vec & ((1 << cand_shift(cfg)) - 1), 7, 2 * ap, it + 1, lo, hi, r == 2);
-                const int hd = __popcll(h0 ^ ho0) + __popcll(h1 ^ ho1) + __popcll(h2 ^ ho2);
-                res.pad[1] = (uint8_t)(r == 2);
-                if (r == 2 && hd <= apc->max_hd) { res.ok = 1; res.lo = lo; res.hi = hi; res.n_its = (int16_t)it; res.pad[0] = (uint8_t)hd; }
-                res.has_out = 0;
+        BT(7);
+        if (any) return BP_DECIDED;
+    }
+#define BP_LDS_AT(arr, byte_off) (*reinterpret_cast<const float*>(reinterpret_cast<const char*>(arr) + (byte_off)))
+#define BP_LOAD_TABLES() do {                                                                                                              \
+        _Pragma("unroll")                                                                                                                  \
+        for (int i = 0; i < 9; i++) {                                                                                                      \
+            const int e = lane + 64 * i;                                                                                                   \
+            const uint32_t xv = (e < 522) ? d_EDGE_V[e] : 174, xc = (e < 522) ? d_EDGE_C[e] : 83;                                          \
+            evc_[i] = (xv << 2) | (xc << 18);                                                                                              \
+        }                                                                                                                                  \
+        n0 = d_CHK_N[c0];                                                                                                                  \
+        n1 = (c1 < 83) ? d_CHK_N[c1] : 0;                                                                                                  \
+        _Pragma("unroll")                                                                                                                  \
+        for (int q = 0; q < 3; q++) {                                                                                                      \
+            const int v = lane + 64 * q, vc = v < 174 ? v : 0;                                                                             \
+            ve_[q] = (uint32_t)d_VAR_E[vc][0] | ((uint32_t)d_VAR_E[vc][1] << 10) | ((uint32_t)d_VAR_E[vc][2] << 20);                       \
+        }                                                                                                                                  \
+    } while (0)
+    {
+        const int c0 = lane, c1 = lane + 64;
+        const uint64_t cm00 = d_CHK_MASK[c0][0], cm01 = d_CHK_MASK[c0][1], cm02 = d_CHK_MASK[c0][2];
+        const uint64_t cm10 = d_CHK_MASK[c1][0], cm11 = d_CHK_MASK[c1][1], cm12 = d_CHK_MASK[c1][2];
+        uint32_t evc_[9];
+        uint32_t ve_[3] = {0u, 0u, 0u};
+        int n0 = 0, n1 = 0;
+        bool tables = AP7 || mode != 0;
+        if (tables) BP_LOAD_TABLES();
+        uint64_t h0, h1, h2;
+        if constexpr (AP7) {
+            const float a0 = ap7_value(apc, ap, lane, v0), a1 = ap7_value(apc, ap, 64 + lane, v1), a2 = ap7_value(apc, ap, 128 + lane, v2);
+            ho0 = __ballot(v0 > 0.0f); ho1 = __ballot(v1 > 0.0f); ho2 = __ballot(lane < 46 && v2 > 0.0f);
+            v0 = a0; v1 = a1; v2 = a2;
+        } else {
+            const ApWords w = ap_words(ap);
+            v0 = ap_select(w.f0, w.v0, lane, v0); v1 = ap_select(w.f1, w.v1, lane, v1);
+        }
+        llr[lane] = v0; llr[64 + lane] = v1;
+        if (lane < 46) llr[128 + lane] = v2;
+        h0 = __ballot(v0 > 0.0f); h1 = __ballot(v1 > 0.0f); h2 = __ballot(lane < 46 && v2 > 0.0f);
+        __syncthreads();
+        Att res; memset(&res, 0, sizeof(res)); res.n_its = -1;
+        float mc[9];
+#pragma unroll
+        for (int i = 0; i < 9; i++) mc[i] = 0.0f;
+        res.has_out = 1;
+        BT(0);
+        for (int it = 0; it < max_iters; it++) {
+            const int par0 = (__popcll(h0 & cm00) + __popcll(h1 & cm01) + __popcll(h2 & cm02)) & 1;
+            const int par1 = (__popcll(h0 & cm10) + __popcll(h1 & cm11) + __popcll(h2 & cm12)) & 1;
+            int ncheck = __popcll(__ballot(par0)) + __popcll(__ballot(par1));
+            if (it == 0) { res.nc0 = (uint8_t)ncheck; if (ncheck > max_nc0) { res.has_out = 0; break; } }
+            if (ncheck == 0) {
+                uint64_t b0 = h0;
+                uint64_t b1 = h1 & ((1ull << 27) - 1);
+                uint64_t lo, hi;
+                int r = ft8_crc_check_wave<EXT>(b0, b1, lane, &lo, &hi, mt);
+                if constexpr (AP7) {
+                    if (r && lane == 0) log_event(ev, evcount, (int)vec >> cand_shift(cfg), (int)vec & ((1 << cand_shift(cfg)) - 1), 7, 2 * ap, it + 1, lo, hi, r == 2);
+                    const int hd = __popcll(h0 ^ ho0) + __popcll(h1 ^ ho1) + __popcll(h2 ^ ho2);
+                    res.pad[1] = (uint8_t)(r == 2);
+                    if (r == 2 && hd <= apc->max_hd) { res.ok = 1; res.lo = lo; res.hi = hi; res.n_its = (int16_t)it; res.pad[0] = (uint8_t)hd; }
+                    res.has_out = 0;
+                    break;
+                }
+                if (r) {
+                    int ipass = (mode == 0) ? 0 : ((ap < 2 && res.nc0 <= cfg.bp_nc0_a && it < cfg.bp_iters_a) ? 3 : 4);
+                    if (lane == 0) log_event(ev, evcount, (int)vec >> cand_shift(cfg), (int)vec & ((1 << cand_shift(cfg)) - 1), ipass, ap, it + 1, lo, hi, r == 2);
+                }
+                if (r == 2) { res.ok = 1; res.lo = lo; res.hi = hi; res.n_its = (int16_t)it; res.has_out = 0; }
                 break;
             }
-            if (r) {
-                int ipass = (mode == 0) ? 0 : ((ap < 2 && res.nc0 <= cfg.bp_nc0_a && it < cfg.bp_iters_a) ? 3 : 4);
-                if (lane == 0) log_event(ev, evcount, (int)vec >> cand_shift(cfg), (int)vec & ((1 << cand_shift(cfg)) - 1), ipass, ap, it + 1, lo, hi, r == 2);
-            }
-            if (r == 2) { res.ok = 1; res.lo = lo; res.hi = hi; res.n_its = (int16_t)it; res.has_out = 0; }
-            break;
-        }
-        BT(1);
-        if (!tables) {
-            tables = true;
-#pragma unroll
-            for (int i = 0; i < 9; i++) { int e = lane + 64 * i; ev_[i] = (e < 522) ? d_EDGE_V[e] : 174; ec_[i] = (e < 522) ? d_EDGE_C[e] : 83; }
-            n0 = d_CHK_N[c0];
-            n1 = (c1 < 83) ? d_CHK_N[c1] : 0;
-#pragma unroll
-            for (int q = 0; q < 3; q++) {
-                const int v = lane + 64 * q, vc = v < 174 ? v : 0;
-                ve_[q] = (uint32_t)d_VAR_E[vc][0] | ((uint32_t)d_VAR_E[vc][1] << 10) | ((uint32_t)d_VAR_E[vc][2] << 20);
-            }
-        }
-#pragma unroll
-        for (int i = 0; i < 9; i++) {
-            const int e = lane + 64 * i;
-            const float v2c = llr[ev_[i]] - mc[i];
-            tl[e] = ft8_tanhf(-v2c);
-        }
-        BT(2);
-        __syncthreads();
-        {
-            float Pp = tl[c0];
-#pragma unroll
-            for (int j = 1; j < 6; j++) Pp = Pp * tl[c0 + 83 * j];
-            if (n0 == 7) Pp = Pp * tl[439 + c0];
-            P[c0] = Pp;
-            if (c1 < 83) {
-                float Q = tl[c1];
-#pragma unroll
-                for (int j = 1; j < 6; j++) Q = Q * tl[c1 + 83 * j];
-                if (n1 == 7) Q = Q * tl[439 + c1];
-                P[c1] = Q;
-            }
-        }
-        BT(3);
-        __syncthreads();
-#pragma unroll
-        for (int i = 0; i < 9; i++) {
-            const int e = lane + 64 * i;
-            const float tti = tl[e];
-            const float Pc = P[ec_[i]];
-            const float nm = (Pc * tti) / (__builtin_fmaf(-1.18f, tti, Pc) * __builtin_fmaf(1.18f, tti, Pc));
-            dl[e] = nm - mc[i];
-            mc[i] = nm;
-        }
-        BT(4);
-        __syncthreads();
-#pragma unroll
-        for (int q = 0; q < 3; q++) {
-            const int v = lane + 64 * q;
-            if (v < 174) {
-                float col = 0.0f;
-                col += dl[ve_[q] & 1023u]; col += dl[(ve_[q] >> 10) & 1023u]; col += dl[ve_[q] >> 20];
-                llr[v] += col;
-            }
-        }
-        __syncthreads();
-        BT(5);
-    }
-    BT(6);
-    if constexpr (AP7) {
-        if (res.ok) res.method = FT8RX_M_LDPC_B;
-        if (lane == 0) { attB[vec * 10 + (ap - 5)] = res; if (!res.pad[1]) work_push(*osdl, bid); }
-        return;
-    }
-    if (res.ok) res.method = (mode == 0) ? FT8RX_M_LDPC_A : FT8RX_M_LDPC_B;
-    if (mode == 2) {
-        if (lane == 0) attB[vec] = res;
-        if (res.has_out) for (int i = lane; i < 174; i += 64) saved[vec * 174 + i] = llr[i];
-        return;
-    }
-    if (mode == 0) { if (lane == 0) attB[vec * 5 + ap] = res; return; }
-    if (lane == 0) attB[vec * 5 + ap] = res;
+            BT(1);
+            uint32_t sh0 = 0, sh16 = 16;
+            asm volatile("" : "+s"(sh0), "+s"(sh16));
+            if (!tables) { tables = true; BP_LOAD_TABLES(); }
+            float g[9];
+#pragma unroll
+            for (int i = 0; i < 9; i++) g[i] = BP_LDS_AT(llr, (evc_[i] >> sh0) & 0xFFFFu);
+#pragma unroll
+            for (int i = 0; i < 9; i++) {
+                const int e = lane + 64 * i;
+                const float v2c = g[i] - mc[i];
+                tl[e] = ft8_tanhf(-v2c);
+            }
+            BT(2);
+            __syncthreads();
+            {
+                float Pp = tl[c0];
+#pragma unroll
+                for (int j = 1; j < 6; j++) Pp = Pp * tl[c0 + 83 * j];
+                if (n0 == 7) Pp = Pp * tl[439 + c0];
+                P[c0] = Pp;
+                if (c1 < 83) {
+                    float Q = tl[c1];
+#pragma unroll
+                    for (int j = 1; j < 6; j++) Q = Q * tl[c1 + 83 * j];
+                    if (n1 == 7) Q = Q * tl[439 + c1];
+                    P[c1] = Q;
+                }
+            }
+            BT(3);
+            __syncthreads();
+#pragma unroll
+            for (int i = 0; i < 9; i++) g[i] = BP_LDS_AT(P, evc_[i] >> sh16);
+#pragma unroll
+            for (int i = 0; i < 9; i++) {
+                const int e = lane + 64 * i;
+                const float tti = tl[e];
+                const float Pc = g[i];
+                const float nm = (Pc * tti) / (__builtin_fmaf(-1.18f, tti, Pc) * __builtin_fmaf(1.18f, tti, Pc));
+                dl[e] = nm - mc[i];
+                mc[i] = nm;
+            }
+            BT(4);
+            __syncthreads();
+            {
+                float nv[3];
+#pragma unroll
+                for (int q = 0; q < 3; q++) {
+                    const int v = lane + 64 * q;
+                    nv[q] = 0.0f;
+                    if (v < 174) {
+                        float col = 0.0f;
+                        col += dl[ve_[q] & 1023u]; col += dl[(ve_[q] >> 10) & 1023u]; col += dl[ve_[q] >> 20];
+                        nv[q] = llr[v] + col;
+                        llr[v] = nv[q];
+                    }
+                }
+                h0 = __ballot(nv[0] > 0.0f); h1 = __ballot(nv[1] > 0.0f); h2 = __ballot(lane < 46 && nv[2] > 0.0f);
+            }
+            __syncthreads();
+            BT(5);
+        }
+        BT(6);
+        if constexpr (AP7) {
+            if (res.ok) res.method = FT8RX_M_LDPC_B;
+            if (lane == 0) { attB[vec * 10 + (ap - 5)] = res; if (!res.pad[1]) work_push(*osdl, bid); }
+            return 0;
+        }
+        if (res.ok) res.method = (mode == 0) ? FT8RX_M_LDPC_A : FT8RX_M_LDPC_B;
+        if (mode == 2) {
+            if (lane == 0) attB[vec] = res;
+            if (res.has_out) for (int i = lane; i < 174; i += 64) saved[vec * 174 + i] = llr[i];
+            return 0;
+        }
+        if (lane == 0) attB[vec * 5 + ap] = res;
+        if (mode == 0) return 0;
 #ifndef BP_TIMING_NO_SAVED
-    if (res.has_out) for (int i = lane; i < 174; i += 64) saved[(vec * 5 + ap) * 174 + i] = llr[i];
+        if (res.has_out) for (int i = lane; i < 174; i += 64) saved[(vec * 5 + ap) * 174 + i] = llr[i];
 #endif
-}
-
+        return __builtin_amdgcn_readfirstlane((res.ok ? BP_OK : 0) | (res.ok && res.nc0 <= cfg.bp_nc0_a && res.n_its < cfg.bp_iters_a ? BP_OK_A : 0));
+    }
+#undef BP_LOAD_TABLES
+#undef BP_LDS_AT
+}
+
+#define BP_LANE_ID() ({ int l_; asm volatile("v_mbcnt_lo_u32_b32 %0, -1, 0\n\tv_mbcnt_hi_u32_b32 %0, -1, %0" : "=v"(l_)); l_ & 63; })
 #define BP_KERNEL(NAME, EXT, MT_PARAM, MT)                                                                                                                       \
-__global__ __launch_bounds__(64, BP_WV) void NAME(int mode, const float* __restrict__ llr_in, ft8rx_record* __restrict__ rec,                         \
-                                           const int32_t* __restrict__ ncand, Att* __restrict__ attG, Att* __restrict__ attB,                         \
+__global__ __launch_bounds__(64, BP_WV) void NAME(int mode, const float* __restrict__ llr_in, Att* __restrict__ attG, Att* __restrict__ attB,          \
                                            float* __restrict__ saved, ft8rx_event* ev, int32_t* evcount, ft8rx_config cfg,                            \
-                                           int max_nc0, int max_iters, WorkList work, int ap_lo, int ap_n MT_PARAM) {                                      \
-    if (mode == 2) { bp_attempt<EXT>(threadIdx.x, 2, blockIdx.x, llr_in, rec, ncand, attG, attB, saved, ev, evcount, cfg, max_nc0, max_iters, MT); return; }\
+                                           int max_nc0, int max_iters, WorkList work, int ap_lo, int ap_n, int n_seq MT_PARAM) {                       \
+    if (mode == 2) { bp_attempt<EXT>(threadIdx.x, 2, blockIdx.x, llr_in, attG, attB, saved, ev, evcount, cfg, max_nc0, max_iters, MT); return; }     \
                     \
                        \
                          \
@@ -195,24 +215,35 @@
         const int n = *work.count;                                                                                                                    \
 _Pragma("unroll 1")                                                                                                                                   \
         for (int item = blockIdx.x; item < n; item += gridDim.x) {                                                                                    \
-            int tid = threadIdx.x;                                                                                                                    \
-            asm volatile("" : "+v"(tid));                           \
-            bp_attempt<EXT>(tid, 0, work.items[item], llr_in, rec, ncand, attG, attB, saved, ev, evcount, cfg, max_nc0, max_iters, MT);                   \
+            const int tid = BP_LANE_ID();                           \
+            bp_attempt<EXT>(tid, 0, work.items[item], llr_in, attG, attB, saved, ev, evcount, cfg, max_nc0, max_iters, MT);                         \
             __syncthreads();                                                                       \
         }                                                                                                                                             \
         return;                                                                                                                                       \
     }                                                                                                                                                 \
-                    \
-                \
+                       \
+               \
     const int item = blockIdx.x;                                                                                                                      \
     if (item >= *work.count * ap_n) return;                                                                                                           \
-    bp_attempt<EXT>(threadIdx.x, mode, work.items[item / ap_n] * 5 + ap_lo + item % ap_n, llr_in, rec, ncand, attG, attB, saved, ev, evcount, cfg, max_nc0, max_iters, MT);\
+    const int cand = work.items[item / ap_n];                                                                                                         \
+                \
+                      \
+    int seen = 0;                                                                                                     \
+_Pragma("unroll 1")                                                                                                                                   \
+    for (int bid = cand * 5 + ap_lo + (item % ap_n) * n_seq, left = n_seq; ; bid++) {                                                                 \
+        const int tid = BP_LANE_ID();                                                                  \
+        seen |= bp_attempt<EXT>(tid, mode, bid, llr_in, attG, attB, saved, ev, evcount, cfg, max_nc0, max_iters, MT);                                 \
+        if (--left == 0) return;                                                                                                                      \
+        if (seen & (bid % 5 == 0 ? BP_DECIDED | BP_OK_A : BP_OK)) return;                                                                             \
+        __syncthreads();                                                                           \
+    }                                                                                                                                                 \
 }
 #define BP_MT_PARAM , unsigned mt
 BP_KERNEL(k_bp, false, , 0u)
 BP_KERNEL(k_bp_ext, true, BP_MT_PARAM, mt)
 #undef BP_MT_PARAM
 #undef BP_KERNEL
+#undef BP_LANE_ID
 
 __global__ void k_select0(ft8rx_record* rec, const int32_t* ncand, const Att* att0, int B, int sh, WorkList next) {
     int c = blockIdx.x * blockDim.x + threadIdx.x;
@@ -254,13 +285,12 @@
         go_on = true;
         const Att* b = attB + (size_t)c * 5;
 #define IS_A(a) ((a).ok && (a).nc0 <= cfg.bp_nc0_a && (a).n_its < cfg.bp_iters_a)
-        if (step == 0) {
+        if (step == 1) {
             const Att& g0 = attG[(size_t)c * 2], & g1 = attG[(size_t)c * 2 + 1];
             if (g0.ok) go_on = sel_take(r, g0, 2, 0, FT8RX_M_GOOD91);
             else if (g1.ok) go_on = sel_take(r, g1, 2, 1, FT8RX_M_GOOD91);
             else if (IS_A(b[0])) go_on = sel_take(r, b[0], 3, 0, FT8RX_M_LDPC_A);
-        } else if (step == 1) {
-            if (IS_A(b[1])) go_on = sel_take(r, b[1], 3, 1, FT8RX_M_LDPC_A);
+            else if (IS_A(b[1])) go_on = sel_take(r, b[1], 3, 1, FT8RX_M_LDPC_A);
             else if (b[0].ok) go_on = sel_take(r, b[0], 4, 0, FT8RX_M_LDPC_B);
             else if (b[1].ok) go_on = sel_take(r, b[1], 4, 1, FT8RX_M_LDPC_B);
         } else if (step == 2) {
diff --git a/pyft8_amd/csrc/kernels/common.hpp b/pyft8_amd/csrc/kernels/common.hpp
--- a/pyft8_amd/csrc/kernels/common.hpp
+++ b/pyft8_amd/csrc/kernels/common.hpp
@@ -33,15 +33,28 @@
     return frame < B;
 }
 #define XCD_GRID(B, per) ((((B) + 7) / 8) * 8 * (per))
-enum { WL_BP0 = 0, WL_FINE = 1, WL_BP1 = 2, WL_BP1B = 3, WL_BP1C = 4, WL_OSD = 5, WL_OSDNAN = 6, WL_N = 7 };
+enum { WL_BP0 = 0, WL_FINE = 1, WL_BP1 = 2, WL_BP1C = 3, WL_OSD = 4, WL_OSDNAN = 5, WL_N = 6 };
 
 #define W6 ((double)(-0.16666667163372040f))
 
 #ifndef FT8RX_ILP_UNIT
-__device__ __constant__ int8_t d_AP_CQ[29]   = {0,0,0,0,0, 0,0,0,0,0, 0,0,0,0,0, 0,0,0,0,0, 0,0,0,0,0, 0,1,0,0};
-__device__ __constant__ int8_t d_AP_END[3][19] = {{0,1, 1,1,1,1,1, 0,0,1,1,1, 0,1,0,1,0, 0,1},
-                                                  {0,1, 1,1,1,1,1, 0,1,0,0,1, 0,1,0,0,0, 0,1},
-                                                  {0,1, 1,1,1,1,1, 0,1,0,0,1, 0,0,1,0,0, 0,1}};
+constexpr int8_t AP_CQ[29]   = {0,0,0,0,0, 0,0,0,0,0, 0,0,0,0,0, 0,0,0,0,0, 0,0,0,0,0, 0,1,0,0};
+constexpr int8_t AP_END[3][19] = {{0,1, 1,1,1,1,1, 0,0,1,1,1, 0,1,0,1,0, 0,1},
+                                  {0,1, 1,1,1,1,1, 0,1,0,0,1, 0,1,0,0,0, 0,1},
+                                  {0,1, 1,1,1,1,1, 0,1,0,0,1, 0,0,1,0,0, 0,1}};
+struct ApMasks { uint64_t f[5][2], v[5][2]; };
+constexpr ApMasks make_ap_masks() {
+    ApMasks m = {};
+    const auto force = [&m](int ap, int i, bool one) {
+        m.f[ap][i >> 6] |= 1ull << (i & 63);
+        if (one) m.v[ap][i >> 6] |= 1ull << (i & 63); else m.v[ap][i >> 6] &= ~(1ull << (i & 63));
+    };
+    for (int i = 0; i < 29; i++) force(1, i, AP_CQ[i] != 0);
+    force(1, 74, false); force(1, 75, false); force(1, 57, false); force(1, 58, false); force(1, 76, true);
+    for (int ap = 2; ap < 5; ap++) for (int i = 58; i < 77; i++) force(ap, i, AP_END[ap - 2][i - 58] != 0);
+    return m;
+}
+constexpr ApMasks AP_MASKS = make_ap_masks();
 __device__ uint8_t  d_CHK_N[83];
 __device__ int16_t  d_CHK_V[83][7];
 __device__ uint8_t  d_EDGE_V[522];
diff --git a/pyft8_amd/csrc/kernels/llr.hpp b/pyft8_amd/csrc/kernels/llr.hpp
--- a/pyft8_amd/csrc/kernels/llr.hpp
+++ b/pyft8_amd/csrc/kernels/llr.hpp
@@ -49,15 +49,38 @@
 }
 
 #ifndef FT8RX_ILP_UNIT
+constexpr int ap_rule(int ap, int i) {
+    if (ap == 1) {
+        if (i < 29) return AP_CQ[i] ? 1 : -1;
+        if (i == 74 || i == 75 || i == 57 || i == 58) return -1;
+        if (i == 76) return 1;
+    } else if (ap >= 2) {
+        if (i >= 58 && i < 77) return AP_END[ap - 2][i - 58] ? 1 : -1;
+    }
+    return 0;
+}
+constexpr bool ap_masks_match_rule() {
+    for (int ap = 0; ap < 5; ap++)
+        for (int i = 0; i < 174; i++) {
+            const bool f = i < 128 && ((AP_MASKS.f[ap][i >> 6 & 1] >> (i & 63)) & 1), one = i < 128 && ((AP_MASKS.v[ap][i >> 6 & 1] >> (i & 63)) & 1);
+            if ((f ? (one ? 1 : -1) : 0) != ap_rule(ap, i) || (!f && one)) return false;
+        }
+    return true;
+}
+static_assert(ap_masks_match_rule(), "AP_MASKS must be the reference's AP rule, position by position");
+#define AP_MASK_WORD(field, ap, w) ((ap) == 1 ? AP_MASKS.field[1][w] : (ap) == 2 ? AP_MASKS.field[2][w] : (ap) == 3 ? AP_MASKS.field[3][w] : \
+                                    (ap) == 4 ? AP_MASKS.field[4][w] : 0ull)
+FT8_DEV float ap_select(uint64_t forced, uint64_t value, int bit, float v) {
+    const float k = ((value >> bit) & 1) ? 5.0f : -5.0f;
+    return ((forced >> bit) & 1) ? k : v;
+}
+struct ApWords { uint64_t f0, v0, f1, v1; };
+FT8_DEV ApWords ap_words(int ap) { return ApWords{AP_MASK_WORD(f, ap, 0), AP_MASK_WORD(v, ap, 0), AP_MASK_WORD(f, ap, 1), AP_MASK_WORD(v, ap, 1)}; }
 FT8_DEV float ap_value(int ap, int i, float v) {
-    if (ap == 1) {
-        if (i < 29) return d_AP_CQ[i] ? 5.0f : -5.0f;
-        if (i == 74 || i == 75 || i == 57 || i == 58) return -5.0f;
-        if (i == 76) return 5.0f;
-    } else if (ap >= 2) {
-        if (i >= 58 && i < 77) return d_AP_END[ap - 2][i - 58] ? 5.0f : -5.0f;
-    }
-    return v;
+    const int w = i >> 6;
+    const uint64_t forced = w == 0 ? AP_MASK_WORD(f, ap, 0) : w == 1 ? AP_MASK_WORD(f, ap, 1) : 0ull;
+    const uint64_t value = w == 0 ? AP_MASK_WORD(v, ap, 0) : AP_MASK_WORD(v, ap, 1);
+    return ap_select(forced, value, i & 63, v);
 }
 
 struct ChkMasks { uint64_t m[6]; };
```

After: 88550. About the same (-0.2%).
